# iris1997jiatong/I-DCCRN-VAE

Hardware: AMD Instinct MI355X
Metric: 4s@16kHz utterances/sec fwd+SI-SNR, DCCRN-CL, 1/2/4/8 MI355X vs host CPU (higher is better)
Workload: dtype f32; 1 GPU; supervised DCCRN-CL forward(train=False) + final_ete_loss (weights 0/0/1); batch_per_gpu=64, utterance=4 s @ 16 kHz (64000 samples, 641 frames), parallelism=replicas x1, streams=1, input=resident in HBM

## Files before the change

i-dccrn-vae_amd/csrc/cgemm_tw.hip:

```cpp
#include <atomic>
#include <cstdint>
#include <cstdlib>
#include <type_traits>
#include "cgemm.hpp"
#include "../../include/idccrn_hip.h"

namespace {

struct TwArgs {
    const float* x0;
    const float* x1;
    int C0, C1;
    int Fin, Fout;
    int J, Jp, Tp;
    const float* wfrag;
    int UP;
    const float* epi;
    int has_fold;
    const float* slope;
    float* out;
    int Cout, cotiles;
    int tshift, t_valid;
    double* stats;
    int stats_rep;
    const float* add;
    int add_div, add_Jp;
    int jtiles, ftiles;
    int xcd_split;
    int cgroups;
    int stagger;
};

constexpr int TW_PACK_CI = 8;

template <int PH> __device__ __forceinline__ int tw_ra(int r) {
    if (PH == 0) return r == 0 ? 0 : (r == 2 ? 2 : 1);
    return r == 0 ? 1 : 2;
}
template <int PH> __device__ __forceinline__ int tw_rb(int r) {
    if (PH == 0) return r == 2 ? 1 : (r == 3 ? 3 : 2);
    return r == 0 ? 2 : 3;
}
template <int PH> __device__ __forceinline__ float tw_cb(int r) {
    if (PH == 0) return r == 1 ? 1.f : -1.f;
    return r == 1 ? 0.f : -1.f;
}
template <int PH> constexpr int tw_nr() { return PH == 0 ? 4 : 3; }
template <int PH> constexpr int tw_nt() { return tw_nr<PH>() * 9; }
template <int PH> constexpr int tw_ntp() { return PH == 0 ? 36 : 32; }
template <int PH> constexpr int tw_ntw() { return (tw_nt<PH>() + 3) / 4; }
__host__ __device__ inline int tw_tile(int ph, int w, int k) {
    if (ph == 0) return w * 9 + k;
    if (w < 3) return k < 6 ? w * 9 + k : w * 9 + 8;
    return k < 6 ? (k >> 1) * 9 + 6 + (k & 1) : -1;
}
template <int PH> constexpr int tw_wslots() { return PH == 0 ? 9 : 8; }

template <int PH, int CIK, bool LEFT, int DBG = 0, int RDW = 2, bool WVEC = true, bool STATS = false, int NCT = 1>
__global__ __launch_bounds__(256 * NCT, NCT == 1 ? 2 : 1) void cconv_tw_kernel(const TwArgs a) {
    constexpr int NR = tw_nr<PH>(), NT = tw_nt<PH>(), NTP = tw_ntp<PH>(), NTW = tw_ntw<PH>();
    constexpr int NRAW = PH == 0 ? 4 : 3, ROW0 = PH == 0 ? 0 : 1;
    constexpr int KS = CIK / 2;
    constexpr int RT = NRAW * 9 * 32;
    constexpr int NE = CIK * RT;
    constexpr int NBUF = 2;
    constexpr int NITEM = CIK * NRAW * 16;
    constexpr int NTHR = 256 * NCT;
    constexpr int NLD = (NITEM + NTHR - 1) / NTHR;
    static_assert(NCT == 1 || NCT == 2, "one or two co tiles per workgroup");
    static_assert(KS % RDW == 0 && NLD <= 2, "weight ring slots are compile-time; at most two staging items per thread");
    static_assert(NLD + NCT - 1 < KS, "the staging k-steps (from 1 on, waves 4 .. 7 one later) end before the barrier's k-step");
    static_assert(NCT * NT * 4 * 64 <= NBUF * NE, "the epilogue exchange (one area per co tile) fits the patch buffers");

    extern __shared__ __attribute__((aligned(16))) float smem[];

    const int tid = threadIdx.x;
    const int lane = tid & 63;
    const int wave = __builtin_amdgcn_readfirstlane(tid >> 6);
    const int w4 = NCT == 1 ? wave : wave & 3, cth = NCT == 1 ? 0 : wave >> 2;
    const int half = lane >> 5, l31 = lane & 31;

    const int bid = blockIdx.x;
    const int xcd = bid & 7, slot = bid >> 3;
    int jt, ft, ct;
    if (a.xcd_split) {
        const int G = 8 / a.cgroups;
        ct = xcd % a.cgroups;
        jt = (slot / a.ftiles) * G + xcd / a.cgroups;
        ft = slot - (slot / a.ftiles) * a.ftiles;
    } else {
        const int per = a.cgroups * a.ftiles;
        jt = (slot / per) * 8 + xcd;
        const int rem = slot - (slot / per) * per;
        ft = rem / a.cgroups;
        ct = rem - ft * a.cgroups;
    }
    if (jt >= a.jtiles) return;
    ct = NCT * ct + cth;
    const int j0 = jt * 64;
    const int m0 = 2 * ft;
    const int rbase = m0 - 1 + ROW0;

    const int Cin = a.C0 + a.C1;
    const int nchunk = (Cin + CIK - 1) / CIK;

    f32x16 acc[NTW];
#pragma unroll
    for (int k = 0; k < NTW; ++k)
#pragma unroll
        for (int r = 0; r < 16; ++r) acc[k][r] = 0.f;
    constexpr int NPAIR = (NTW - 1) / 2;
    constexpr bool UNI = PH == 0;
    int offA[UNI ? 1 : NPAIR + 1], offB[UNI ? 1 : NPAIR + 1];
    float cbj[UNI ? 1 : NPAIR + 1];
    if (UNI) {
        cbj[0] = tw_cb<PH>(w4);
        offA[0] = (tw_ra<PH>(w4) - ROW0) * 288;
        offB[0] = (tw_rb<PH>(w4) - ROW0) * 288;
    } else {
#pragma unroll
        for (int j = 0; j <= NPAIR; ++j) {
            int t = tw_tile(PH, w4, j < NPAIR ? 2 * j : NTW - 1);
            t = t < 0 ? 0 : t;
            const int r = t / 9, plane = t - r * 9;
            cbj[j] = tw_cb<PH>(r);
            const int po = plane == 8 ? 256 : (plane >> 1) * 64;
            offA[j] = (tw_ra<PH>(r) - ROW0) * 288 + po;
            offB[j] = cbj[j] != 0.f ? (tw_rb<PH>(r) - ROW0) * 288 + po : offA[j];
        }
    }

    f32x4 v_r[NLD], v_i[NLD];
    float e_r[NLD], e_i[NLD];
    unsigned off_v[NLD], off_e[NLD], ldsoff[NLD];
    unsigned okmask[NLD];
    int item_cl[NLD];
    bool interior[NLD];
#pragma unroll
    for (int i = 0; i < NLD; ++i) {
        const int e = tid + i * NTHR;
        const int c8 = e & 15;
        const int rl = (e >> 4) % NRAW, cl = e / (16 * NRAW);
        item_cl[i] = cl;
        const int f = rbase + rl;
        const int jc = j0 + 4 * c8;
        const int je = LEFT ? jc - 1 : jc + 4;
        const bool exists = e < NITEM;
        const bool okr = exists && f >= 0 && f < a.Fin;
        unsigned m = 0;
#pragma unroll
        for (int q = 0; q < 5; ++q) {
            const int c = jc + q + (LEFT ? -1 : 0);
            if (c >= 0 && c < a.J) m |= 1u << q;
        }
        if (okr) m |= 1u << 5;
        if (exists) m |= 1u << 7;
        const int jcv = jc + 3 < a.Jp ? jc : 0;
        const int jev = (je >= 0 && je < a.Jp) ? je : 0;
        off_v[i] = okr ? (unsigned)((cl * a.Fin + f) * a.Jp + jcv) : 0u;
        off_e[i] = okr ? (unsigned)((cl * a.Fin + f) * a.Jp + jev) : 0u;
        if (jc + 3 >= a.Jp) m &= ~0x1fu;
        if (!(je >= 0 && je < a.Jp)) m &= LEFT ? ~1u : ~(1u << 4);
        okmask[i] = m;
        interior[i] = __builtin_amdgcn_ballot_w64((m & 0xbfu) == 0xbfu) == ~0ull;
        ldsoff[i] = (unsigned)((cl * NRAW + rl) * 288 + 4 * c8);
    }
    auto stage_load = [&](int chunk, int i) {
        const int ci0 = chunk * CIK;
        const bool from0 = ci0 < a.C0;
        const float* br = from0 ? a.x0 + (size_t)ci0 * a.Fin * a.Jp : a.x1 + (size_t)(ci0 - a.C0) * a.Fin * a.Jp;
        const float* bi = from0 ? br + (size_t)a.C0 * a.Fin * a.Jp : br + (size_t)a.C1 * a.Fin * a.Jp;
        const int cvalid = (from0 ? a.C0 : Cin) - ci0;
        const bool dead = item_cl[i] >= cvalid;
        const unsigned ov = dead ? 0u : off_v[i], oe = dead ? 0u : off_e[i];
        v_r[i] = *(const f32x4*)(br + ov);
        v_i[i] = *(const f32x4*)(bi + ov);
        e_r[i] = br[oe];
        e_i[i] = bi[oe];
    };
    float fr[5], fi[5];
    auto stage_window = [&](int chunk, int i) {
        const int ci0s = chunk * CIK;
        const int cvalid = (ci0s < a.C0 ? a.C0 : Cin) - ci0s;
        constexpr bool left = LEFT;
        if (interior[i] && cvalid >= CIK) {
#pragma unroll
            for (int q = 0; q < 5; ++q) {
                fr[q] = left ? (q == 0 ? e_r[i] : v_r[i][q == 0 ? 0 : q - 1]) : (q == 4 ? e_r[i] : v_r[i][q == 4 ? 3 : q]);
                fi[q] = left ? (q == 0 ? e_i[i] : v_i[i][q == 0 ? 0 : q - 1]) : (q == 4 ? e_i[i] : v_i[i][q == 4 ? 3 : q]);
            }
            return;
        }
        unsigned m = okmask[i];
        if (item_cl[i] >= cvalid || !((m >> 5) & 1u)) m &= ~0x1fu;
#pragma unroll
        for (int q = 0; q < 5; ++q) {
            const float xr = left ? (q == 0 ? e_r[i] : v_r[i][q == 0 ? 0 : q - 1]) : (q == 4 ? e_r[i] : v_r[i][q == 4 ? 3 : q]);
            const float xi = left ? (q == 0 ? e_i[i] : v_i[i][q == 0 ? 0 : q - 1]) : (q == 4 ? e_i[i] : v_i[i][q == 4 ? 3 : q]);
            const bool cok = (m >> q) & 1u;
            fr[q] = cok ? xr : 0.f;
            fi[q] = cok ? xi : 0.f;
        }
    };
    auto plane_val = [&](int gt, int pr) -> float {
        const int g = gt / 3, tau = gt - g * 3;
        const int q0 = 2 * pr;
        const float xa_ = g == 0 ? fr[q0] + fi[q0] : (g == 1 ? fr[q0] : fi[q0]);
        const float xb_ = g == 0 ? fr[q0 + 1] + fi[q0 + 1] : (g == 1 ? fr[q0 + 1] : fi[q0 + 1]);
        const float xd_ = g == 0 ? fr[q0 + 2] + fi[q0 + 2] : (g == 1 ? fr[q0 + 2] : fi[q0 + 2]);
        return tau == 0 ? xa_ - xb_ : (tau == 1 ? xb_ : xb_ - xd_);
    };
    auto item_exists = [&](int i) -> bool { return NITEM >= (i + 1) * NTHR || wave * 64 + i * NTHR < NITEM; };
    auto stage_plane2 = [&](float* dst, int i, int j) {
        if (!item_exists(i)) return;
        if (j < 4) {
            f32x4 o = {plane_val(2 * j, 0), plane_val(2 * j + 1, 0), plane_val(2 * j, 1), plane_val(2 * j + 1, 1)};
            *(f32x4*)(dst + ldsoff[i] + j * 64) = o;
        } else {
            *(float2*)(dst + ldsoff[i] - 2 * (int)(tid & 15) + 256) = make_float2(plane_val(8, 0), plane_val(8, 1));
        }
    };
    auto stage_store = [&](float* dst, int chunk, int i) {
        stage_window(chunk, i);
#pragma unroll
        for (int j = 0; j < 5; ++j) stage_plane2(dst, i, j);
    };

    constexpr int WS = tw_wslots<PH>();
    const float* wbase = a.wfrag + ((size_t)(PH == 1 ? (size_t)a.cotiles * a.UP * tw_ntp<0>() : 0) + (size_t)ct * a.UP * NTP) * 64 +
                         (size_t)w4 * WS * 64;
    const int total_ks = nchunk * KS;
    float a_w[RDW][NTW];
    auto load_w = [&](int g, float (&dst)[NTW]) {
        g = g < total_ks ? g : total_ks - 1;
        const float* ws = wbase + (size_t)g * NTP * 64;
        if (WVEC) {
            const f32x4 w0 = *(const f32x4*)(ws + lane * 4), w1 = *(const f32x4*)(ws + 256 + lane * 4);
#pragma unroll
            for (int k = 0; k < 4; ++k) {
                dst[k] = w0[k];
                if (4 + k < NTW) dst[4 + k] = w1[k];
            }
            if (NTW == 9) dst[NTW - 1] = ws[512 + lane];
        } else {
#pragma unroll
            for (int k = 0; k < NTW; ++k) dst[k] = ws[k * 64 + lane];
        }
    };
    float xa[NTW], xb[NTW];
    auto load_raw2 = [&](const float* base, int j) {
        if (j < NPAIR) {
            const int oa = UNI ? offA[0] + j * 64 : offA[UNI ? 0 : j], ob = UNI ? offB[0] + j * 64 : offB[UNI ? 0 : j];
            const float2 pa_ = *(const float2*)(base + oa + 2 * l31), pb_ = *(const float2*)(base + ob + 2 * l31);
            xa[2 * j] = pa_.x; xa[2 * j + 1] = pa_.y;
            xb[2 * j] = pb_.x; xb[2 * j + 1] = pb_.y;
        } else {
            xa[NTW - 1] = base[(UNI ? offA[0] + 256 : offA[UNI ? 0 : NPAIR]) + l31];
            xb[NTW - 1] = base[(UNI ? offB[0] + 256 : offB[UNI ? 0 : NPAIR]) + l31];
        }
    };
    auto load_raw_all = [&](const float* base) {
#pragma unroll
        for (int j = 0; j <= NPAIR; ++j) load_raw2(base, j);
    };

#pragma unroll
    for (int i = 0; i < NLD; ++i) stage_load(0, i);
#pragma unroll
    for (int u = 0; u < RDW; ++u) load_w(u, a_w[u]);
#pragma unroll
    for (int i = 0; i < NLD; ++i) stage_store(smem, 0, i);
#pragma unroll
    for (int i = 0; i < NLD; ++i) stage_load(nchunk > 1 ? 1 : 0, i);
    __syncthreads();

    load_raw_all(smem + (size_t)half * RT);
    auto run = [&](auto late_) {
        constexpr bool LATE = decltype(late_)::value;
        for (int chunk = 0; chunk < nchunk; ++chunk) {
            const float* P = smem + (chunk & 1) * NE;
            float* Pn = smem + ((chunk + 1) & 1) * NE;
            const int nxt = chunk + 1 < nchunk ? chunk + 1 : chunk, nxt2 = chunk + 2 < nchunk ? chunk + 2 : nchunk - 1;
#pragma unroll
            for (int ul = 0; ul < KS; ++ul) {
                const float* bnext = ul + 1 < KS ? P + (size_t)(2 * (ul + 1) + half) * RT : Pn + (size_t)half * RT;
                const int si = ul - 1 - (LATE ? 1 : 0);
                const bool staging = !(DBG & 1) && si >= 0 && si < NLD;
#pragma unroll
                for (int k = 0; k < NTW; ++k) {
                    const float b = xa[k] + cbj[UNI ? 0 : (k >> 1 < NPAIR ? k >> 1 : NPAIR)] * xb[k];
                    acc[k] = __builtin_amdgcn_mfma_f32_32x32x2f32(a_w[ul % RDW][k], b, acc[k], 0, 0, 0);
                    if (ul == KS - 1 && k == 0) {
                        __builtin_amdgcn_sched_barrier(0);
                        __syncthreads();
                    }
                    if ((k & 1) && (k >> 1) < NPAIR) load_raw2(bnext, k >> 1);
                    if (k == NTW - 1) load_raw2(bnext, NPAIR);
                    if (staging) {
                        if (k == 0) stage_window(nxt, si);
                        if ((k & 1) && k < 6) stage_plane2(Pn, si, k >> 1);
                        if (k == (NTW == 9 ? 7 : 6)) stage_plane2(Pn, si, 3);
                        if (k == NTW - 1) stage_plane2(Pn, si, 4);
                        if (k == NTW - 1) stage_load(nxt2, si);
                    }
                    __builtin_amdgcn_sched_barrier(0);
                }
                if (!(DBG & 2)) load_w(chunk * KS + ul + RDW, a_w[ul % RDW]);
            }
        }
    };
    if (NCT == 2 && PH == 1 && a.stagger && cth)
        run(std::integral_constant<bool, NCT == 2 && PH == 1>{});
    else
        run(std::false_type{});
    __syncthreads();

    const float slope = a.slope ? *a.slope : 1.0f;
    const bool has_act = a.slope != nullptr;
    float* E = smem + cth * (NT * 4 * 64);
    const int jA = j0 + 2 * l31;
    bool keep[2], inb[2];
    int ja[2];
#pragma unroll
    for (int q = 0; q < 2; ++q) {
        const int j = jA + q;
        const int bj = j / a.Tp, tp = j - bj * a.Tp;
        inb[q] = j < a.J;
        keep[q] = inb[q] && tp >= 1 && tp <= a.t_valid;
        ja[q] = j - (bj - bj / a.add_div) * a.Tp;
    }
#pragma unroll
    for (int s = 0; s < ((DBG & 4) ? 1 : 4); ++s) {
        if (s > 0) __syncthreads();
#pragma unroll
        for (int k = 0; k < NTW; ++k) {
            const int t = tw_tile(PH, w4, k);
            if (t >= 0) {
#pragma unroll
                for (int rr = 0; rr < 4; ++rr) E[(t * 4 + rr) * 64 + lane] = acc[k][4 * s + rr];
            }
        }
        __syncthreads();
        float v[NT];
#pragma unroll
        for (int t = 0; t < NT; ++t) v[t] = E[(t * 4 + w4) * 64 + lane];
        float pr[NR][2], pi[NR][2];
#pragma unroll
        for (int r = 0; r < NR; ++r) {
            float y[3][2];
#pragma unroll
            for (int g = 0; g < 3; ++g) {
                const float m1 = v[r * 9 + g * 3], m2 = v[r * 9 + g * 3 + 1], m3 = v[r * 9 + g * 3 + 2];
                y[g][0] = m1 + m2;
                y[g][1] = m2 - m3;
            }
#pragma unroll
            for (int q = 0; q < 2; ++q) {
                pr[r][q] = y[0][q] - y[2][q];
                pi[r][q] = y[0][q] + y[1][q];
            }
        }
        const int rg = 4 * s + w4;
        const int co = ct * 32 + (rg & 3) + 8 * (rg >> 2) + 4 * half;
        const bool cok = co < a.Cout;
        const f32x4 e0 = *(const f32x4*)(a.epi + (size_t)co * 8);
        const float e4 = a.epi[(size_t)co * 8 + 4], e5 = a.epi[(size_t)co * 8 + 5];
        float st[5] = {0.f, 0.f, 0.f, 0.f, 0.f};
#pragma unroll
        for (int rt = 0; rt < 2; ++rt) {
            const int fo = 2 * m0 + PH + 2 * rt;
            if (fo >= a.Fout) continue;
            float yr[2], yi[2];
#pragma unroll
            for (int q = 0; q < 2; ++q) {
                float re, im;
                if (PH == 0) {
                    re = rt == 0 ? pr[0][q] + pr[1][q] + pr[2][q] : pr[1][q] - pr[2][q] - pr[NR - 1][q];
                    im = rt == 0 ? pi[0][q] + pi[1][q] + pi[2][q] : pi[1][q] - pi[2][q] - pi[NR - 1][q];
                } else {
                    re = rt == 0 ? pr[0][q] + pr[1][q] : pr[1][q] - pr[2][q];
                    im = rt == 0 ? pi[0][q] + pi[1][q] : pi[1][q] - pi[2][q];
                }
                if (a.add && cok && inb[q]) {
                    re += a.add[((size_t)co * a.Fout + fo) * a.add_Jp + ja[q]];
                    im += a.add[((size_t)(a.Cout + co) * a.Fout + fo) * a.add_Jp + ja[q]];
                }
                float r_, i_;
                if (a.has_fold) {
                    r_ = e0[0] * re + e0[1] * im + e4;
                    i_ = e0[2] * re + e0[3] * im + e5;
                } else {
                    r_ = re + e4;
                    i_ = im + e5;
                }
                if (has_act) {
                    r_ = r_ >= 0.f ? r_ : slope * r_;
                    i_ = i_ >= 0.f ? i_ : slope * i_;
                }
                yr[q] = keep[q] ? r_ : 0.f;
                yi[q] = keep[q] ? i_ : 0.f;
                if (STATS && keep[q]) {
                    st[0] += yr[q];
                    st[1] += yi[q];
                    st[2] += yr[q] * yr[q];
                    st[3] += yi[q] * yi[q];
                    st[4] += yr[q] * yi[q];
                }
            }
            if (cok) {
                float* o_r = a.out + ((size_t)co * a.Fout + fo) * a.Jp + jA;
                float* o_i = a.out + ((size_t)(a.Cout + co) * a.Fout + fo) * a.Jp + jA;
                if (inb[1]) {
                    *(float2*)o_r = make_float2(yr[0], yr[1]);
                    *(float2*)o_i = make_float2(yi[0], yi[1]);
                } else if (inb[0]) {
                    o_r[0] = yr[0];
                    o_i[0] = yi[0];
                }
            }
        }
        if (STATS) {
#pragma unroll
            for (int q = 0; q < 5; ++q) {
                float tsum = st[q];
#pragma unroll
                for (int o = 16; o > 0; o >>= 1) tsum += __shfl_xor(tsum, o, 64);
                if (l31 == 0 && cok)
                    atomicAdd(&a.stats[((size_t)(a.stats_rep > 1 ? (blockIdx.x & (a.stats_rep - 1)) : 0) * a.Cout + co) * 5 + q], (double)tsum);
            }
        }
    }
}

__global__ void pack_cconv_tw_kernel(const float* __restrict__ wino, int cotiles, int UN, int UP, int vec, float* __restrict__ out) {
    const long long n0 = (long long)cotiles * UP * tw_ntp<0>() * 64, n1 = (long long)cotiles * UP * tw_ntp<1>() * 64;
    for (long long idx = blockIdx.x * (long long)blockDim.x + threadIdx.x; idx < n0 + n1; idx += (long long)gridDim.x * blockDim.x) {
        const int ph = idx >= n0;
        const long long i = ph ? idx - n0 : idx;
        const int ntp = ph ? tw_ntp<1>() : tw_ntp<0>(), nt = ph ? tw_nt<1>() : tw_nt<0>();
        const int lane = (int)(i & 63);
        long long t_ = i >> 6;
        const int t = (int)(t_ % ntp); t_ /= ntp;
        const int u = (int)(t_ % UP);
        const int ct = (int)(t_ / UP);
        float val = 0.f;
        const int ws_ = ph ? tw_wslots<1>() : tw_wslots<0>();
        const int pos = t * 64 + lane, w = pos / (ws_ * 64), q = pos % (ws_ * 64);
        const bool vec_ = (vec >> ph) & 1;
        const int k = !vec_ ? q >> 6 : (q < 512 ? (q >> 8) * 4 + (q & 3) : 8);
        const int ln = !vec_ ? q & 63 : (q < 512 ? (q & 255) >> 2 : q - 512);
        const int tt = k < (ph ? 7 : 9) ? tw_tile(ph, w, k) : -1;
        const int ci = 2 * u + (ln >> 5), co = ln & 31;
        if (tt >= 0 && ci * 3 < UN) {
            const int r = tt / 9, g = (tt % 9) / 3, tau = tt % 3;
            const float* src = wino + ((((size_t)ph * cotiles + ct) * UN + (size_t)ci * 3 + g) * 4 + r) * 64;
            const float w0 = src[co], w1 = src[32 + co];
            val = tau == 0 ? w0 : (tau == 1 ? w0 + w1 : w1);
        }
        out[idx] = val;
    }
}

template <int PH, int CIK, bool LEFT, int DBG, int RDW, bool WVEC = true, bool STATS = false, int NCT = 1>
int launch_tw_ph_l(const TwArgs& a, hipStream_t st);
inline int tw_wvec_mask() {
    static const int v = [] { const char* e = getenv("IDV_TW_WVEC"); return e ? atoi(e) : 1; }();
    return v;
}
template <int PH, int CIK, int DBG = 0, int RDW = 2>
int launch_tw_ph(const TwArgs& a, hipStream_t st) {
    const bool wv = (tw_wvec_mask() >> PH) & 1;
    if (DBG == 0 && RDW == 2 && wv == (PH == 0) && a.cotiles % 2 == 0 && ((idv_tw_pair(-1) >> PH) & 1)) {
        constexpr bool WV = PH == 0;
        if (a.stats) return a.tshift ? launch_tw_ph_l<PH, CIK, true, 0, 2, WV, true, 2>(a, st) : launch_tw_ph_l<PH, CIK, false, 0, 2, WV, true, 2>(a, st);
        return a.tshift ? launch_tw_ph_l<PH, CIK, true, 0, 2, WV, false, 2>(a, st) : launch_tw_ph_l<PH, CIK, false, 0, 2, WV, false, 2>(a, st);
    }
    if (DBG == 0 && RDW == 2 && a.stats) {
        constexpr bool WV = PH == 0;
        if (wv != WV) return IDV_EINVAL;
        return a.tshift ? launch_tw_ph_l<PH, CIK, true, 0, 2, WV, true>(a, st) : launch_tw_ph_l<PH, CIK, false, 0, 2, WV, true>(a, st);
    }
    if (DBG == 0 && RDW == 2 && !wv)
        return a.tshift ? launch_tw_ph_l<PH, CIK, true, 0, 2, false>(a, st) : launch_tw_ph_l<PH, CIK, false, 0, 2, false>(a, st);
    return a.tshift ? launch_tw_ph_l<PH, CIK, true, DBG, RDW>(a, st) : launch_tw_ph_l<PH, CIK, false, DBG, RDW>(a, st);
}
template <int PH, int CIK, bool LEFT, int DBG, int RDW, bool WVEC, bool STATS, int NCT>
int launch_tw_ph_l(const TwArgs& a, hipStream_t st) {
    constexpr int NE = CIK * (PH == 0 ? 4 : 3) * 9 * 32;
    constexpr size_t smem = 2 * NE * sizeof(float);
    static_assert(smem * (NCT == 1 ? 2 : 1) <= 160 * 1024, "the patch buffers of two workgroups (NCT = 2: of one) must fit the 160 KB of LDS");
    TwArgs b = a;
    b.jtiles = (a.J + 63) / 64;
    b.ftiles = PH == 1 ? a.Fin / 2 : (a.Fin + 1) / 2;
    if (b.ftiles == 0) return IDV_OK;
    static const int xsplit = [] { const char* e = getenv("IDV_TW_XCD_SPLIT"); return e ? atoi(e) : 1; }();
    b.cgroups = b.cotiles / NCT;
    if (b.cgroups * NCT != b.cotiles) return IDV_EINVAL;
    static const int stag = [] { const char* e = getenv("IDV_TW_PAIR_STAGGER"); return e ? atoi(e) : 1; }();
    b.stagger = stag;
    b.xcd_split = (xsplit && (b.cgroups == 2 || b.cgroups == 4 || b.cgroups == 8)) ? 1 : 0;
    long long nblk = (long long)((b.jtiles + 7) / 8) * 8 * b.ftiles * b.cgroups;
    if (b.xcd_split) {
        const int G = 8 / b.cgroups;
        nblk = (long long)((b.jtiles + G - 1) / G) * b.ftiles * 8;
    }
    if (nblk > 0x7fffffffLL) return IDV_EINVAL;
    auto k = cconv_tw_kernel<PH, CIK, LEFT, DBG, RDW, WVEC, STATS, NCT>;
    static std::atomic<bool> attr_set[64];
    int dev = 0;
    if (hipGetDevice(&dev) != hipSuccess || dev < 0 || dev >= 64) return IDV_ELAUNCH;
    if (smem > 64 * 1024 && !attr_set[dev].load(std::memory_order_acquire)) {
        if (hipFuncSetAttribute((const void*)k, hipFuncAttributeMaxDynamicSharedMemorySize, (int)smem) != hipSuccess) return IDV_ELAUNCH;
        attr_set[dev].store(true, std::memory_order_release);
    }
    hipLaunchKernelGGL(k, dim3((unsigned)nblk), dim3(256 * NCT), smem, st, b);
    if (NCT > 1) idv_tw_pair_note_launch();
    return idv_launch_status();
}

}

namespace {
std::atomic<int>& tw_pair_mask() {
    static std::atomic<int> v{[] { const char* e = getenv("IDV_TW_PAIR"); return e ? atoi(e) & IDV_TW_PAIR_ALL : IDV_TW_PAIR_DEFAULT; }()};
    return v;
}
std::atomic<long long> tw_pair_launches{0};
}
void idv_tw_pair_note_launch() { tw_pair_launches.fetch_add(1, std::memory_order_relaxed); }
extern "C" int idv_tw_pair(int mask) {
    if (mask < 0) return tw_pair_mask().load(std::memory_order_relaxed);
    return tw_pair_mask().exchange(mask & IDV_TW_PAIR_ALL, std::memory_order_relaxed);
}
extern "C" long long idv_tw_pair_launches(int reset) {
    return reset ? tw_pair_launches.exchange(0, std::memory_order_relaxed) : tw_pair_launches.load(std::memory_order_relaxed);
}

extern "C" int idv_cconv_tw_supported(int C0, int C1, int Cout, int Fin) {
    static const int min_cout = [] { const char* e = getenv("IDV_TW_MIN_COUT"); return e ? atoi(e) : 32; }();
    if (Cout < min_cout || Fin < 2) return 0;
    if (!idv_cconv_gauss_supported(C0, C1, Cout)) return 0;
    return (C1 == 0 || C0 % 8 == 0) ? 1 : 0;
}

extern "C" long long idv_cconv_tw_wfrag_floats(int Cout, int cin_used) {
    const long long cotiles = (Cout + 31) / 32, cpad = (cin_used + TW_PACK_CI - 1) / TW_PACK_CI * TW_PACK_CI;
    return cotiles * (cpad / 2) * (36 + 32) * 64;
}

extern "C" int idv_pack_cconv_tw(const float* wino_frag, int Cout, int cin_used, float* tw_frag, void* stream) {
    if (!wino_frag || !tw_frag || Cout <= 0 || cin_used <= 0) return IDV_EINVAL;
    const int cotiles = (Cout + 31) / 32;
    const int cpad = (cin_used + TW_PACK_CI - 1) / TW_PACK_CI * TW_PACK_CI;
    const long long n = idv_cconv_tw_wfrag_floats(Cout, cin_used);
    const unsigned blocks = (unsigned)((n + 255) / 256 > 4096 ? 4096 : (n + 255) / 256);
    hipLaunchKernelGGL(pack_cconv_tw_kernel, dim3(blocks), dim3(256), 0, (hipStream_t)stream, wino_frag, cotiles, cpad * 3, cpad / 2,
                       tw_wvec_mask(), tw_frag);
    return idv_launch_status();
}

extern "C" int idv_ctconv2d_tw_fwd(const float* x0, int C0, const float* x1, int C1, const float* wfrag, const float* epi, int has_fold,
                                   const float* prelu_slope, float* out, double* stats, double* stats_work, int stats_rep, int tshift,
                                   int Cout, int Fin, int B, int Tp, int Jp, int t_valid_out, const float* addend, int addend_div,
                                   int addend_Jp, void* stream) {
    if (!x0 || !wfrag || !epi || !out || C0 <= 0 || Cout <= 0 || Fin <= 0 || B <= 0 || Tp <= 1) return IDV_EINVAL;
    if (stats && stats_work && (stats_rep < 2 || (stats_rep & (stats_rep - 1)))) return IDV_EINVAL;
    if (addend && (addend_div < 1 || B % addend_div || addend_Jp < (B / addend_div) * Tp)) return IDV_EINVAL;
    if (C1 > 0 && !x1) return IDV_EINVAL;
    if (tshift != 0 && tshift != -1) return IDV_EINVAL;
    if (!idv_cconv_tw_supported(C0, C1, Cout, Fin)) return IDV_EINVAL;
    if ((Jp & 3) || (reinterpret_cast<uintptr_t>(x0) & 15) || (C1 > 0 && (reinterpret_cast<uintptr_t>(x1) & 15)) ||
        (reinterpret_cast<uintptr_t>(out) & 7))
        return IDV_EINVAL;
    TwArgs a{};
    a.x0 = x0; a.x1 = x1; a.C0 = C0; a.C1 = C1;
    a.Fin = Fin; a.Fout = 2 * Fin - 1;
    a.J = B * Tp; a.Jp = Jp; a.Tp = Tp;
    a.wfrag = wfrag; a.UP = (C0 + C1 + TW_PACK_CI - 1) / TW_PACK_CI * TW_PACK_CI / 2;
    a.epi = epi; a.has_fold = has_fold; a.slope = prelu_slope; a.out = out;
    a.Cout = Cout; a.cotiles = (Cout + 31) / 32;
    a.tshift = tshift; a.t_valid = t_valid_out;
    a.add = addend; a.add_div = addend ? addend_div : 1; a.add_Jp = addend_Jp;
    if (Jp < a.J) return IDV_EINVAL;
    if ((long long)8 * Fin * (long long)Jp >= 0xffffffffLL) return IDV_EINVAL;
    hipStream_t st = (hipStream_t)stream;
    a.stats = stats;
    if (stats && stats_work) { a.stats = stats_work; a.stats_rep = stats_rep; }
    int rc = 0;
#ifdef IDV_TW_EXPERIMENTS
    static const int dbg = [] { const char* e = getenv("IDV_TW_DBG"); return e ? atoi(e) : 0; }();
    static const int only = [] { const char* e = getenv("IDV_TW_ONLY"); return e ? atoi(e) : 0; }();
    if (dbg && !stats) {
        if (only != 2) rc = dbg == 1 ? launch_tw_ph<0, 8, 1>(a, st) : (dbg == 2 ? launch_tw_ph<0, 8, 2>(a, st) : launch_tw_ph<0, 8, 3>(a, st));
        if (rc) return rc;
        if (only != 1) rc = dbg == 1 ? launch_tw_ph<1, 8, 1>(a, st) : (dbg == 2 ? launch_tw_ph<1, 8, 2>(a, st) : launch_tw_ph<1, 8, 3>(a, st));
        return rc;
    }
    if (only) return only == 1 ? launch_tw_ph<0, 8>(a, st) : launch_tw_ph<1, 8>(a, st);
#endif
    rc = launch_tw_ph<0, 8>(a, st);
    if (!rc) rc = launch_tw_ph<1, 8>(a, st);
    if (rc || !(stats && stats_work)) return rc;
    return idv_launch_stats_collapse(stats_work, stats_rep, Cout * 5, stats, st);
}
```

i-dccrn-vae_amd/csrc/cgemm_tw2.hip:

```cpp
#include <atomic>
#include <cstdint>
#include <cstdlib>
#include <type_traits>
#include "cgemm.hpp"
#include "../../include/idccrn_hip.h"

namespace {

struct Tw2Args {
    const float* x0;
    int Cin;
    int Fin, Fout;
    int J, Jp, Tp;
    const float* wfrag;
    int UP;
    const float* epi;
    int has_fold;
    const float* slope;
    float* out;
    int Cout, cotiles;
    int tshift, t_valid;
    double* stats;
    int stats_rep;
    int jtiles, ftiles;
    int xcd_split;
    int cgroups;
    int stagger;
};

constexpr int TW2_PACK_CI = 8;

__host__ __device__ constexpr int tw2_ra(int q) { return q == 0 ? 0 : (q == 1 ? 2 : (q == 2 ? 4 : (q == 3 ? 2 : (q == 4 ? 1 : 3)))); }
__host__ __device__ constexpr int tw2_rb(int q) { return q == 0 ? 4 : (q == 1 ? 4 : (q == 2 ? 2 : (q == 3 ? 6 : (q == 4 ? 3 : (q == 5 ? 3 : 5))))); }
__host__ __device__ constexpr float tw2_cb(int q) { return q == 1 ? 1.f : (q == 5 ? 0.f : -1.f); }
__host__ __device__ constexpr int tw2_qx(int a) { return a == 0 ? 0 : (a == 1 ? 1 : 3); }
__host__ __device__ constexpr int tw2_qy(int a) { return a == 0 ? 4 : (a == 1 ? 5 : 6); }
__host__ __device__ constexpr int tw2_main_acc(int w) { return w == 2 ? 3 : w; }
__host__ __device__ inline void tw2_slot(int w, int k, int& q, int& plane) {
    if (w < 3) {
        if (k < 14) { q = (k & 1) ? tw2_qy(tw2_main_acc(w)) : tw2_qx(tw2_main_acc(w)); plane = k >> 1; }
        else { q = 2; plane = 2 * w + (k - 14); }
    } else {
        if (k < 12) { const int a = tw2_main_acc(k >> 2); q = (k & 1) ? tw2_qy(a) : tw2_qx(a); plane = 7 + ((k >> 1) & 1); }
        else if (k < 15) { q = 2; plane = 6 + (k - 12); }
        else { q = -1; plane = 0; }
    }
}
__host__ __device__ inline int tw2_acc_tile(int w, int i) {
    if (w < 3) return i < 7 ? tw2_main_acc(w) * 9 + i : 2 * 9 + 2 * w + (i - 7);
    return i < 6 ? tw2_main_acc(i >> 1) * 9 + 7 + (i & 1) : 2 * 9 + 6 + (i - 6);
}

__device__ __forceinline__ int tw2_poff(int p, int l31) { return p < 8 ? (p >> 1) * 64 + 2 * l31 + (p & 1) : 256 + l31; }

constexpr int tw2_smem_floats(int nct) {
    return nct == 1 ? 2 * 4 * 7 * 288 : (2 * (4 * 7 * 288 + 288) > 2 * 36 * 4 * 64 ? 2 * (4 * 7 * 288 + 288) : 2 * 36 * 4 * 64);
}
template <bool LEFT, bool STATS, int DBG = 0, int NCT = 1>
__global__ __launch_bounds__(256 * NCT, NCT == 1 ? 2 : 1) void cconv_tw2_kernel(const Tw2Args a) {
    constexpr int NT = 36, NACC = 9, NSLOT = 16;
    constexpr int NRAW = 7, CIK = 4, KS = 2;
    constexpr int RT = NRAW * 288;
    constexpr int NE = CIK * RT;
    constexpr int NEB = NCT == 1 ? NE : NE + 288;
    constexpr int NITEM = CIK * NRAW * 16;
    constexpr int NTHR = 256 * NCT;
    constexpr int NLD = (NITEM + NTHR - 1) / NTHR;
    static_assert(NCT == 1 || NCT == 2, "one or two co tiles per workgroup");
    static_assert(2 * NEB <= tw2_smem_floats(NCT) && NCT * NT * 4 * 64 <= tw2_smem_floats(NCT),
                  "the patch buffers and the epilogue exchange (one area per co tile) fit the allocation");

    extern __shared__ __attribute__((aligned(16))) float smem[];

    const int tid = threadIdx.x;
    const int lane = tid & 63;
    const int wave = __builtin_amdgcn_readfirstlane(tid >> 6);
    const int w4 = NCT == 1 ? wave : wave & 3, cth = NCT == 1 ? 0 : wave >> 2;
    const int half = lane >> 5, l31 = lane & 31;

    const int bid = blockIdx.x;
    const int xcd = bid & 7, slot = bid >> 3;
    int jt, ft, ct;
    if (a.xcd_split) {
        const int G = 8 / a.cgroups;
        ct = xcd % a.cgroups;
        jt = (slot / a.ftiles) * G + xcd / a.cgroups;
        ft = slot - (slot / a.ftiles) * a.ftiles;
    } else {
        const int per = a.cgroups * a.ftiles;
        jt = (slot / per) * 8 + xcd;
        const int rem = slot - (slot / per) * per;
        ft = rem / a.cgroups;
        ct = rem - ft * a.cgroups;
    }
    if (jt >= a.jtiles) return;
    ct = NCT * ct + cth;
    const int j0 = jt * 64;
    const int m0 = 2 * ft;
    const int rbase = 2 * m0 - 2;

    const int Cin = a.Cin;
    const int nchunk = (Cin + CIK - 1) / CIK;

    f32x16 acc[NACC];
#pragma unroll
    for (int k = 0; k < NACC; ++k)
#pragma unroll
        for (int r = 0; r < 16; ++r) acc[k][r] = 0.f;

    f32x4 v_r[NLD], v_i[NLD];
    float e_r[NLD], e_i[NLD];
    unsigned off_v[NLD], ldsoff[NLD];
    unsigned okmask[NLD];
    bool interior[NLD];
    auto item_cl = [&](int i) -> int { return (tid + i * NTHR) / (16 * NRAW); };
#pragma unroll
    for (int i = 0; i < NLD; ++i) {
        const int e = tid + i * NTHR;
        const int c8 = e & 15;
        const int cl = e / (16 * NRAW), rl = (NCT == 2 && e >= NITEM) ? 0 : (e >> 4) % NRAW;
        const int f = rbase + rl;
        const int jc = j0 + 4 * c8;
        const int je = LEFT ? jc - 1 : jc + 4;
        const bool exists = e < NITEM;
        const bool okr = exists && f >= 0 && f < a.Fin;
        unsigned m = 0;
#pragma unroll
        for (int q = 0; q < 5; ++q) {
            const int c = jc + q + (LEFT ? -1 : 0);
            if (c >= 0 && c < a.J) m |= 1u << q;
        }
        if (okr) m |= 1u << 5;
        const int jcv = jc + 3 < a.Jp ? jc : 0;
        off_v[i] = okr ? (unsigned)((cl * a.Fin + f) * a.Jp + jcv) : 4u;
        if (jc + 3 >= a.Jp) m &= ~0x1fu;
        if (!(je >= 0 && je < a.Jp)) m &= LEFT ? ~1u : ~(1u << 4);
        okmask[i] = m;
        interior[i] = __builtin_amdgcn_ballot_w64((m & 0x3fu) == 0x3fu) == ~0ull;
        ldsoff[i] = (unsigned)((cl * NRAW + rl) * 288 + 4 * c8);
    }
    auto item_exists = [&](int i) -> bool { return i == 0 || wave * 64 + 256 < NITEM; };
    auto stage_load = [&](int chunk, int i) {
        if (!item_exists(i)) return;
        const int ci0 = chunk * CIK;
        const float* br = a.x0 + (size_t)ci0 * a.Fin * a.Jp;
        const float* bi = br + (size_t)Cin * a.Fin * a.Jp;
        const bool dead = item_cl(i) >= Cin - ci0;
        const unsigned ov = dead ? 4u : off_v[i];
        v_r[i] = *(const f32x4*)(br + ov);
        v_i[i] = *(const f32x4*)(bi + ov);
        e_r[i] = (br + ov)[LEFT ? -1 : 4];
        e_i[i] = (bi + ov)[LEFT ? -1 : 4];
    };
    float fr[5], fi[5];
    auto stage_window = [&](int chunk, int i) {
        if (!item_exists(i)) return;
        const int cvalid = Cin - chunk * CIK;
        constexpr bool left = LEFT;
        if (interior[i] && cvalid >= CIK) {
#pragma unroll
            for (int q = 0; q < 5; ++q) {
                fr[q] = left ? (q == 0 ? e_r[i] : v_r[i][q == 0 ? 0 : q - 1]) : (q == 4 ? e_r[i] : v_r[i][q == 4 ? 3 : q]);
                fi[q] = left ? (q == 0 ? e_i[i] : v_i[i][q == 0 ? 0 : q - 1]) : (q == 4 ? e_i[i] : v_i[i][q == 4 ? 3 : q]);
            }
            return;
        }
        unsigned m = okmask[i];
        if (item_cl(i) >= cvalid || !((m >> 5) & 1u)) m &= ~0x1fu;
#pragma unroll
        for (int q = 0; q < 5; ++q) {
            const float xr = left ? (q == 0 ? e_r[i] : v_r[i][q == 0 ? 0 : q - 1]) : (q == 4 ? e_r[i] : v_r[i][q == 4 ? 3 : q]);
            const float xi = left ? (q == 0 ? e_i[i] : v_i[i][q == 0 ? 0 : q - 1]) : (q == 4 ? e_i[i] : v_i[i][q == 4 ? 3 : q]);
            const bool cok = (m >> q) & 1u;
            fr[q] = cok ? xr : 0.f;
            fi[q] = cok ? xi : 0.f;
        }
    };
    auto plane_val = [&](int gt, int pr) -> float {
        const int g = gt / 3, tau = gt - g * 3;
        const int q0 = 2 * pr;
        const float xa_ = g == 0 ? fr[q0] + fi[q0] : (g == 1 ? fr[q0] : fi[q0]);
        const float xb_ = g == 0 ? fr[q0 + 1] + fi[q0 + 1] : (g == 1 ? fr[q0 + 1] : fi[q0 + 1]);
        const float xd_ = g == 0 ? fr[q0 + 2] + fi[q0 + 2] : (g == 1 ? fr[q0 + 2] : fi[q0 + 2]);
        return tau == 0 ? xa_ - xb_ : (tau == 1 ? xb_ : xb_ - xd_);
    };
    auto stage_plane2 = [&](float* dst, int i, int j) {
        if (!item_exists(i)) return;
        if (j < 4) {
            f32x4 o = {plane_val(2 * j, 0), plane_val(2 * j + 1, 0), plane_val(2 * j, 1), plane_val(2 * j + 1, 1)};
            *(f32x4*)(dst + ldsoff[i] + j * 64) = o;
        } else {
            *(float2*)(dst + ldsoff[i] - 2 * (int)(tid & 15) + 256) = make_float2(plane_val(8, 0), plane_val(8, 1));
        }
    };
    auto stage_store = [&](float* dst, int chunk, int i) {
        stage_window(chunk, i);
#pragma unroll
        for (int j = 0; j < 5; ++j) stage_plane2(dst, i, j);
    };

    const float* wbase = a.wfrag + (((size_t)ct * a.UP) * 4 + w4) * 1024 + lane * 4;
    const int total_ks = nchunk * KS;
    float a_w[NSLOT];
    auto load_wg = [&](int g, int grp) {
        g = g < total_ks ? g : total_ks - 1;
        const f32x4 w4 = *(const f32x4*)(wbase + (size_t)g * 4096 + grp * 256);
#pragma unroll
        for (int k = 0; k < 4; ++k) a_w[grp * 4 + k] = w4[k];
    };

    const int am = tw2_main_acc(w4 < 3 ? w4 : 0);
    const int qxm = tw2_qx(am), qym = tw2_qy(am);
    const int rxa = tw2_ra(qxm) * 288, rxb = tw2_rb(qxm) * 288, rya = tw2_ra(qym) * 288, ryb = tw2_rb(qym) * 288;
    const float cbx = tw2_cb(qxm), cby = tw2_cb(qym);
    const int r2a = tw2_ra(2) * 288 + w4 * 64, r2b = tw2_rb(2) * 288 + w4 * 64;
    float xa[2][4], xb[2][4];
    auto load_grp_a = [&](const float* base, int g, float (&oa)[4], float (&ob)[4]) {
        if (g < 3) {
            const float2 xa_ = *(const float2*)(base + rxa + g * 64 + 2 * l31), xb_ = *(const float2*)(base + rxb + g * 64 + 2 * l31);
            const float2 ya_ = *(const float2*)(base + rya + g * 64 + 2 * l31), yb_ = *(const float2*)(base + ryb + g * 64 + 2 * l31);
            oa[0] = xa_.x; oa[2] = xa_.y; ob[0] = xb_.x; ob[2] = xb_.y;
            oa[1] = ya_.x; oa[3] = ya_.y; ob[1] = yb_.x; ob[3] = yb_.y;
        } else {
            oa[0] = base[rxa + 3 * 64 + 2 * l31]; ob[0] = base[rxb + 3 * 64 + 2 * l31];
            oa[1] = base[rya + 3 * 64 + 2 * l31]; ob[1] = base[ryb + 3 * 64 + 2 * l31];
            const float2 pa_ = *(const float2*)(base + r2a + 2 * l31), pb_ = *(const float2*)(base + r2b + 2 * l31);
            oa[2] = pa_.x; oa[3] = pa_.y; ob[2] = pb_.x; ob[3] = pb_.y;
        }
    };
    auto load_grp_b = [&](const float* base, int g, float (&oa)[4], float (&ob)[4]) {
#pragma unroll
        for (int s4 = 0; s4 < 4; ++s4) {
            int q, plane;
            tw2_slot(3, 4 * g + s4, q, plane);
            if (q < 0) continue;
            oa[s4] = base[tw2_ra(q) * 288 + tw2_poff(plane, l31)];
            ob[s4] = base[tw2_rb(q) * 288 + tw2_poff(plane, l31)];
        }
    };

#pragma unroll
    for (int i = 0; i < NLD; ++i) stage_load(0, i);
#pragma unroll
    for (int grp = 0; grp < 4; ++grp) load_wg(0, grp);
#pragma unroll
    for (int i = 0; i < NLD; ++i) stage_store(smem, 0, i);
#pragma unroll
    for (int i = 0; i < NLD; ++i) stage_load(nchunk > 1 ? 1 : 0, i);
    __syncthreads();
    if (w4 < 3)
        load_grp_a(smem + (size_t)half * RT, 0, xa[0], xb[0]);
    else
        load_grp_b(smem + (size_t)half * RT, 0, xa[0], xb[0]);

    auto run = [&](auto role, auto late_) {
        constexpr bool ROLE_B = decltype(role)::value;
        for (int chunk = 0; chunk < nchunk; ++chunk) {
            const float* P = smem + (chunk & 1) * NEB;
            float* Pn = smem + ((chunk + 1) & 1) * NEB;
            const int nxt = chunk + 1 < nchunk ? chunk + 1 : chunk, nxt2 = chunk + 2 < nchunk ? chunk + 2 : nchunk - 1;
#pragma unroll
            for (int ul = 0; ul < KS; ++ul) {
                const float* bnext = ul + 1 < KS ? P + (size_t)(2 * (ul + 1) + half) * RT : Pn + (size_t)half * RT;
                const bool staging = !(DBG & 1) && ul == 0;
#pragma unroll
                for (int k = 0; k < (ROLE_B ? NSLOT - 1 : NSLOT); ++k) {
                    const int g = k >> 2, s4 = k & 3;
                    float cb;
                    int ai;
                    if (ROLE_B) {
                        int q, plane;
                        tw2_slot(3, k, q, plane);
                        cb = tw2_cb(q);
                        ai = k < 12 ? k >> 1 : 6 + (k - 12);
                    } else {
                        cb = k < 14 ? ((k & 1) ? cby : cbx) : -1.f;
                        ai = k < 14 ? k >> 1 : 7 + (k - 14);
                    }
                    if (s4 == 0) {
                        const float* src = g < 3 ? P + (size_t)(2 * ul + half) * RT : bnext;
                        if (!(ul == KS - 1 && g == 3)) {
                            if (ROLE_B) load_grp_b(src, (g + 1) & 3, xa[(g + 1) & 1], xb[(g + 1) & 1]);
                            else load_grp_a(src, (g + 1) & 3, xa[(g + 1) & 1], xb[(g + 1) & 1]);
                        }
                    }
                    const float b = xa[g & 1][s4] + cb * xb[g & 1][s4];
                    acc[ai] = __builtin_amdgcn_mfma_f32_32x32x2f32(a_w[k], b, acc[ai], 0, 0, 0);
                    if (ul == KS - 1 && k == 0) {
                        __builtin_amdgcn_sched_barrier(0);
                        __syncthreads();
                    }
                    if (ul == KS - 1 && k == 12) {
                        if (ROLE_B) load_grp_b(bnext, 0, xa[0], xb[0]);
                        else load_grp_a(bnext, 0, xa[0], xb[0]);
                    }
                    if (((k & 3) == 3 || (ROLE_B && k == NSLOT - 2)) && !(DBG & 2)) load_wg(chunk * KS + ul + 1, k >> 2);
                    if constexpr (NCT == 2) if (staging) {
                        constexpr bool late = decltype(late_)::value;
                        if (k <= 5 && !late) {
                            if (k == 0) stage_window(nxt, 0);
                            if (k >= 1) stage_plane2(Pn, 0, k - 1);
                            if (k == 5) stage_load(nxt2, 0);
                        }
                        if (k >= 8 && k <= 13 && late) {
                            if (k == 8) stage_window(nxt, 0);
                            if (k >= 9) stage_plane2(Pn, 0, k - 9);
                            if (k == 13) stage_load(nxt2, 0);
                        }
                    }
                    if constexpr (NCT == 1) if (staging) {
                        if (k == 0) stage_window(nxt, 0);
                        if (k >= 1 && k <= 5) stage_plane2(Pn, 0, k - 1);
                        if (k == 5) stage_load(nxt2, 0);
                        if (!ROLE_B) {
                            if (k == 8) stage_window(nxt, 1);
                            if (k >= 9 && k <= 13) stage_plane2(Pn, 1, k - 9);
                            if (k == 13) stage_load(nxt2, 1);
                        }
                    }
                    __builtin_amdgcn_sched_barrier(0);
                }
            }
        }
    };
    if (NCT == 2 && a.stagger && cth) {
        if (w4 < 3)
            run(std::false_type{}, std::integral_constant<bool, NCT == 2>{});
        else
            run(std::true_type{}, std::integral_constant<bool, NCT == 2>{});
    } else if (w4 < 3)
        run(std::false_type{}, std::false_type{});
    else
        run(std::true_type{}, std::false_type{});
    __syncthreads();

    const float slope = a.slope ? *a.slope : 1.0f;
    const bool has_act = a.slope != nullptr;
    float* E = smem + cth * (NT * 4 * 64);
    const int jA = j0 + 2 * l31;
    bool keep[2], inb[2];
#pragma unroll
    for (int q = 0; q < 2; ++q) {
        const int j = jA + q;
        const int tp = j % a.Tp;
        inb[q] = j < a.J;
        keep[q] = inb[q] && tp >= 1 && tp <= a.t_valid;
    }
#pragma unroll
    for (int s = 0; s < 4; ++s) {
        if (s > 0) __syncthreads();
#pragma unroll
        for (int k = 0; k < NACC; ++k) {
            const int t = tw2_acc_tile(w4, k);
#pragma unroll
            for (int rr = 0; rr < 4; ++rr) E[(t * 4 + rr) * 64 + lane] = acc[k][4 * s + rr];
        }
        __syncthreads();
        float v[NT];
#pragma unroll
        for (int t = 0; t < NT; ++t) v[t] = E[(t * 4 + w4) * 64 + lane];
        float pr[4][2], pi[4][2];
#pragma unroll
        for (int r = 0; r < 4; ++r) {
            float y[3][2];
#pragma unroll
            for (int g = 0; g < 3; ++g) {
                const float m1 = v[r * 9 + g * 3], m2 = v[r * 9 + g * 3 + 1], m3 = v[r * 9 + g * 3 + 2];
                y[g][0] = m1 + m2;
                y[g][1] = m2 - m3;
            }
#pragma unroll
            for (int q = 0; q < 2; ++q) {
                pr[r][q] = y[0][q] - y[2][q];
                pi[r][q] = y[0][q] + y[1][q];
            }
        }
        const int rg = 4 * s + w4;
        const int co = ct * 32 + (rg & 3) + 8 * (rg >> 2) + 4 * half;
        const bool cok = co < a.Cout;
        const f32x4 e0 = *(const f32x4*)(a.epi + (size_t)co * 8);
        const float e4 = a.epi[(size_t)co * 8 + 4], e5 = a.epi[(size_t)co * 8 + 5];
        float st[5] = {0.f, 0.f, 0.f, 0.f, 0.f};
#pragma unroll
        for (int rt = 0; rt < 2; ++rt) {
            const int fo = m0 + rt;
            if (fo >= a.Fout) continue;
            float yr[2], yi[2];
#pragma unroll
            for (int q = 0; q < 2; ++q) {
                const float re = rt == 0 ? pr[0][q] + pr[1][q] + pr[2][q] : pr[1][q] - pr[2][q] - pr[3][q];
                const float im = rt == 0 ? pi[0][q] + pi[1][q] + pi[2][q] : pi[1][q] - pi[2][q] - pi[3][q];
                float r_, i_;
                if (a.has_fold) {
                    r_ = e0[0] * re + e0[1] * im + e4;
                    i_ = e0[2] * re + e0[3] * im + e5;
                } else {
                    r_ = re + e4;
                    i_ = im + e5;
                }
                if (has_act) {
                    r_ = r_ >= 0.f ? r_ : slope * r_;
                    i_ = i_ >= 0.f ? i_ : slope * i_;
                }
                yr[q] = keep[q] ? r_ : 0.f;
                yi[q] = keep[q] ? i_ : 0.f;
                if (STATS && keep[q]) {
                    st[0] += yr[q];
                    st[1] += yi[q];
                    st[2] += yr[q] * yr[q];
                    st[3] += yi[q] * yi[q];
                    st[4] += yr[q] * yi[q];
                }
            }
            if (cok) {
                float* o_r = a.out + ((size_t)co * a.Fout + fo) * a.Jp + jA;
                float* o_i = a.out + ((size_t)(a.Cout + co) * a.Fout + fo) * a.Jp + jA;
                if (inb[1]) {
                    *(float2*)o_r = make_float2(yr[0], yr[1]);
                    *(float2*)o_i = make_float2(yi[0], yi[1]);
                } else if (inb[0]) {
                    o_r[0] = yr[0];
                    o_i[0] = yi[0];
                }
            }
        }
        if (STATS) {
#pragma unroll
            for (int q = 0; q < 5; ++q) {
                float tsum = st[q];
#pragma unroll
                for (int o = 16; o > 0; o >>= 1) tsum += __shfl_xor(tsum, o, 64);
                if (l31 == 0 && cok)
                    atomicAdd(&a.stats[((size_t)(a.stats_rep > 1 ? (blockIdx.x & (a.stats_rep - 1)) : 0) * a.Cout + co) * 5 + q], (double)tsum);
            }
        }
    }
}

__global__ void pack_cconv_tw2_kernel(const float* __restrict__ wino, int cotiles, int UN, int UP, float* __restrict__ out) {
    const long long n = (long long)cotiles * UP * 4096;
    for (long long idx = blockIdx.x * (long long)blockDim.x + threadIdx.x; idx < n; idx += (long long)gridDim.x * blockDim.x) {
        const int kk = (int)(idx & 3), ln = (int)((idx >> 2) & 63), grp = (int)((idx >> 8) & 3), w = (int)((idx >> 10) & 3);
        const long long t_ = idx >> 12;
        const int u = (int)(t_ % UP), ct = (int)(t_ / UP);
        int q, plane;
        tw2_slot(w, grp * 4 + kk, q, plane);
        float val = 0.f;
        const int ci = 2 * u + (ln >> 5), co = ln & 31;
        if (q >= 0 && ci * 3 < UN) {
            const int g = plane / 3, tau = plane % 3;
            const float* src = wino + ((((size_t)ct * UN + (size_t)ci * 3 + g) * 8 + q)) * 64;
            const float w0 = src[co], w1 = src[32 + co];
            val = tau == 0 ? w0 : (tau == 1 ? w0 + w1 : w1);
        }
        out[idx] = val;
    }
}

template <bool LEFT, bool STATS, int DBG, int NCT = 1>
int launch_tw2(const Tw2Args& a, hipStream_t st) {
    constexpr size_t smem = tw2_smem_floats(NCT) * sizeof(float);
    static_assert(smem * (NCT == 1 ? 2 : 1) <= 160 * 1024, "the patch buffers of two workgroups (NCT = 2: of one) must fit the 160 KB of LDS");
    Tw2Args b = a;
    b.jtiles = (a.J + 63) / 64;
    b.ftiles = (a.Fout + 1) / 2;
    static const int xsplit = [] { const char* e = getenv("IDV_TW_XCD_SPLIT"); return e ? atoi(e) : 1; }();
    b.cgroups = b.cotiles / NCT;
    if (b.cgroups * NCT != b.cotiles) return IDV_EINVAL;
    static const int stag = [] { const char* e = getenv("IDV_TW_PAIR_STAGGER"); return e ? atoi(e) : 1; }();
    b.stagger = stag;
    b.xcd_split = (xsplit && (b.cgroups == 2 || b.cgroups == 4 || b.cgroups == 8)) ? 1 : 0;
    long long nblk = (long long)((b.jtiles + 7) / 8) * 8 * b.ftiles * b.cgroups;
    if (b.xcd_split) {
        const int G = 8 / b.cgroups;
        nblk = (long long)((b.jtiles + G - 1) / G) * b.ftiles * 8;
    }
    if (nblk > 0x7fffffffLL) return IDV_EINVAL;
    auto k = cconv_tw2_kernel<LEFT, STATS, DBG, NCT>;
    static std::atomic<bool> attr_set[64];
    int dev = 0;
    if (hipGetDevice(&dev) != hipSuccess || dev < 0 || dev >= 64) return IDV_ELAUNCH;
    if (smem > 64 * 1024 && !attr_set[dev].load(std::memory_order_acquire)) {
        if (hipFuncSetAttribute((const void*)k, hipFuncAttributeMaxDynamicSharedMemorySize, (int)smem) != hipSuccess) return IDV_ELAUNCH;
        attr_set[dev].store(true, std::memory_order_release);
    }
    hipLaunchKernelGGL(k, dim3((unsigned)nblk), dim3(256 * NCT), smem, st, b);
    if (NCT > 1) idv_tw_pair_note_launch();
    return idv_launch_status();
}

}

extern "C" int idv_cconv_tw2_supported(int Cin, int Cout, int Fin) {
    static const int min_cout = [] { const char* e = getenv("IDV_TW2_MIN_COUT"); return e ? atoi(e) : 32; }();
    static const int min_cin = [] { const char* e = getenv("IDV_TW2_MIN_CIN"); return e ? atoi(e) : 64; }();
    if (Cout < min_cout || Cin < min_cin || (Fin - 1) / 2 + 1 < 2) return 0;
    return idv_cconv_gauss_supported(Cin, 0, Cout);
}

extern "C" long long idv_cconv_tw2_wfrag_floats(int Cout, int cin_used) {
    const long long cotiles = (Cout + 31) / 32, cpad = (cin_used + TW2_PACK_CI - 1) / TW2_PACK_CI * TW2_PACK_CI;
    return cotiles * (cpad / 2) * 4096;
}

extern "C" int idv_pack_cconv_tw2(const float* wino_frag, int Cout, int cin_used, float* tw_frag, void* stream) {
    if (!wino_frag || !tw_frag || Cout <= 0 || cin_used <= 0) return IDV_EINVAL;
    const int cotiles = (Cout + 31) / 32;
    const int cpad = (cin_used + TW2_PACK_CI - 1) / TW2_PACK_CI * TW2_PACK_CI;
    const long long n = idv_cconv_tw2_wfrag_floats(Cout, cin_used);
    const unsigned blocks = (unsigned)((n + 255) / 256 > 4096 ? 4096 : (n + 255) / 256);
    hipLaunchKernelGGL(pack_cconv_tw2_kernel, dim3(blocks), dim3(256), 0, (hipStream_t)stream, wino_frag, cotiles, cpad * 3, cpad / 2,
                       tw_frag);
    return idv_launch_status();
}

extern "C" int idv_cconv2d_tw_fwd(const float* x0, int Cin, const float* wfrag, const float* epi, int has_fold, const float* prelu_slope,
                                  float* out, double* stats, double* stats_work, int stats_rep, int tshift, int Cout, int Fin, int B, int Tp,
                                  int Jp, int t_valid_out, void* stream) {
    if (!x0 || !wfrag || !epi || !out || Cin <= 0 || Cout <= 0 || Fin <= 0 || B <= 0 || Tp <= 1) return IDV_EINVAL;
    if (stats && stats_work && (stats_rep < 2 || (stats_rep & (stats_rep - 1)))) return IDV_EINVAL;
    if (tshift != 0 && tshift != -1) return IDV_EINVAL;
    if (!idv_cconv_tw2_supported(Cin, Cout, Fin)) return IDV_EINVAL;
    if ((Jp & 3) || (reinterpret_cast<uintptr_t>(x0) & 15) || (reinterpret_cast<uintptr_t>(out) & 7)) return IDV_EINVAL;
    Tw2Args a{};
    a.x0 = x0; a.Cin = Cin;
    a.Fin = Fin; a.Fout = (Fin - 1) / 2 + 1;
    a.J = B * Tp; a.Jp = Jp; a.Tp = Tp;
    a.wfrag = wfrag; a.UP = (Cin + TW2_PACK_CI - 1) / TW2_PACK_CI * TW2_PACK_CI / 2;
    a.epi = epi; a.has_fold = has_fold; a.slope = prelu_slope; a.out = out;
    a.Cout = Cout; a.cotiles = (Cout + 31) / 32;
    a.tshift = tshift; a.t_valid = t_valid_out;
    if (Jp < a.J) return IDV_EINVAL;
    if ((long long)4 * Fin * (long long)Jp >= 0xffffffffLL) return IDV_EINVAL;
    hipStream_t st = (hipStream_t)stream;
    a.stats = stats;
    if (stats && stats_work) { a.stats = stats_work; a.stats_rep = stats_rep; }
    int rc;
#ifdef IDV_TW_EXPERIMENTS
    static const int dbg = [] { const char* e = getenv("IDV_TW_DBG"); return e ? atoi(e) : 0; }();
    if (!stats && dbg == 1) return tshift ? launch_tw2<true, false, 1>(a, st) : launch_tw2<false, false, 1>(a, st);
    if (!stats && dbg == 2) return tshift ? launch_tw2<true, false, 2>(a, st) : launch_tw2<false, false, 2>(a, st);
    if (!stats && dbg == 3) return tshift ? launch_tw2<true, false, 3>(a, st) : launch_tw2<false, false, 3>(a, st);
#endif
    const bool pair = a.cotiles % 2 == 0 && (idv_tw_pair(-1) & IDV_TW_PAIR_CONV);
    if (stats && pair)
        rc = tshift ? launch_tw2<true, true, 0, 2>(a, st) : launch_tw2<false, true, 0, 2>(a, st);
    else if (stats)
        rc = tshift ? launch_tw2<true, true, 0>(a, st) : launch_tw2<false, true, 0>(a, st);
    else if (pair)
        rc = tshift ? launch_tw2<true, false, 0, 2>(a, st) : launch_tw2<false, false, 0, 2>(a, st);
    else
        rc = tshift ? launch_tw2<true, false, 0>(a, st) : launch_tw2<false, false, 0>(a, st);
    if (rc || !(stats && stats_work)) return rc;
    return idv_launch_stats_collapse(stats_work, stats_rep, Cout * 5, stats, st);
}
```

i-dccrn-vae_amd/csrc/common.hpp:

```cpp
#pragma once
#include <hip/hip_runtime.h>
#include <stdint.h>

#define IDV_SLACK 256

typedef float f32x16 __attribute__((ext_vector_type(16)));
typedef float f32x4 __attribute__((ext_vector_type(4)));

#define IDV_OK 0
#define IDV_EINVAL (-1)
#define IDV_ELAUNCH (-2)

static inline int idv_launch_status() {
    hipError_t e = hipGetLastError();
    return e == hipSuccess ? IDV_OK : IDV_ELAUNCH;
}

__device__ __forceinline__ float wave_sum(float v) {
#pragma unroll
    for (int o = 32; o > 0; o >>= 1) v += __shfl_xor(v, o, 64);
    return v;
}
__device__ __forceinline__ double wave_sum_d(double v) {
#pragma unroll
    for (int o = 32; o > 0; o >>= 1) v += __shfl_xor(v, o, 64);
    return v;
}

__device__ __forceinline__ float sigmoidf_(float x) {
    return __builtin_amdgcn_rcpf(1.0f + __builtin_amdgcn_exp2f(-1.44269504088896341f * x));
}
__device__ __forceinline__ float tanhf_(float x) {
    return 2.0f * __builtin_amdgcn_rcpf(1.0f + __builtin_amdgcn_exp2f(-2.88539008177792681f * x)) - 1.0f;
}

int idv_launch_stats_collapse(const double* work, int rep, int n, double* stats, hipStream_t st);
void idv_tw_pair_note_launch();
```

i-dccrn-vae_amd/ops.py:

```python
from __future__ import annotations

import os
from typing import Optional, Sequence

import torch

from . import _lib as L
from ._lib import call, p, i, f, d, ll, stream_ptr

SLACK = 256

PRECISION = os.environ.get("IDV_PRECISION", "fp32")


def set_precision(mode: str):
    global PRECISION
    if mode not in ("fp32", "bf16x3"):
        raise ValueError("precision must be 'fp32' or 'bf16x3'")
    PRECISION = mode


def bucket(n: int) -> int:
    if n <= 4096:
        return n
    step = 1 << (n.bit_length() - 4)
    return (n + step - 1) // step * step


class Planar:

    __slots__ = ("buf", "C", "F", "B", "T", "Tp", "Jp", "lengths")

    def __init__(self, buf, C, F, B, T, Tp, Jp, lengths=None):
        self.buf, self.C, self.F, self.B, self.T, self.Tp, self.Jp, self.lengths = buf, C, F, B, T, Tp, Jp, lengths

    @staticmethod
    def jp_for(B: int, Tp: int) -> int:
        return (B * Tp + 3) // 4 * 4

    @classmethod
    def empty(cls, C, F, B, T, Tp, device, zero=False):
        Jp = cls.jp_for(B, Tp)
        n = bucket(2 * C * F * Jp + 2 * SLACK)
        buf = (torch.zeros if zero else torch.empty)(n, dtype=torch.float32, device=device)
        return cls(buf, C, F, B, T, Tp, Jp)

    @property
    def data(self) -> torch.Tensor:
        return self.buf[SLACK:SLACK + 2 * self.C * self.F * self.Jp]

    def ptr(self, plane_offset: int = 0):
        return L._P(self.buf.data_ptr() + 4 * (SLACK + plane_offset * self.F * self.Jp))

    def planes(self) -> torch.Tensor:
        return torch.as_strided(self.buf, (2, self.C, self.F, self.B, self.Tp),
                                (self.C * self.F * self.Jp, self.F * self.Jp, self.Jp, self.Tp, 1), SLACK)

    def tensor5(self) -> torch.Tensor:
        return self.planes()[..., 1:1 + self.T].permute(3, 1, 2, 4, 0)

    def tensor4(self) -> torch.Tensor:
        return self.tensor5()[:, 0]

    def channel_slice(self, c0: int, c1: int) -> torch.Tensor:
        assert self.F == 1
        return self.planes()[:, c0:c1, 0, :, 1:1 + self.T].permute(2, 3, 1, 0)

    @classmethod
    def from_tensor5(cls, x: torch.Tensor, Tp: Optional[int] = None):
        B, C, F, T, _ = x.shape
        Tp = Tp or T + 1
        out = cls.empty(C, F, B, T, Tp, x.device, zero=True)
        out.tensor5().copy_(x)
        return out


IMG_SLACK = 4096
IMAGE_PATH = os.environ.get("IDV_IMAGE_PATH", "1") != "0"
IMAGE_TRAIN = os.environ.get("IDV_IMAGE_TRAIN", "1") != "0"


class Image:

    __slots__ = ("buf", "C", "F", "B", "T", "Tp", "Jp", "lo_off")

    def __init__(self, buf, C, F, B, T, Tp, Jp, lo_off):
        self.buf, self.C, self.F, self.B, self.T, self.Tp, self.Jp, self.lo_off = buf, C, F, B, T, Tp, Jp, lo_off

    @classmethod
    def empty(cls, C, F, B, T, Tp, device):
        Jp = Planar.jp_for(B, Tp)
        plane = (2 * C + 7) // 8 * F * Jp * 8
        lo_off = plane + IMG_SLACK
        buf = torch.empty(bucket(2 * IMG_SLACK + lo_off + plane), dtype=torch.int16, device=device)
        return cls(buf, C, F, B, T, Tp, Jp, lo_off)

    def ptr(self):
        return L._P(self.buf.data_ptr() + 2 * IMG_SLACK)

    @property
    def lo_slots(self) -> int:
        return self.lo_off // 8


def to_image(x: Planar) -> Image:
    out = Image.empty(x.C, x.F, x.B, x.T, x.Tp, x.buf.device)
    call("idv_planar_to_image", x.ptr(), i(x.C), i(x.F), i(x.B * x.Tp), i(x.Jp), out.ptr(), ll(out.lo_off), stream_ptr())
    return out


def to_image_repeat(x: Planar, n: int) -> Image:
    out = Image.empty(x.C, x.F, x.B * n, x.T, x.Tp, x.buf.device)
    call("idv_planar_to_image_repeat", x.ptr(), i(x.C), i(x.F), i(x.B), i(x.Tp), i(x.Jp), i(n), out.ptr(), ll(out.lo_off),
         i(out.Jp), stream_ptr())
    return out


def to_planar(x: Image) -> Planar:
    out = Planar.empty(x.C, x.F, x.B, x.T, x.Tp, x.buf.device)
    call("idv_image_to_planar", x.ptr(), ll(x.lo_off), i(x.C), i(x.F), i(x.B * x.Tp), i(x.Jp), out.ptr(), stream_ptr())
    return out


class KImage:

    __slots__ = ("buf", "nplanes", "Jp", "lo_off")

    def __init__(self, nplanes: int, Jp: int, device):
        assert nplanes % 8 == 0
        plane = nplanes // 8 * Jp * 8
        self.nplanes, self.Jp, self.lo_off = nplanes, Jp, plane + IMG_SLACK
        self.buf = torch.empty(bucket(2 * IMG_SLACK + self.lo_off + plane), dtype=torch.int16, device=device)

    def ptr(self, octet: int = 0):
        return L._P(self.buf.data_ptr() + 2 * IMG_SLACK + 16 * octet * self.Jp)

    @property
    def lo_slots(self) -> int:
        return self.lo_off // 8

    @classmethod
    def from_planes(cls, x_ptr, nvalid: int, J: int, Jp: int, device, pad_to: int = 8):
        nplanes = (nvalid + pad_to - 1) // pad_to * pad_to
        out = cls(nplanes, Jp, device)
        call("idv_planar_to_kimage", x_ptr, i(nvalid), i(nplanes), i(J), i(Jp), out.ptr(), ll(out.lo_off), stream_ptr())
        return out


def pack_pw_bf16(w):
    M, K = w.shape
    L.lib().idv_pw_bf16_wfrag_bytes.restype = L._L
    wf = torch.empty(int(L.lib().idv_pw_bf16_wfrag_bytes(i(M), i(K))), dtype=torch.uint8, device=w.device)
    call("idv_pack_pw_bf16", p(w.contiguous()), i(M), i(K), p(wf), stream_ptr())
    return wf


def pw_bf16x3(kimg: KImage, octet0: int, K: int, wfrag16, bias, M: int, B: int, Tp: int, t_valid: int, out_ptr):
    call("idv_pw_bf16x3", kimg.ptr(octet0), ll(kimg.lo_slots), i(K), p(wfrag16), p(bias), out_ptr, i(M), i(B), i(Tp), i(kimg.Jp),
         i(t_valid), stream_ptr())


def pw_bf16x3_rows(kimg: KImage, K: int, wfrag16, bias, M: int, ldo: int, B: int, T: int, Tp: int, out_ptr):
    call("idv_pw_bf16x3_rows", kimg.ptr(), ll(kimg.lo_slots), i(K), p(wfrag16), p(bias), out_ptr, i(M), i(ldo), i(B), i(T), i(Tp),
         i(kimg.Jp), stream_ptr())


def _dev_scratch(n: int, device, dtype=torch.float32, zero=False):
    return (torch.zeros if zero else torch.empty)(n, dtype=dtype, device=device)


def mtiles_alloc(M: int) -> int:
    return (M + 127) // 128 * 4


def cbn_fold(moments, g_rr, g_ri, g_ii, b_r, b_i):
    C = g_rr.numel()
    fold = torch.empty(C, 6, dtype=torch.float32, device=g_rr.device)
    call("idv_cbn_fold", p(moments), p(g_rr), p(g_ri), p(g_ii), p(b_r), p(b_i), i(C), p(fold), stream_ptr())
    return fold


def pack_cconv(w_re, w_im, b_re, b_im, fold, cin_used: Optional[int] = None, transposed=False):
    if transposed:
        cin_total, cout = w_re.shape[0], w_re.shape[1]
    else:
        cout, cin_total = w_re.shape[0], w_re.shape[1]
    cin_used = cin_total if cin_used is None else cin_used
    cck = L.lib().idv_cconv_cck(cin_used)
    ccp = (2 * cin_used + cck - 1) // cck * cck
    mt = mtiles_alloc(2 * cout)
    wfrag = torch.empty(mt * ccp * 5 * 64, dtype=torch.float32, device=w_re.device)
    bias = torch.empty(mt * 32, dtype=torch.float32, device=w_re.device)
    call("idv_pack_cconv", p(w_re.contiguous()), p(w_im.contiguous()), p(b_re.contiguous()), p(b_im.contiguous()),
         p(fold), i(cout), i(cin_total), i(cin_used), i(1 if transposed else 0), p(wfrag), p(bias), stream_ptr())
    return wfrag, bias


SKIP_ONCE = os.environ.get("IDV_SKIP_ONCE", "1") != "0"
GAUSS_FWD = os.environ.get("IDV_GAUSS_FWD", "1") != "0"
GAUSS_BWD = os.environ.get("IDV_GAUSS_BWD", "1") != "0"


def gauss_supported(c0: int, c1: int, cout: int, bwd: bool = False) -> bool:
    if not (GAUSS_BWD if bwd else GAUSS_FWD):
        return False
    return bool(L.lib().idv_cconv_gauss_supported(i(c0), i(c1), i(cout)))


def pack_cconv_gauss(w_re, w_im, b_re, b_im, fold, cin_used: Optional[int] = None, transposed=False, *, adjoint_of=None):
    if adjoint_of is not None:
        cout, cin_total, cin_used, transposed = adjoint_of
    else:
        if transposed:
            cin_total, cout = w_re.shape[0], w_re.shape[1]
        else:
            cout, cin_total = w_re.shape[0], w_re.shape[1]
        cin_used = cin_total if cin_used is None else cin_used
    lib = L.lib()
    lib.idv_cconv_gauss_wfrag_floats.restype = L._L
    wfrag = torch.empty(int(lib.idv_cconv_gauss_wfrag_floats(i(cout), i(cin_used))), dtype=torch.float32, device=w_re.device)
    epi = torch.empty(int(lib.idv_cconv_gauss_epi_rows(i(cout))) * 8, dtype=torch.float32, device=w_re.device)
    if adjoint_of is not None:
        call("idv_pack_cconv_gauss", p(w_re), p(w_im), p(None), p(None), p(None), i(cout), i(cin_total), i(cin_used),
             i(1 if transposed else 0), i(1), p(wfrag), p(epi), stream_ptr())
        return (wfrag, epi, 0) + _pack_wino_tw(w_re, w_im, cout, cin_total, cin_used, transposed, 1)
    w_re, w_im = w_re.contiguous(), w_im.contiguous()
    call("idv_pack_cconv_gauss", p(w_re), p(w_im), p(b_re.contiguous()), p(b_im.contiguous()), p(fold),
         i(cout), i(cin_total), i(cin_used), i(1 if transposed else 0), i(0), p(wfrag), p(epi), stream_ptr())
    return (wfrag, epi, (1 if fold is not None else 0)) + _pack_wino_tw(w_re, w_im, cout, cin_total, cin_used, transposed, 0)


WINO = os.environ.get("IDV_WINO", "1") != "0"
WINO_CFG = 4000000


def _pack_wino(w_re, w_im, cout: int, cin_total: int, cin_used: int, transposed: bool, conj: int):
    if not WINO:
        return None
    n = int(_ll_fn("idv_cconv_wino_wfrag_floats")(i(1 if transposed else 0), i(cout), i(cin_used)))
    wf = torch.empty(n, dtype=torch.float32, device=w_re.device)
    call("idv_pack_cconv_wino", p(w_re), p(w_im), i(cout), i(cin_total), i(cin_used), i(1 if transposed else 0), i(conj), p(wf),
         stream_ptr())
    return wf


TW = os.environ.get("IDV_TW", "1") != "0"
TW_CONV = os.environ.get("IDV_TW_CONV", "1") != "0"
TW_CFG = 5000000
TW_PAIR = None
_tw_pair_lib = None
_tw_pair_pushed = None


def _sync_tw_pair():
    global _tw_pair_lib, _tw_pair_pushed
    if TW_PAIR == _tw_pair_pushed:
        return
    if _tw_pair_lib is None:
        _tw_pair_lib = int(L.lib().idv_tw_pair(-1))
    L.lib().idv_tw_pair(_tw_pair_lib if TW_PAIR is None else int(TW_PAIR))
    _tw_pair_pushed = TW_PAIR


def tw_pair_launches(reset: bool = False) -> int:
    return int(L.lib().idv_tw_pair_launches(1 if reset else 0))


def _pack_wino_tw(w_re, w_im, cout: int, cin_total: int, cin_used: int, transposed: bool, conj: int):
    wf = _pack_wino(w_re, w_im, cout, cin_total, cin_used, transposed, conj)
    if wf is None or not TW or (not transposed and not TW_CONV):
        return wf, None
    if transposed:
        tw = torch.empty(int(_ll_fn("idv_cconv_tw_wfrag_floats")(i(cout), i(cin_used))), dtype=torch.float32, device=w_re.device)
        call("idv_pack_cconv_tw", p(wf), i(cout), i(cin_used), p(tw), stream_ptr())
    else:
        tw = torch.empty(int(_ll_fn("idv_cconv_tw2_wfrag_floats")(i(cout), i(cin_used))), dtype=torch.float32, device=w_re.device)
        call("idv_pack_cconv_tw2", p(wf), i(cout), i(cin_used), p(tw), stream_ptr())
    return wf, tw


def _tw2_ok(gauss, x: Planar, c1: int, cout: int) -> bool:
    return (gauss is not None and TW and TW_CONV and WINO and c1 == 0 and len(gauss) > 4 and gauss[4] is not None and x.Jp % 4 == 0
            and bool(L.lib().idv_cconv_tw2_supported(i(x.C), i(cout), i(x.F))))


def _tw_ok(gauss, x: Planar, c1: int, cout: int, skip_jp: Optional[int]) -> bool:
    return (gauss is not None and TW and WINO and len(gauss) > 4 and gauss[4] is not None and x.Jp % 4 == 0
            and (skip_jp is None or skip_jp == x.Jp) and bool(L.lib().idv_cconv_tw_supported(i(x.C), i(c1), i(cout), i(x.F))))


def _wino_ok(gauss, transposed: bool, x: Planar, c1: int, cout: int, skip_jp: Optional[int]) -> bool:
    return (gauss is not None and WINO and len(gauss) > 3 and gauss[3] is not None and x.Jp % 4 == 0
            and (skip_jp is None or skip_jp == x.Jp)
            and bool(L.lib().idv_cconv_wino_supported(i(1 if transposed else 0), i(x.C), i(c1), i(cout), i(x.F))))


def pack_cconv_gauss_skip_part(w_re, w_im, c0: int):
    wr, wi = w_re[c0:].contiguous(), w_im[c0:].contiguous()
    cin, cout = wr.shape[0], wr.shape[1]
    lib = L.lib()
    lib.idv_cconv_gauss_wfrag_floats.restype = L._L
    wfrag = torch.empty(int(lib.idv_cconv_gauss_wfrag_floats(i(cout), i(cin))), dtype=torch.float32, device=wr.device)
    epi = torch.empty(int(lib.idv_cconv_gauss_epi_rows(i(cout))) * 8, dtype=torch.float32, device=wr.device)
    call("idv_pack_cconv_gauss", p(wr), p(wi), p(None), p(None), p(None), i(cout), i(cin), i(cin), i(1), i(0), p(wfrag), p(epi),
         stream_ptr())
    return (wfrag, epi, 0) + _pack_wino_tw(wr, wi, cout, cin, cin, True, 0)


def bf16_supported(transposed: bool, c0: int, c1: int, skip_div: int, cout: int) -> bool:
    return bool(L.lib().idv_cconv_bf16_supported(i(1 if transposed else 0), i(c0), i(c1), i(skip_div), i(cout)))


def pack_cconv_bf16(w_re, w_im, fold, cin_used: Optional[int] = None, transposed=False):
    if transposed:
        cin_total, cout = w_re.shape[0], w_re.shape[1]
    else:
        cout, cin_total = w_re.shape[0], w_re.shape[1]
    cin_used = cin_total if cin_used is None else cin_used
    L.lib().idv_cconv_bf16_wfrag_bytes.restype = L._L
    nbytes = L.lib().idv_cconv_bf16_wfrag_bytes(i(cout), i(cin_used))
    wfrag = torch.empty(int(nbytes), dtype=torch.uint8, device=w_re.device)
    call("idv_pack_cconv_bf16", p(w_re.contiguous()), p(w_im.contiguous()), p(fold), i(cout), i(cin_total), i(cin_used),
         i(1 if transposed else 0), p(wfrag), stream_ptr())
    return wfrag


def pack_ctconv_c1(w_re, w_im, fold, cin_used: Optional[int] = None):
    cin_total = w_re.shape[0]
    cin_used = cin_total if cin_used is None else cin_used
    L.lib().idv_ctconv_c1_wfrag_bytes.restype = L._L
    wfrag = torch.empty(int(L.lib().idv_ctconv_c1_wfrag_bytes(i(cin_used))), dtype=torch.uint8, device=w_re.device)
    call("idv_pack_ctconv_c1_bf16", p(w_re.contiguous()), p(w_im.contiguous()), p(fold), i(cin_total), i(cin_used), p(wfrag),
         stream_ptr())
    return wfrag


def ctconv_c1(x, wfrag_c1, bias, *, slope=None, skip=None) -> Planar:
    out = Planar.empty(1, 2 * x.F - 1, x.B, x.T, x.Tp, x.buf.device)
    c1 = skip.C if skip is not None else 0
    if LAUNCH_LOG is not None:
        macs = 4 * (x.C + c1) * 10 * x.B * x.T * x.F
        ev0, ev1 = torch.cuda.Event(enable_timing=True), torch.cuda.Event(enable_timing=True)
        ev0.record()
    if isinstance(x, Image):
        if skip is not None and not isinstance(skip, Image):
            raise RuntimeError("ctconv_c1: x and skip must have the same format")
        call("idv_ctconv_c1_img_fwd", x.ptr(), ll(x.lo_slots), i(x.C), skip.ptr() if skip is not None else p(None),
             ll(skip.lo_slots if skip is not None else 0), i(c1), p(wfrag_c1), p(bias), p(slope), out.ptr(), i(x.F), i(x.B),
             i(x.Tp), i(x.Jp), i(x.T), stream_ptr())
    else:
        call("idv_ctconv_c1_bf16x3_fwd", x.ptr(), i(x.C), skip.ptr() if skip is not None else p(None), i(c1),
             i(skip.Jp if skip is not None else 0), p(wfrag_c1), p(bias), p(slope), out.ptr(), i(x.F), i(x.B), i(x.Tp), i(x.Jp),
             i(x.T), stream_ptr())
    if LAUNCH_LOG is not None:
        ev1.record()
        LAUNCH_LOG.append((-98 if isinstance(x, Image) else -99, macs, ev0, ev1))
    return out


def pack_pw(w, bias):
    M, K = w.shape
    mt = mtiles_alloc(M)
    ks = (K + 7) // 8 * 4
    wfrag = torch.empty(mt * ks * 64, dtype=torch.float32, device=w.device)
    bout = torch.empty(mt * 32, dtype=torch.float32, device=w.device)
    call("idv_pack_pw", p(w.contiguous()), p(None if bias is None else bias.contiguous()), i(M), i(K), p(wfrag),
         p(bout), stream_ptr())
    return wfrag, bout


LAUNCH_LOG = None

STREAM_SPLIT = int(os.environ.get("IDV_STREAM_SPLIT", "1"))
CONCURRENT = os.environ.get("IDV_CONCURRENT", "0") != "0"
STREAM_STAGGER = os.environ.get("IDV_STREAM_STAGGER", "1") != "0"
STREAM_STAGGER_BELOW = 1 << 30
STREAM_SPLIT_MIN_BATCH = 16
_SIDE_STREAMS = {}


def stream_split(batch: int) -> int:
    n = max(1, STREAM_SPLIT)
    while n > 1 and batch < n * STREAM_SPLIT_MIN_BATCH:
        n -= 1
    return n


def side_streams(n: int, device):
    key = (torch.device(device).index or 0)
    pool = _SIDE_STREAMS.setdefault(key, [])
    while len(pool) < n:
        pool.append(torch.cuda.Stream(device=device))
    return pool[:n]


def repeat_batch(x: Planar, n: int) -> Planar:
    out = Planar.empty(x.C, x.F, x.B * n, x.T, x.Tp, x.buf.device)
    dst = torch.as_strided(out.buf, (2, x.C, x.F, x.B, n, x.Tp),
                           (x.C * x.F * out.Jp, x.F * out.Jp, out.Jp, n * x.Tp, x.Tp, 1), SLACK)
    dst.copy_(x.planes().unsqueeze(4).expand(2, x.C, x.F, x.B, n, x.Tp))
    return out


def concurrent(fns, device=None):
    if not CONCURRENT:
        return [fn() for fn in fns]
    device = torch.device("cuda", torch.cuda.current_device()) if device is None else device
    main = torch.cuda.current_stream(device)
    streams = side_streams(len(fns), device)
    ready = torch.cuda.Event()
    ready.record(main)
    outs = []
    for fn, st in zip(fns, streams):
        st.wait_event(ready)
        with torch.cuda.stream(st):
            outs.append(fn())
    for st in streams:
        main.wait_stream(st)
    hand_over(outs, main)
    return outs


def hand_over(obj, stream):
    if isinstance(obj, torch.Tensor):
        if obj.is_cuda:
            obj.record_stream(stream)
        pl = getattr(obj, "_idv", None)
        if pl is not None and isinstance(getattr(pl, "buf", None), torch.Tensor) and pl.buf.is_cuda:
            pl.buf.record_stream(stream)
    elif isinstance(obj, (Planar, Image)):
        obj.buf.record_stream(stream)
    elif isinstance(obj, (tuple, list)):
        for o in obj:
            hand_over(o, stream)


class CoopTimeout(RuntimeError):
    """A cooperative (spin-synchronised) recurrence ran into its spin bound: its outputs are NaN-poisoned."""


def coop_check(sync: bool = True, clear: bool = True) -> None:
    if sync:
        torch.cuda.current_stream().synchronize()
    if L.lib().idv_coop_last_status(1 if clear else 0) != 0:
        raise CoopTimeout("a cooperative LSTM recurrence timed out on this device (a sibling workgroup never became resident, e.g. "
                          "a CU-masked or shared GPU): results computed since the last check are NaN-poisoned"
                          + ("" if clear else "; cooperative launches are refused until ops.coop_clear()"))


def coop_clear() -> bool:
    return L.lib().idv_coop_last_status(1) != 0


STATS_REP = int(os.environ.get("IDV_STATS_REP", "32"))


def _stats_work(stats, cout: int):
    if stats is None or STATS_REP < 2:
        return None
    return torch.zeros(STATS_REP, cout, 5, dtype=torch.float64, device=stats.device)


def cconv2d(x: Planar, wfrag, bias, cout: int, *, transposed=False, causal=True, slope=None, skip: Optional[Planar] = None,
            skip_div: int = 1, stats: Optional[torch.Tensor] = None, out: Optional[Planar] = None,
            wfrag_bf16: Optional[torch.Tensor] = None, image: str = "", adjoint_time: bool = False, gauss=None,
            addend: Optional[Planar] = None, addend_div: int = 1):
    Fout = 2 * x.F - 1 if transposed else (x.F - 1) // 2 + 1
    if causal:
        t_out = x.T
    else:
        t_out = x.T + 1 if transposed else x.T - 1
    tshift = -1 if (causal or transposed) else 0
    if adjoint_time:
        assert transposed and causal
        tshift = 0
    if out is None and image != "only":
        out = Planar.empty(cout, Fout, x.B, t_out, x.Tp, x.buf.device)
    c1 = skip.C if skip is not None else 0
    if image:
        assert stats is None and skip_div == 1 and wfrag_bf16 is None
        img = Image.empty(cout, Fout, x.B, t_out, x.Tp, x.buf.device)
        call("idv_cconv2d_fwd_img", x.ptr(), i(x.C), skip.ptr() if skip is not None else p(None), i(c1),
             i(skip.Jp if skip is not None else 0), p(wfrag), p(bias), p(slope), out.ptr() if out is not None else p(None),
             img.ptr(), ll(img.lo_off), i(1 if transposed else 0), i(tshift), i(cout), i(x.F), i(x.B), i(x.Tp), i(x.Jp),
             i(t_out), stream_ptr())
        return out, img
    if LAUNCH_LOG is not None:
        cfg = L.lib().idv_cconv_config(i(1 if transposed else 0), i(x.C + c1), i(cout), i(x.F))
        pos = x.B * x.T * (x.F if transposed else Fout)
        macs = 4 * (x.C + c1) * cout * 10 * pos
        ev0, ev1 = torch.cuda.Event(enable_timing=True), torch.cuda.Event(enable_timing=True)
        ev0.record()
    if wfrag_bf16 is not None:
        if LAUNCH_LOG is not None:
            cfg = -(1000000 + L.lib().idv_cconv_bf16_config(i(1 if transposed else 0), i(cout), i(x.F)))
        swork = _stats_work(stats, cout)
        call("idv_cconv2d_bf16x3_fwd", x.ptr(), i(x.C), skip.ptr() if skip is not None else p(None), i(c1),
             i(skip.Jp if skip is not None else 0), i(skip_div), p(wfrag_bf16), p(bias), p(slope), out.ptr(), p(stats), p(swork),
             i(STATS_REP), i(1 if transposed else 0), i(tshift), i(cout), i(x.F), i(x.B), i(x.Tp), i(x.Jp), i(t_out), stream_ptr())
        if LAUNCH_LOG is not None:
            ev1.record()
            LAUNCH_LOG.append((cfg, macs, ev0, ev1))
        return out
    if transposed and skip_div == 1 and _tw_ok(gauss, x, c1, cout, skip.Jp if skip is not None else None):
        if LAUNCH_LOG is not None:
            cfg = TW_CFG + (1 if tshift else 0)
        swork = _stats_work(stats, cout)
        _sync_tw_pair()
        call("idv_ctconv2d_tw_fwd", x.ptr(), i(x.C), skip.ptr() if skip is not None else p(None), i(c1), p(gauss[4]), p(gauss[1]),
             i(gauss[2]), p(slope), out.ptr(), p(stats), p(swork), i(STATS_REP), i(tshift), i(cout), i(x.F), i(x.B), i(x.Tp), i(x.Jp),
             i(t_out), addend.ptr() if addend is not None else p(None), i(addend_div), i(addend.Jp if addend is not None else 0),
             stream_ptr())
    elif not transposed and addend is None and _tw2_ok(gauss, x, c1, cout):
        if LAUNCH_LOG is not None:
            cfg = TW_CFG + 2 + (1 if tshift else 0)
        swork = _stats_work(stats, cout)
        _sync_tw_pair()
        call("idv_cconv2d_tw_fwd", x.ptr(), i(x.C), p(gauss[4]), p(gauss[1]), i(gauss[2]), p(slope), out.ptr(), p(stats), p(swork),
             i(STATS_REP), i(tshift), i(cout), i(x.F), i(x.B), i(x.Tp), i(x.Jp), i(t_out), stream_ptr())
    elif skip_div == 1 and _wino_ok(gauss, transposed, x, c1, cout, skip.Jp if skip is not None else None):
        if LAUNCH_LOG is not None:
            cfg = WINO_CFG + (1000 if transposed else 0) + L.lib().idv_cconv_wino_config(i(1 if transposed else 0), i(x.C + c1), i(cout))
        swork = _stats_work(stats, cout)
        call("idv_cconv2d_wino_fwd", x.ptr(), i(x.C), skip.ptr() if skip is not None else p(None), i(c1), p(gauss[3]), p(gauss[1]),
             i(gauss[2]), p(slope), out.ptr(), p(stats), p(swork), i(STATS_REP), i(1 if transposed else 0), i(tshift), i(cout), i(x.F),
             i(x.B), i(x.Tp), i(x.Jp), i(t_out), addend.ptr() if addend is not None else p(None), i(addend_div),
             i(addend.Jp if addend is not None else 0), stream_ptr())
    elif gauss is not None:
        if LAUNCH_LOG is not None:
            cfg = L.lib().idv_cconv_gauss_config(i(1 if transposed else 0), i(x.C + c1), i(cout), i(x.F))
        swork = _stats_work(stats, cout)
        call("idv_cconv2d_gauss_fwd", x.ptr(), i(x.C), skip.ptr() if skip is not None else p(None), i(c1),
             i(skip.Jp if skip is not None else 0), i(skip_div), p(gauss[0]), p(gauss[1]), i(gauss[2]), p(slope), out.ptr(),
             p(stats), p(swork), i(STATS_REP), i(1 if transposed else 0), i(tshift), i(cout), i(x.F), i(x.B), i(x.Tp), i(x.Jp), i(t_out),
             addend.ptr() if addend is not None else p(None), i(addend_div), i(addend.Jp if addend is not None else 0), stream_ptr())
    else:
        swork = _stats_work(stats, cout)
        call("idv_cconv2d_fwd", x.ptr(), i(x.C), skip.ptr() if skip is not None else p(None), i(c1),
             i(skip.Jp if skip is not None else 0), i(skip_div), p(wfrag), p(bias), p(slope), out.ptr(), p(stats), p(swork),
             i(STATS_REP), i(1 if transposed else 0), i(tshift), i(cout), i(x.F), i(x.B), i(x.Tp), i(x.Jp), i(t_out), stream_ptr())
    if LAUNCH_LOG is not None:
        ev1.record()
        LAUNCH_LOG.append((cfg, macs, ev0, ev1))
    return out


def cconv2d_img(x, wfrag_bf16, bias, cout: int, *, transposed=False, causal=True, slope=None, skip=None,
                want_planar=False, want_image=True, adjoint=False):
    src_img = isinstance(x, Image)
    if skip is not None and isinstance(skip, Image) != src_img:
        raise RuntimeError("cconv2d_img: x and skip must have the same format")
    Fout = 2 * x.F - 1 if transposed else (x.F - 1) // 2 + 1
    t_out = x.T if causal else (x.T + 1 if transposed else x.T - 1)
    tshift = -1 if (causal or transposed) else 0
    if adjoint:
        assert causal
        tshift, t_out = 0, x.T
    dev = x.buf.device
    outp = Planar.empty(cout, Fout, x.B, t_out, x.Tp, dev) if want_planar else None
    outi = Image.empty(cout, Fout, x.B, t_out, x.Tp, dev) if want_image else None
    c1 = skip.C if skip is not None else 0
    if LAUNCH_LOG is not None:
        cfg = -(100000000 + L.lib().idv_cconv_img_config(i(1 if src_img else 0), i(1 if transposed else 0), i(x.C + c1),
                                                          i(cout), i(x.F)))
        pos = x.B * x.T * (x.F if transposed else Fout)
        macs = 4 * (x.C + c1) * cout * 10 * pos
        ev0, ev1 = torch.cuda.Event(enable_timing=True), torch.cuda.Event(enable_timing=True)
        ev0.record()
    call("idv_cconv2d_img_fwd", i(1 if src_img else 0), x.ptr(), ll(x.lo_slots if src_img else 0), i(x.C),
         skip.ptr() if skip is not None else p(None), ll(skip.lo_slots if (skip is not None and src_img) else 0), i(c1),
         p(wfrag_bf16), p(bias), p(slope), outp.ptr() if outp is not None else p(None),
         outi.ptr() if outi is not None else p(None), ll(outi.lo_off if outi is not None else 0),
         i(1 if transposed else 0), i(tshift), i(cout), i(x.F), i(x.B), i(x.Tp), i(x.Jp), i(t_out), stream_ptr())
    if LAUNCH_LOG is not None:
        ev1.record()
        LAUNCH_LOG.append((cfg, macs, ev0, ev1))
    return outp, outi


def cconv2d_img_train(x: Image, wfrag_bf16, bias, cout: int, stats, *, transposed=False, skip: Optional[Image] = None) -> Planar:
    Fout = 2 * x.F - 1 if transposed else (x.F - 1) // 2 + 1
    out = Planar.empty(cout, Fout, x.B, x.T, x.Tp, x.buf.device)
    c1 = skip.C if skip is not None else 0
    if LAUNCH_LOG is not None:
        cfg = -(100000000 + L.lib().idv_cconv_img_config(i(1), i(1 if transposed else 0), i(x.C + c1), i(cout), i(x.F)))
        macs = 4 * (x.C + c1) * cout * 10 * x.B * x.T * (x.F if transposed else Fout)
        ev0, ev1 = torch.cuda.Event(enable_timing=True), torch.cuda.Event(enable_timing=True)
        ev0.record()
    swork = _stats_work(stats, cout)
    call("idv_cconv2d_img_train_fwd", x.ptr(), ll(x.lo_slots), i(x.C), skip.ptr() if skip is not None else p(None),
         ll(skip.lo_slots if skip is not None else 0), i(c1), p(wfrag_bf16), p(bias), out.ptr(), p(stats), p(swork), i(STATS_REP),
         i(1 if transposed else 0), i(cout), i(x.F), i(x.B), i(x.Tp), i(x.Jp), i(x.T), stream_ptr())
    if LAUNCH_LOG is not None:
        ev1.record()
        LAUNCH_LOG.append((cfg, macs, ev0, ev1))
    return out


def pw_gemm(x_ptr, K: int, wfrag, bias, M: int, B: int, Tp: int, Jp: int, t_valid: int, out_ptr, *, slope=None,
            swap=False, ldo=0):
    call("idv_pw_gemm", x_ptr, i(K), p(wfrag), p(bias), p(slope), out_ptr, i(M), i(B), i(Tp), i(Jp), i(t_valid),
         i(1 if swap else 0), i(ldo), stream_ptr())


def pack_lstm(sd_get, H: int, K: int, layer: int, device):
    g = lambda n: sd_get(n).contiguous()
    l = layer
    M = 8 * H
    mt = mtiles_alloc(M)
    ks = (K + 7) // 8 * 4
    wih = torch.empty(mt * ks * 64, dtype=torch.float32, device=device)
    bih = torch.empty(mt * 32, dtype=torch.float32, device=device)
    call("idv_pack_lstm_ih", p(g(f"lstm_re.weight_ih_l{l}")), p(g(f"lstm_re.bias_ih_l{l}")), p(g(f"lstm_re.bias_hh_l{l}")),
         p(g(f"lstm_im.weight_ih_l{l}")), p(g(f"lstm_im.bias_ih_l{l}")), p(g(f"lstm_im.bias_hh_l{l}")), i(H), i(K),
         p(wih), p(bih), stream_ptr())
    whh = torch.empty(4 * 4 * H * H, dtype=torch.float32, device=device)
    call("idv_pack_lstm_hh", p(g(f"lstm_re.weight_hh_l{l}")), p(g(f"lstm_im.weight_hh_l{l}")), i(H), p(whh), stream_ptr())
    wih16 = None
    if L.lib().idv_lstm_proj_bf16_supported(i(H), i(K)) and (layer == 0 or (4 * H) % 256 == 0):
        L.lib().idv_lstm_ih_bf16_bytes.restype = L._L
        wih16 = torch.empty(int(L.lib().idv_lstm_ih_bf16_bytes(i(H), i(K))), dtype=torch.uint8, device=device)
        call("idv_pack_lstm_ih_bf16", p(g(f"lstm_re.weight_ih_l{l}")), p(g(f"lstm_im.weight_ih_l{l}")), i(H), i(K), p(wih16),
             stream_ptr())
    wih_hh = None
    if layer == 1 and K == H and H == 128:
        wih_hh = torch.empty(4 * 4 * H * H, dtype=torch.float32, device=device)
        call("idv_pack_lstm_hh", p(g(f"lstm_re.weight_ih_l{l}")), p(g(f"lstm_im.weight_ih_l{l}")), i(H), p(wih_hh), stream_ptr())
    return wih, bih, whh, wih16, wih_hh


LSTM_PERSISTENT = os.environ.get("IDV_LSTM_PERSISTENT", "1") != "0"
LSTM_STACK2 = os.environ.get("IDV_LSTM_STACK2", "1") != "0"


def clstm(x: Planar, packed0, packed1, H: int) -> Planar:
    K = x.C * x.F
    out = Planar.empty(H, 1, x.B, x.T, x.Tp, x.buf.device)
    nwork = L.lib().idv_clstm_work_floats(i(H), i(x.B), i(x.T), i(x.Jp))
    work = torch.empty(bucket(int(nwork)), dtype=torch.float32, device=x.buf.device)
    flags = 1 if PRECISION == "bf16x3" else 0
    if not LSTM_PERSISTENT:
        flags |= 8
    if (flags & 1) and packed0[3] is not None:
        kimg = KImage.from_planes(x.ptr(), 2 * K, x.B * x.Tp, x.Jp, x.buf.device)
        call("idv_lstm_proj_bf16x3", kimg.ptr(), ll(kimg.lo_slots), i(K), p(packed0[3]), p(packed0[1]), p(work), i(H), i(x.B),
             i(x.T), i(x.Tp), i(x.Jp), stream_ptr())
        flags |= 2
    call("idv_clstm_fwd2", x.ptr(), i(K), p(packed0[0]), p(packed0[1]), p(packed0[2]), p(packed1[0]), p(packed1[1]),
         p(packed1[2]), p(packed1[4] if (LSTM_STACK2 and len(packed1) > 4) else None), i(H), i(x.B), i(x.T), i(x.Tp), i(x.Jp), p(work), out.ptr(),
         i(flags), p(packed1[3] if (flags & 1) else None), stream_ptr())
    return out


def cdense(x: Planar, packed_r, packed_i, M: int, C_out: int, F_out: int) -> Planar:
    K = x.C * x.F
    out = Planar.empty(C_out, F_out, x.B, x.T, x.Tp, x.buf.device)
    if PRECISION == "bf16x3" and K % 64 == 0 and len(packed_r) > 2 and packed_r[2] is not None:
        kimg = KImage.from_planes(x.ptr(), 2 * K, x.B * x.Tp, x.Jp, x.buf.device)
        for ri, pk in enumerate((packed_r, packed_i)):
            pw_bf16x3(kimg, ri * K // 8, K, pk[2], pk[1], M, x.B, x.Tp, x.T, out.ptr(ri * C_out))
        return out
    for ri, pk in enumerate((packed_r, packed_i)):
        pw_gemm(x.ptr(ri * x.C), K, pk[0], pk[1], M, x.B, x.Tp, x.Jp, x.T, out.ptr(ri * C_out))
    return out


class DftPlan:

    def __init__(self, n_fft, win, hop, T, device):
        self.n_fft, self.win, self.hop, self.T = n_fft, win, hop, T
        self.F = n_fft // 2 + 1
        F = self.F
        w_fwd = torch.empty(2 * F, win, dtype=torch.float32, device=device)
        w_inv = torch.empty(win, 2 * F, dtype=torch.float32, device=device)
        self.env_inv = torch.empty(n_fft + hop * (T - 1), dtype=torch.float32, device=device)
        call("idv_make_dft", i(n_fft), i(win), i(hop), i(T), p(w_fwd), p(w_inv), p(self.env_inv), stream_ptr())
        self.fwd = pack_pw(w_fwd, None)
        self.inv = pack_pw(w_inv, None)
        self.fwd16 = pack_pw_bf16(w_fwd)
        self.inv16 = pack_pw_bf16(w_inv)
        self._w_fwd, self._w_inv = w_fwd, w_inv
        self._fwd_T = self._inv_T = None

    def fwd_T(self):
        if self._fwd_T is None:
            self._fwd_T = pack_pw(self._w_fwd.t().contiguous(), None)
        return self._fwd_T

    def inv_T(self):
        if self._inv_T is None:
            self._inv_T = pack_pw(self._w_inv.t().contiguous(), None)
        return self._inv_T


def check_lengths(lengths, B: int, L: int, n_fft: Optional[int]) -> list:
    if isinstance(lengths, Lengths):
        lengths = lengths.host
    if isinstance(lengths, torch.Tensor):
        if lengths.is_cuda:
            raise ValueError("lengths must be a python sequence or a CPU integer tensor: they size the batch on the host, and "
                             "a GPU tensor would have to be fetched with a synchronisation")
        if lengths.dim() != 1 or lengths.is_floating_point() or lengths.is_complex() or lengths.dtype == torch.bool:
            raise ValueError("lengths must be a 1-D integer tensor")
        lengths = lengths.tolist()
    elif isinstance(lengths, (str, bytes)) or not isinstance(lengths, Sequence):
        raise ValueError("lengths must be a python sequence or a CPU integer tensor")
    if any(isinstance(v, bool) or not isinstance(v, int) for v in lengths):
        raise ValueError("lengths must be integers (sample counts)")
    if len(lengths) != B:
        raise ValueError(f"{len(lengths)} lengths for a batch of {B} utterances")
    for b, v in enumerate(lengths):
        if n_fft is None and v <= 0:
            raise ValueError(f"lengths[{b}] = {v}: a length must be positive")
        if n_fft is not None and v <= n_fft // 2:
            raise ValueError(f"lengths[{b}] = {v}: torch.stft's reflect padding needs more than n_fft/2 = {n_fft // 2} samples")
        if v > L:
            raise ValueError(f"lengths[{b}] = {v} exceeds the {L} samples per row of the padded batch")
    return list(lengths)


class Lengths:

    __slots__ = ("host", "dev")

    def __init__(self, host, device, dev=None):
        self.host = list(host)
        self.dev = torch.tensor(self.host, dtype=torch.int32, device=device) if dev is None else dev

    def __len__(self):
        return len(self.host)

    def part(self, b0: int, b1: int) -> "Lengths":
        return Lengths(self.host[b0:b1], None, self.dev[b0:b1])

    def outputs(self, hop: int) -> "Lengths":
        return Lengths([hop * (v // hop) for v in self.host], self.dev.device)


def _ragged_rows(x: torch.Tensor) -> torch.Tensor:
    if x.dtype != torch.float32 or x.stride(1) != 1 or x.stride(0) < x.shape[1]:
        x = x.float().contiguous()
    return x


def stft(x: torch.Tensor, plan: DftPlan, Tp: Optional[int] = None, lengths=None) -> Planar:
    if lengths is not None:
        return _stft_ragged(x, plan, Tp, lengths)
    B, Lx = x.shape
    T = 1 + Lx // plan.hop
    assert T == plan.T, "DftPlan built for another length"
    Tp = Tp or T + 1
    x = x.contiguous()
    if PRECISION == "bf16x3":
        Jp = Planar.jp_for(B, Tp)
        kimg = KImage((plan.win + 63) // 64 * 64, Jp, x.device)
        call("idv_stft_frames_kimage", p(x), i(B), i(Lx), i(plan.n_fft), i(plan.win), i(plan.hop), i(T), kimg.ptr(),
             ll(kimg.lo_off), i(Tp), i(Jp), stream_ptr())
        out = Planar.empty(1, plan.F, B, T, Tp, x.device)
        pw_bf16x3(kimg, 0, plan.win, plan.fwd16, None, 2 * plan.F, B, Tp, T, out.ptr())
        return out
    fr = Planar.empty(1, plan.win // 2, B, T, Tp, x.device)
    assert plan.win % 2 == 0
    call("idv_stft_frames", p(x), i(B), i(Lx), i(plan.n_fft), i(plan.win), i(plan.hop), i(T), fr.ptr(), i(Tp), i(fr.Jp),
         stream_ptr())
    out = Planar.empty(1, plan.F, B, T, Tp, x.device)
    pw_gemm(fr.ptr(), plan.win, plan.fwd[0], plan.fwd[1], 2 * plan.F, B, Tp, fr.Jp, T, out.ptr())
    return out


def _stft_ragged(x: torch.Tensor, plan: DftPlan, Tp: Optional[int], lengths) -> Planar:
    B, Lx = x.shape
    T = 1 + Lx // plan.hop
    assert T == plan.T, "DftPlan built for another length"
    host = check_lengths(lengths, B, Lx, plan.n_fft)
    if not isinstance(lengths, Lengths):
        lengths = Lengths(host, x.device)
    Tp = Tp or T + 1
    x = _ragged_rows(x)
    assert plan.win % 2 == 0
    out = Planar.empty(1, plan.F, B, T, Tp, x.device)
    out.lengths = lengths
    if PRECISION == "bf16x3":
        kimg = KImage((plan.win + 63) // 64 * 64, out.Jp, x.device)
        call("idv_stft_frames_kimage_ragged", p(x), ll(x.stride(0)), p(lengths.dev), i(B), i(plan.n_fft), i(plan.win), i(plan.hop),
             i(T), kimg.ptr(), ll(kimg.lo_off), i(Tp), i(out.Jp), stream_ptr())
        pw_bf16x3(kimg, 0, plan.win, plan.fwd16, None, 2 * plan.F, B, Tp, T, out.ptr())
        return out
    fr = Planar.empty(1, plan.win // 2, B, T, Tp, x.device)
    call("idv_stft_frames_ragged", p(x), ll(x.stride(0)), p(lengths.dev), i(B), i(plan.n_fft), i(plan.win), i(plan.hop), i(T),
         fr.ptr(), i(Tp), i(fr.Jp), stream_ptr())
    pw_gemm(fr.ptr(), plan.win, plan.fwd[0], plan.fwd[1], 2 * plan.F, B, Tp, fr.Jp, T, out.ptr())
    return out


def istft(spec: Planar, plan: DftPlan, lengths=None) -> torch.Tensor:
    B, T = spec.B, spec.T
    if lengths is not None:
        nl = len(lengths)
        if nl < 1 or B % nl:
            raise ValueError(f"{nl} lengths for {B} rows: the row count must be a multiple of the number of lengths")
        if not isinstance(lengths, Lengths):
            lengths = Lengths(check_lengths(lengths, nl, plan.hop * T + plan.hop - 1, plan.n_fft), spec.buf.device)
        if max(lengths.host) // plan.hop + 1 > T:
            raise ValueError("a length needs more frames than the spectrum holds")
    fr = Planar.empty(1, plan.win // 2, B, T, spec.Tp, spec.buf.device)
    if PRECISION == "bf16x3":
        kimg = KImage.from_planes(spec.ptr(), 2 * plan.F, B * spec.Tp, spec.Jp, spec.buf.device, pad_to=64)
        pw_bf16x3(kimg, 0, 2 * plan.F, plan.inv16, None, plan.win, B, spec.Tp, T, fr.ptr())
    else:
        pw_gemm(spec.ptr(), 2 * plan.F, plan.inv[0], plan.inv[1], plan.win, B, spec.Tp, spec.Jp, T, fr.ptr())
    y = torch.empty(B, plan.hop * (T - 1), dtype=torch.float32, device=spec.buf.device)
    if lengths is not None:
        call("idv_istft_ola_ragged", fr.ptr(), p(lengths.dev), i(B // len(lengths)), i(B), i(plan.n_fft), i(plan.win), i(plan.hop),
             i(T), i(spec.Tp), i(fr.Jp), p(y), ll(y.stride(0)), stream_ptr())
        return y
    call("idv_istft_ola", fr.ptr(), p(plan.env_inv), i(B), i(plan.n_fft), i(plan.win), i(plan.hop), i(T), i(spec.Tp),
         i(fr.Jp), p(y), stream_ptr())
    return y


def mask_apply(mask: Planar, X: Planar, x_div: int = 1):
    B, F, T = mask.B, mask.F, mask.T
    pred = Planar.empty(1, F, B, T, mask.Tp, mask.buf.device)
    pc = torch.empty(B, F, T, 2, dtype=torch.float32, device=mask.buf.device)
    call("idv_mask_apply", mask.ptr(), X.ptr(), i(x_div), i(X.Jp), pred.ptr(), p(pc), i(F), i(B), i(T), i(mask.Tp),
         i(mask.Jp), stream_ptr())
    return pred, torch.view_as_complex(pc)


def msd(a: Planar, ca0: int, b: Planar, cb0: int, C: int) -> torch.Tensor:
    work = torch.empty(3, dtype=torch.float64, device=a.buf.device)
    out = torch.empty(1, dtype=torch.float32, device=a.buf.device)
    call("idv_msd", a.ptr(), i(a.C), i(ca0), i(a.Jp), b.ptr(), i(b.C), i(cb0), i(b.Jp), i(C), i(a.F), i(a.B), i(a.Tp), i(a.T),
         p(work), p(out), stream_ptr())
    return out[0]


def planar_to_complex(act: Planar) -> torch.Tensor:
    pc = torch.empty(act.B, act.F, act.T, 2, dtype=torch.float32, device=act.buf.device)
    call("idv_planar_to_complex", act.ptr(), p(pc), i(act.F), i(act.B), i(act.T), i(act.Tp), i(act.Jp), stream_ptr())
    return torch.view_as_complex(pc)


def cbn_train(act: Planar, stats: torch.Tensor, bn, slope, first_call: bool, momentum: float = 0.9):
    C = act.C
    dev = act.buf.device
    moments = torch.empty(5, C, dtype=torch.float32, device=dev)
    fold = torch.empty(C, 6, dtype=torch.float32, device=dev)
    count = float(act.B) * act.F * act.T
    if BN_SYNC is not None:
        count = count * BN_SYNC(stats)
    call("idv_cbn_finalize", p(stats), d(count), p(bn.gamma_rr), p(bn.gamma_ri), p(bn.gamma_ii), p(bn.beta_r), p(bn.beta_i),
         i(C), i(1 if first_call else 0), f(momentum), p(bn.running_mean_real), p(bn.running_mean_imag), p(bn.Vrr), p(bn.Vri),
         p(bn.Vii), p(moments), p(fold), stream_ptr())
    call("idv_cbn_apply_prelu", act.ptr(), p(fold), p(slope), i(C), i(act.F), i(act.B), i(act.Tp), i(act.Jp), i(act.T),
         stream_ptr())
    return moments


def reparam(lat: Planar, off, zdim: int, eps_r, eps_i, ns: int) -> Planar:
    B, T = lat.B, lat.T
    z = Planar.empty(zdim, 1, B * ns, T, lat.Tp, lat.buf.device)
    call("idv_reparam", lat.ptr(), i(lat.C), i(off[0]), i(off[1]), i(off[2]), i(zdim), p(eps_r.contiguous()),
         p(eps_i.contiguous()), i(ns), i(B), i(T), i(lat.Tp), i(lat.Jp), z.ptr(), i(z.Jp), stream_ptr())
    return z


def check_dev_f32(t: torch.Tensor, name: str, device=None):
    if not isinstance(t, torch.Tensor) or not t.is_cuda:
        raise L.IdvError(f"{name}: expected a CUDA (ROCm) tensor, got {type(t).__name__} on "
                         f"{getattr(t, 'device', '?')}; the HIP hot path has no CPU fallback")
    if device is not None and t.device != torch.device(device):
        raise L.IdvError(f"{name}: on {t.device}, expected {device}")


def sisnr(source: torch.Tensor, est: torch.Tensor, src_div: int = 1) -> torch.Tensor:
    B, Ln = est.shape
    check_dev_f32(source, "source", est.device)
    if source.dtype != torch.float32 or est.dtype != torch.float32 or source.shape[-1] < Ln:
        raise L.IdvError("sisnr: float32 tensors with source length >= estimate length expected")
    assert source.stride(-1) == 1 and est.stride(-1) == 1
    work = torch.empty(3 * B, dtype=torch.float64, device=est.device)
    out = torch.empty(1, dtype=torch.float32, device=est.device)
    call("idv_sisnr", p(source), i(source.stride(0)), i(src_div), p(est), i(est.stride(0)), i(B), i(Ln), p(work), p(out),
         stream_ptr())
    return out[0]


def recon_loss(pred_c: torch.Tensor, ori: torch.Tensor, ori_div: int = 1):
    pr = torch.view_as_real(pred_c)
    assert pr.is_contiguous()
    check_dev_f32(ori, "ori_cpx_stft", pr.device)
    if ori.dtype != torch.float32:
        raise L.IdvError("recon_loss: float32 STFT expected")
    B, F, T, _ = pr.shape
    if tuple(ori.shape[1:]) != (F, T, 2):
        raise L.IdvError(f"recon_loss: STFT shape {tuple(ori.shape)} does not match the prediction {tuple(pr.shape)}")
    work = torch.empty(3, dtype=torch.float64, device=pr.device)
    out = torch.empty(2, dtype=torch.float32, device=pr.device)
    sb, sf, st, sr = ori.stride()
    call("idv_recon_loss", p(pr), p(ori), ll(sb), ll(sf), ll(st), ll(sr), i(ori_div), i(B), i(F), i(T), p(work), p(out),
         stream_ptr())
    return out[0], out[1]


def ckl(q1: Planar, off1, q2: Optional[Planar], off2, zdim: int, eps: float) -> torch.Tensor:
    work = torch.empty(3, dtype=torch.float64, device=q1.buf.device)
    out = torch.empty(1, dtype=torch.float32, device=q1.buf.device)
    o2 = off2 if q2 is not None else (0, 0, 0)
    call("idv_ckl", q1.ptr(), i(q1.C), i(q1.Jp), i(off1[0]), i(off1[1]), i(off1[2]),
         q2.ptr() if q2 is not None else p(None), i(q2.C if q2 is not None else 0), i(q2.Jp if q2 is not None else 0),
         i(o2[0]), i(o2[1]), i(o2[2]), i(zdim), f(eps), i(q1.B), i(q1.T), i(q1.Tp), p(work), p(out), stream_ptr())
    return out[0]


def mi_estimate(lat: Planar, off, z: Planar, zdim: int, ns: int, eps: float):
    lib = L.lib()
    lib.idv_mi_work_floats.restype = L._L
    if (z.C, z.B, z.T, z.Tp) != (zdim, lat.B * ns, lat.T, lat.Tp):
        raise ValueError(f"mutual_information: samples {(z.C, z.B, z.T)} do not belong to a posterior {(zdim, lat.B, lat.T)} x {ns}")
    work = torch.empty(int(lib.idv_mi_work_floats(i(lat.B), i(ns), i(lat.T), i(zdim))), dtype=torch.float32, device=lat.buf.device)
    acc = torch.empty(1, dtype=torch.float64, device=lat.buf.device)
    out = torch.empty(1, dtype=torch.float32, device=lat.buf.device)
    call("idv_mi_fwd", lat.ptr(), i(lat.C), i(lat.Jp), i(off[0]), i(off[1]), i(off[2]), z.ptr(), i(z.Jp), i(zdim), i(ns), i(lat.B),
         i(lat.T), i(lat.Tp), f(eps), p(work), p(acc), p(out), stream_ptr())
    return out[0], work


def mi_bwd(lat: Planar, off, z: Planar, zdim: int, ns: int, eps: float, work, gout, dlat: Optional[Planar], dz: Optional[Planar]):
    call("idv_mi_bwd", lat.ptr(), i(lat.C), i(lat.Jp), i(off[0]), i(off[1]), i(off[2]), z.ptr(), i(z.Jp), i(zdim), i(ns), i(lat.B),
         i(lat.T), i(lat.Tp), f(eps), p(work), p(gout), dlat.ptr() if dlat is not None else p(None),
         dz.ptr() if dz is not None else p(None), stream_ptr())


def miu_dist(q1: Planar, off1: int, q2: Planar, off2: int, zdim: int) -> torch.Tensor:
    work = torch.empty(3 * 2 * zdim, dtype=torch.float64, device=q1.buf.device)
    out = torch.empty(1, dtype=torch.float32, device=q1.buf.device)
    call("idv_miu_dist", q1.ptr(), i(q1.C), i(q1.Jp), i(off1), q2.ptr(), i(q2.C), i(q2.Jp), i(off2), i(zdim), i(q1.B), i(q1.T),
         i(q1.Tp), p(work), p(out), stream_ptr())
    return out[0]


def cbn_stats(act: Planar) -> torch.Tensor:
    stats = torch.zeros(act.C, 5, dtype=torch.float64, device=act.buf.device)
    call("idv_cbn_stats", act.ptr(), i(act.C), i(act.F), i(act.B), i(act.Tp), i(act.Jp), i(act.T), p(stats), stream_ptr())
    return stats


def cbn_apply(act: Planar, fold: torch.Tensor, slope=None):
    call("idv_cbn_apply_prelu", act.ptr(), p(fold), p(slope), i(act.C), i(act.F), i(act.B), i(act.Tp), i(act.Jp), i(act.T),
         stream_ptr())
    return act


_LL = L._L


def _ll_fn(name):
    fn = getattr(L.lib(), name)
    fn.restype = _LL
    return fn


def like(x: Planar, C: Optional[int] = None, F: Optional[int] = None, zero=False) -> Planar:
    return Planar.empty(x.C if C is None else C, x.F if F is None else F, x.B, x.T, x.Tp, x.buf.device, zero=zero)


def rewrap(buf: torch.Tensor, x: Planar, C: Optional[int] = None, F: Optional[int] = None) -> Planar:
    return Planar(buf, x.C if C is None else C, x.F if F is None else F, x.B, x.T, x.Tp, x.Jp)


def pack_cconv_adjoint(w_re, w_im, cout: int, cin_total: int, cin_used: int, transposed: bool):
    cck = L.lib().idv_cconv_cck(cin_used)
    ccp = (2 * cin_used + cck - 1) // cck * cck
    mt = mtiles_alloc(2 * cout)
    wfrag = torch.empty(mt * ccp * 5 * 64, dtype=torch.float32, device=w_re.device)
    bias = torch.empty(mt * 32, dtype=torch.float32, device=w_re.device)
    call("idv_pack_cconv_adjoint", p(w_re), p(w_im), i(cout), i(cin_total), i(cin_used), i(1 if transposed else 0), p(wfrag),
         p(bias), stream_ptr())
    return wfrag, bias


def pack_cconv_bf16_adjoint(w_re, w_im, cout: int, cin_total: int, cin_used: int, transposed: bool):
    L.lib().idv_cconv_bf16_wfrag_bytes.restype = L._L
    wfrag = torch.empty(int(L.lib().idv_cconv_bf16_wfrag_bytes(i(cout), i(cin_used))), dtype=torch.uint8, device=w_re.device)
    call("idv_pack_cconv_bf16_adjoint", p(w_re), p(w_im), i(cout), i(cin_total), i(cin_used), i(1 if transposed else 0),
         p(wfrag), stream_ptr())
    return wfrag


_ZBIAS = {}


def zero_bias(cout: int, device):
    key = (mtiles_alloc(2 * cout), str(device))
    if key not in _ZBIAS:
        _ZBIAS[key] = torch.zeros(key[0] * 32, dtype=torch.float32, device=device)
        torch.cuda.current_stream(device).synchronize()
    return _ZBIAS[key]


def cconv_dgrad(dy: Planar, wfrag, bias, cout_adj: int, fwd_transposed: bool, causal: bool, wfrag_bf16=None, gauss=None) -> Planar:
    adj_transposed = not fwd_transposed
    Fout = 2 * dy.F - 1 if adj_transposed else (dy.F - 1) // 2 + 1
    if causal:
        tshift_adj, t_out = 0, dy.T
    elif adj_transposed:
        tshift_adj, t_out = -1, dy.T + 1
    else:
        tshift_adj, t_out = 0, dy.T - 1
    if t_out + 1 > dy.Tp:
        raise RuntimeError("cconv_dgrad: the input of the block had more frames than the buffer's columns per utterance")
    out = Planar.empty(cout_adj, Fout, dy.B, t_out, dy.Tp, dy.buf.device)
    if LAUNCH_LOG is not None:
        cfg = L.lib().idv_cconv_config(i(1 if adj_transposed else 0), i(dy.C), i(cout_adj), i(dy.F))
        macs = 4 * dy.C * cout_adj * 10 * dy.B * dy.T * (dy.F if adj_transposed else Fout)
        ev0, ev1 = torch.cuda.Event(enable_timing=True), torch.cuda.Event(enable_timing=True)
        if wfrag_bf16 is not None:
            cfg = -(1000000 + L.lib().idv_cconv_bf16_config(i(1 if adj_transposed else 0), i(cout_adj), i(dy.F)))
        ev0.record()
    if wfrag_bf16 is None and adj_transposed and _tw_ok(gauss, dy, 0, cout_adj, None):
        if LAUNCH_LOG is not None:
            cfg = TW_CFG + (1 if tshift_adj else 0)
        _sync_tw_pair()
        call("idv_ctconv2d_tw_fwd", dy.ptr(), i(dy.C), p(None), i(0), p(gauss[4]), p(gauss[1]), i(0), p(None), out.ptr(), p(None), p(None),
             i(0), i(tshift_adj), i(cout_adj), i(dy.F), i(dy.B), i(dy.Tp), i(dy.Jp), i(t_out), p(None), i(1), i(0), stream_ptr())
    elif wfrag_bf16 is None and not adj_transposed and _tw2_ok(gauss, dy, 0, cout_adj):
        if LAUNCH_LOG is not None:
            cfg = TW_CFG + 2 + (1 if tshift_adj else 0)
        _sync_tw_pair()
        call("idv_cconv2d_tw_fwd", dy.ptr(), i(dy.C), p(gauss[4]), p(gauss[1]), i(0), p(None), out.ptr(), p(None), p(None), i(0),
             i(tshift_adj), i(cout_adj), i(dy.F), i(dy.B), i(dy.Tp), i(dy.Jp), i(t_out), stream_ptr())
    elif wfrag_bf16 is None and _wino_ok(gauss, adj_transposed, dy, 0, cout_adj, None):
        if LAUNCH_LOG is not None:
            cfg = WINO_CFG + (1000 if adj_transposed else 0) + L.lib().idv_cconv_wino_config(i(1 if adj_transposed else 0), i(dy.C), i(cout_adj))
        call("idv_cconv2d_wino_fwd", dy.ptr(), i(dy.C), p(None), i(0), p(gauss[3]), p(gauss[1]), i(0), p(None), out.ptr(), p(None), p(None),
             i(0), i(1 if adj_transposed else 0), i(tshift_adj), i(cout_adj), i(dy.F), i(dy.B), i(dy.Tp), i(dy.Jp), i(t_out), p(None), i(1),
             i(0), stream_ptr())
    elif gauss is not None and wfrag_bf16 is None:
        if LAUNCH_LOG is not None:
            cfg = L.lib().idv_cconv_gauss_config(i(1 if adj_transposed else 0), i(dy.C), i(cout_adj), i(dy.F))
        call("idv_cconv2d_gauss_fwd", dy.ptr(), i(dy.C), p(None), i(0), i(0), i(1), p(gauss[0]), p(gauss[1]), i(0), p(None),
             out.ptr(), p(None), p(None), i(0), i(1 if adj_transposed else 0), i(tshift_adj), i(cout_adj), i(dy.F), i(dy.B), i(dy.Tp),
             i(dy.Jp), i(t_out), p(None), i(1), i(0), stream_ptr())
    elif wfrag_bf16 is not None:
        call("idv_cconv2d_bf16x3_fwd", dy.ptr(), i(dy.C), p(None), i(0), i(0), i(1), p(wfrag_bf16), p(bias), p(None), out.ptr(), p(None),
             p(None), i(0), i(1 if adj_transposed else 0), i(tshift_adj), i(cout_adj), i(dy.F), i(dy.B), i(dy.Tp), i(dy.Jp), i(t_out),
             stream_ptr())
    else:
        call("idv_cconv2d_fwd", dy.ptr(), i(dy.C), p(None), i(0), i(0), i(1), p(wfrag), p(bias), p(None), out.ptr(), p(None), p(None),
             i(0), i(1 if adj_transposed else 0), i(tshift_adj), i(cout_adj), i(dy.F), i(dy.B), i(dy.Tp), i(dy.Jp), i(t_out), stream_ptr())
    if LAUNCH_LOG is not None:
        ev1.record()
        LAUNCH_LOG.append((cfg, macs, ev0, ev1))
    return out


_WORK = {}
WGRAD_BF16_CFG = -96
WGRAD_BF16 = os.environ.get("IDV_WGRAD_BF16", "1") != "0"
WGRAD_GAUSS_CFG = -95
WGRAD_CFG = -97


def _scratch(n: int, device, tag="w") -> torch.Tensor:
    key = (str(device), torch.cuda.current_stream().cuda_stream, tag)
    t = _WORK.get(key)
    if t is None or t.numel() < n:
        t = torch.empty(bucket(n), dtype=torch.float32, device=device)
        _WORK[key] = t
    return t


def cconv_wgrad(x: Planar, ci_off: int, dy: Planar, cout: int, cin_total: int, transposed: bool, causal: bool, dw_re, dw_im):
    tshift = -1 if (causal or transposed) else 0
    cs, cl = (x.C, cout) if transposed else (cout, x.C)
    bf16 = PRECISION == "bf16x3" and WGRAD_BF16 and 2 * cs >= 32 and 2 * cl >= 32
    gauss = not bf16 and bool(L.lib().idv_cconv_wgrad_gauss_supported(i(cs), i(cl)))
    if gauss:
        n = int(_ll_fn("idv_cconv_wgrad_gauss_work_floats")(i(x.C), i(cout), i(1 if transposed else 0), i(x.F), i(x.B), i(x.Tp),
                                                            i(x.Jp), i(dy.Jp)))
    else:
        n = int(_ll_fn("idv_cconv_wgrad_bf16_work_floats" if bf16 else "idv_cconv_wgrad_work_floats")(i(cs), i(cl), i(x.B), i(x.Tp)))
    work = _scratch(n, x.buf.device)
    if LAUNCH_LOG is not None:
        macs = 4 * x.C * cout * 10 * x.B * x.T * (x.F if transposed else dy.F)
        ev0, ev1 = torch.cuda.Event(enable_timing=True), torch.cuda.Event(enable_timing=True)
        ev0.record()
    call("idv_cconv2d_bwd_weight_bf16x3" if bf16 else ("idv_cconv2d_bwd_weight_gauss" if gauss else "idv_cconv2d_bwd_weight"),
         x.ptr(), i(x.C), i(ci_off), dy.ptr(), i(cout), i(cin_total), i(1 if transposed else 0),
         i(tshift), i(x.F), i(x.B), i(x.Tp), i(x.Jp), i(dy.Jp), p(work), ll(work.numel()), p(dw_re), p(dw_im), stream_ptr())
    if LAUNCH_LOG is not None:
        ev1.record()
        LAUNCH_LOG.append((WGRAD_BF16_CFG if bf16 else (WGRAD_GAUSS_CFG if gauss else WGRAD_CFG), macs, ev0, ev1))


def cconv_bias_grad(dy: Planar):
    stats = cbn_stats(dy)
    db_re = torch.empty(dy.C, dtype=torch.float32, device=dy.buf.device)
    db_im = torch.empty_like(db_re)
    call("idv_cconv2d_bwd_bias", p(stats), i(dy.C), p(db_re), p(db_im), stream_ptr())
    return db_re, db_im


def train_image_ok(C: int) -> bool:
    return PRECISION == "bf16x3" and IMAGE_TRAIN and C % 8 == 0 and 2 * C >= 64


def cbn_apply_to(y: Planar, fold, slope, want_image: bool = False):
    out = like(y)
    if want_image:
        img = Image.empty(y.C, y.F, y.B, y.T, y.Tp, y.buf.device)
        call("idv_cbn_apply_prelu_to_img", y.ptr(), p(fold), p(slope), i(y.C), i(y.F), i(y.B), i(y.Tp), i(y.Jp), i(y.T), out.ptr(),
             img.ptr(), ll(img.lo_off), stream_ptr())
        return out, img
    call("idv_cbn_apply_prelu_to", y.ptr(), p(fold), p(slope), i(y.C), i(y.F), i(y.B), i(y.Tp), i(y.Jp), i(y.T), out.ptr(),
         stream_ptr())
    return out


BN_SYNC = None


def cbn_bwd(dz: Planar, y: Planar, fold, moments, bn, slope, count: float, want_image: bool = False):
    C, dev = y.C, y.buf.device
    sums = torch.empty(C, 8, dtype=torch.float64, device=dev)
    call("idv_cbn_bwd_reduce", dz.ptr(), y.ptr(), p(fold), p(slope), i(C), i(y.F), i(y.B), i(y.Tp), i(y.Jp), i(y.T), p(sums),
         stream_ptr())
    world = 1
    if BN_SYNC is not None:
        world = BN_SYNC(sums)
        count = count * world
    coef = torch.empty(C, 12, dtype=torch.float32, device=dev)
    g = [torch.empty(C, dtype=torch.float32, device=dev) for _ in range(5)]
    dslope = torch.zeros(1, dtype=torch.float32, device=dev)
    call("idv_cbn_bwd_finalize", p(sums), d(count), p(moments), p(bn[0]), p(bn[1]), p(bn[2]), i(C), p(coef), p(g[0]), p(g[1]),
         p(g[2]), p(g[3]), p(g[4]), p(dslope if slope is not None else None), f(1.0 / world), stream_ptr())
    dy = like(y)
    if want_image:
        img = Image.empty(y.C, y.F, y.B, y.T, y.Tp, dev)
        call("idv_cbn_bwd_apply_img", dz.ptr(), y.ptr(), p(fold), p(coef), p(slope), i(C), i(y.F), i(y.B), i(y.Tp), i(y.Jp), i(y.T),
             dy.ptr(), img.ptr(), ll(img.lo_off), stream_ptr())
        return ((dy, img), *g, dslope)
    call("idv_cbn_bwd_apply", dz.ptr(), y.ptr(), p(fold), p(coef), p(slope), i(C), i(y.F), i(y.B), i(y.Tp), i(y.Jp), i(y.T),
         dy.ptr(), stream_ptr())
    return (dy, *g, dslope)


def cbn_finalize(stats, count: float, bn_mod, first_call: bool, momentum: float, update_running: bool = True):
    C = bn_mod.C
    dev = stats.device
    if BN_SYNC is not None:
        count = count * BN_SYNC(stats)
    moments = torch.empty(5, C, dtype=torch.float32, device=dev)
    fold = torch.empty(C, 6, dtype=torch.float32, device=dev)
    rb = (bn_mod.running_mean_real, bn_mod.running_mean_imag, bn_mod.Vrr, bn_mod.Vri, bn_mod.Vii) if update_running else (None,) * 5
    call("idv_cbn_finalize", p(stats), d(count), p(bn_mod.gamma_rr), p(bn_mod.gamma_ri), p(bn_mod.gamma_ii), p(bn_mod.beta_r),
         p(bn_mod.beta_i), i(C), i(1 if first_call else 0), f(momentum), p(rb[0]), p(rb[1]), p(rb[2]), p(rb[3]), p(rb[4]),
         p(moments), p(fold), stream_ptr())
    return moments, fold


def pw_wgrad(dout_ptr, M: int, Jp_d: int, x_ptr, K: int, Jp_x: int, J: int, dw: torch.Tensor, *, shift=0, rowmap=0, H=0,
             accumulate=False):
    n = int(_ll_fn("idv_pw_wgrad_work_floats")(i(M), i(K), i(J)))
    work = _scratch(n, dw.device)
    bf16 = PRECISION == "bf16x3" and WGRAD_BF16 and M >= 64 and K >= 64
    call("idv_pw_bwd_weight_bf16x3" if bf16 else "idv_pw_bwd_weight", dout_ptr, i(M), i(Jp_d), x_ptr, i(K), i(Jp_x), i(J), i(shift), p(work), ll(work.numel()), p(dw),
         i(dw.stride(0)), i(rowmap), i(H), i(1 if accumulate else 0), stream_ptr())


def planar_rowsum(x_ptr, M: int, Jp: int, J: int, out: torch.Tensor, accumulate=False):
    call("idv_planar_rowsum", x_ptr, i(M), i(Jp), i(J), i(1 if accumulate else 0), p(out), stream_ptr())


def mask_apply_bwd(mask: Planar, X: Planar, x_div: int, dpred: Optional[Planar], dpred_c, want_dx: bool = False):
    dm = like(mask)
    dX = like(X) if want_dx else None
    call("idv_mask_apply_bwd", mask.ptr(), X.ptr(), i(x_div), i(X.Jp), dpred.ptr() if dpred is not None else p(None),
         p(dpred_c), i(mask.F), i(mask.B), i(mask.T), i(mask.Tp), i(mask.Jp), dm.ptr(), dX.ptr() if dX is not None else p(None),
         stream_ptr())
    return dm, dX


def complex_to_planar(xc: torch.Tensor, Tp: Optional[int] = None) -> Planar:
    B, F, T, _ = xc.shape
    out = Planar.empty(1, F, B, T, Tp or T + 1, xc.device)
    call("idv_complex_to_planar", p(xc.contiguous()), out.ptr(), i(F), i(B), i(T), i(out.Tp), i(out.Jp), stream_ptr())
    return out


def istft_bwd(dy: torch.Tensor, spec: Planar, plan: "DftPlan") -> Planar:
    B, T = spec.B, spec.T
    dfr = Planar.empty(1, plan.win // 2, B, T, spec.Tp, dy.device)
    call("idv_istft_ola_bwd", p(dy.contiguous()), p(plan.env_inv), i(B), i(plan.n_fft), i(plan.win), i(plan.hop), i(T),
         i(spec.Tp), i(dfr.Jp), dfr.ptr(), stream_ptr())
    out = like(spec)
    wT = plan.inv_T()
    pw_gemm(dfr.ptr(), plan.win, wT[0], wT[1], 2 * plan.F, B, spec.Tp, dfr.Jp, T, out.ptr())
    return out


def stft_bwd(dX: Planar, plan: "DftPlan", Lx: int) -> torch.Tensor:
    B, T = dX.B, dX.T
    dfr = Planar.empty(1, plan.win // 2, B, T, dX.Tp, dX.buf.device)
    wT = plan.fwd_T()
    pw_gemm(dX.ptr(), 2 * plan.F, wT[0], wT[1], plan.win, B, dX.Tp, dX.Jp, T, dfr.ptr())
    dx = torch.empty(B, Lx, dtype=torch.float32, device=dX.buf.device)
    call("idv_stft_frames_bwd", dfr.ptr(), i(B), i(Lx), i(plan.n_fft), i(plan.win), i(plan.hop), i(T), i(dX.Tp), i(dfr.Jp),
         p(dx), stream_ptr())
    return dx


def reparam_bwd(lat: Planar, off, zdim: int, eps_r, eps_i, ns: int, dz: Planar, dlat: Planar):
    call("idv_reparam_bwd", lat.ptr(), i(lat.C), i(off[0]), i(off[1]), i(off[2]), i(zdim), p(eps_r), p(eps_i), i(ns), i(lat.B),
         i(lat.T), i(lat.Tp), i(lat.Jp), dz.ptr(), i(dz.Jp), dlat.ptr(), stream_ptr())
```

include/idccrn_hip.h:

```cpp
#ifndef IDCCRN_HIP_H
#define IDCCRN_HIP_H

#ifdef __cplusplus
extern "C" {
#endif

#define IDV_ABI_VERSION 9
#define IDV_SLACK_FLOATS 256

int idv_abi_version(void);

int idv_coop_last_status(int clear);
int idv_coop_max_workgroups(void);


int idv_cconv_cck(int cin_used);
int idv_cconv_config(int transposed, int cin_used, int Cout, int Fin);

int idv_cbn_fold(const float* moments, const float* gamma_rr, const float* gamma_ri, const float* gamma_ii,
                 const float* beta_r, const float* beta_i, int C, float* fold, void* stream);

int idv_pack_cconv(const float* w_re, const float* w_im, const float* b_re, const float* b_im, const float* fold,
                   int Cout, int Cin_total, int Cin_used, int transposed, float* wfrag, float* bias_out, void* stream);

int idv_pack_pw(const float* w, const float* bias, int M, int K, float* wfrag, float* bias_out, void* stream);

int idv_pack_lstm_ih(const float* w_ih_re, const float* b_ih_re, const float* b_hh_re, const float* w_ih_im,
                     const float* b_ih_im, const float* b_hh_im, int H, int K, float* wfrag, float* bias_out,
                     void* stream);
int idv_pack_lstm_hh(const float* w_hh_re, const float* w_hh_im, int H, float* whh_frag, void* stream);

int idv_make_dft(int n_fft, int win, int hop, int T, float* w_fwd, float* w_inv, float* env_inv, void* stream);


int idv_cconv2d_fwd(const float* x0, int C0, const float* x1, int C1, int Jp1, int x1_div, const float* wfrag,
                    const float* bias, const float* prelu_slope, float* out, double* stats, double* stats_work, int stats_rep,
                    int transposed, int tshift, int Cout, int Fin, int B, int Tp, int Jp, int t_valid_out, void* stream);

int idv_cconv_gauss_supported(int C0, int C1, int Cout);
long long idv_cconv_gauss_wfrag_floats(int Cout, int cin_used);
int idv_cconv_gauss_epi_rows(int Cout);
int idv_cconv_gauss_config(int transposed, int Cin, int Cout, int Fin);
int idv_pack_cconv_gauss(const float* w_re, const float* w_im, const float* b_re, const float* b_im, const float* fold, int Cout,
                         int Cin_total, int Cin_used, int transposed, int conj, float* wfrag, float* epi, void* stream);
int idv_cconv2d_gauss_fwd(const float* x0, int C0, const float* x1, int C1, int Jp1, int x1_div, const float* wfrag,
                          const float* epi, int has_fold, const float* prelu_slope, float* out, double* stats, double* stats_work,
                          int stats_rep, int transposed, int tshift, int Cout, int Fin, int B, int Tp, int Jp, int t_valid_out,
                          const float* addend, int addend_div, int addend_Jp, void* stream);

long long idv_cconv_bf16_wfrag_bytes(int Cout, int cin_used);
int idv_cconv_bf16_supported(int transposed, int C0, int C1, int x1_div, int Cout);
int idv_cconv_bf16_config(int transposed, int Cout, int Fin);
int idv_pack_cconv_bf16(const float* w_re, const float* w_im, const float* fold, int Cout, int Cin_total, int Cin_used,
                        int transposed, void* wfrag, void* stream);
int idv_cconv2d_bf16x3_fwd(const float* x0, int C0, const float* x1, int C1, int Jp1, int x1_div, const void* wfrag_bf16,
                           const float* bias, const float* prelu_slope, float* out, double* stats, double* stats_work,
                           int stats_rep, int transposed, int tshift, int Cout, int Fin, int B, int Tp, int Jp, int t_valid_out,
                           void* stream);

int idv_cconv2d_fwd_img(const float* x0, int C0, const float* x1, int C1, int Jp1, const float* wfrag, const float* bias,
                        const float* prelu_slope, float* out_planar, void* out_img, long long out_lo_off_elems,
                        int transposed, int tshift, int Cout, int Fin, int B, int Tp, int Jp, int t_valid_out,
                        void* stream);
int idv_cconv2d_img_train_fwd(const void* x0_img, long long lo_off0, int C0, const void* x1_img, long long lo_off1, int C1,
                              const void* wfrag_bf16, const float* bias, float* out_planar, double* stats, double* stats_work,
                              int stats_rep, int transposed, int Cout, int Fin, int B, int Tp, int Jp, int t_valid_out, void* stream);
int idv_cconv_img_config(int src_is_image, int transposed, int Cin, int Cout, int Fin);
int idv_planar_to_image(const float* x, int C, int F, int J, int Jp, void* img, long long lo_off_elems, void* stream);
int idv_planar_to_image_repeat(const float* x, int C, int F, int B, int Tp, int Jp_in, int rep, void* img, long long lo_off_elems,
                               int Jp, void* stream);
int idv_image_to_planar(const void* img, long long lo_off_elems, int C, int F, int J, int Jp, float* x, void* stream);
int idv_cconv2d_img_fwd(int src_is_image , const void* x0_img, long long lo_off0_slots, int C0, const void* x1_img, long long lo_off1_slots,
                        int C1, const void* wfrag_bf16, const float* bias, const float* prelu_slope, float* out_planar,
                        void* out_img, long long out_lo_off_elems, int transposed, int tshift,
                        int Cout, int Fin, int B, int Tp, int Jp, int t_valid_out, void* stream);

long long idv_ctconv_c1_wfrag_bytes(int cin_used);
int idv_pack_ctconv_c1_bf16(const float* w_re, const float* w_im, const float* fold, int Cin_total, int Cin_used,
                            void* wfrag, void* stream);
int idv_ctconv_c1_bf16x3_fwd(const float* x0, int C0, const float* x1, int C1, int Jp1, const void* wfrag,
                             const float* bias, const float* prelu_slope, float* out, int Fin, int B, int Tp, int Jp,
                             int t_valid_out, void* stream);
int idv_ctconv_c1_img_fwd(const void* x0_img, long long lo_off0_slots, int C0, const void* x1_img, long long lo_off1_slots,
                          int C1, const void* wfrag, const float* bias, const float* prelu_slope, float* out, int Fin, int B,
                          int Tp, int Jp, int t_valid_out, void* stream);

int idv_pw_gemm(const float* x, int K, const float* wfrag, const float* bias, const float* prelu_slope, float* out,
                int M, int B, int Tp, int Jp, int t_valid, int swap, int ldo, void* stream);

int idv_cbn_finalize(const double* stats, double count, const float* gamma_rr, const float* gamma_ri,
                     const float* gamma_ii, const float* beta_r, const float* beta_i, int C, int first_call,
                     float momentum, float* running_mean_r, float* running_mean_i, float* Vrr, float* Vri,
                     float* Vii, float* moments, float* fold, void* stream);
int idv_cbn_stats(const float* act, int C, int F, int B, int Tp, int Jp, int t_valid, double* stats, void* stream);
int idv_cbn_apply_prelu(float* act, const float* fold, const float* prelu_slope, int C, int F, int B, int Tp, int Jp,
                        int t_valid, void* stream);

int idv_stft_frames(const float* x, int B, int L, int n_fft, int win, int hop, int T, float* frames, int Tp, int Jp,
                    void* stream);
int idv_istft_ola(const float* frames, const float* env_inv, int B, int n_fft, int win, int hop, int T, int Tp,
                  int Jp, float* y, void* stream);

int idv_mask_apply(const float* mask, const float* X, int x_div, int JpX, float* pred, float* pred_c, int F, int B,
                   int T, int Tp, int Jp, void* stream);
int idv_datanorm(const float* X, const float* mean, const float* stdv, int F, int B, int T, int Tp, int Jp, float* out, void* stream);
int idv_datadenorm(const float* P, const float* mean, const float* stdv, int F, int B, int T, int Tp, int Jp, float* out,
                   float* out_c, void* stream);
int idv_datanorm_bwd(const float* dout, const float* stdv, int F, int B, int T, int Tp, int Jp, float* dX, void* stream);
int idv_datadenorm_bwd(const float* dout, const float* dout_c, const float* stdv, int F, int B, int T, int Tp, int Jp, float* dP,
                       void* stream);
int idv_outtype_estimate(const float* speech_c, const float* noise_c, const float* X, long long sb, long long sf, long long st,
                         long long sr, int mode, int ns, int B, int F, int T, int Tp, int Jp, float* out, float* out_c,
                         void* stream);
int idv_planar_to_complex(const float* act, float* out_c, int F, int B, int T, int Tp, int Jp, void* stream);

long long idv_clstm_work_floats(int H, int B, int T, int Jp);
int idv_lstm_pers_supported(int H, int B);
long long idv_lstm_pers_work_bytes(int H, int B);
int idv_lstm_rec_pers(const float* g, long long g_run_z, long long g_run_s, int ldg, const float* whh_frag, float* hout, int H,
                      int B, int T, void* work, void* kimg, long long kimg_lo_slots, int Tp, int Jp, float* gsave, float* csave,
                      void* stream);
int idv_lstm_proj1_bf16x3(const void* himg, long long lo_off_slots, const void* wfrag_bf16, const float* bias, float* G1, int H,
                          int B, int T, int Tp, int Jp, void* stream);
int idv_lstm_coop_f32_supported(int H, int B);
long long idv_lstm_coop_f32_work_bytes(int H, int B);
int idv_lstm_rec_coop_f32(const float* g, long long g_run_z, long long g_run_s, int ldg, const float* whh_frag, float* hout, int H,
                          int B, int T, void* work, float* gsave, float* csave, void* stream);
int idv_lstm_pers_f32_supported(int H, int B);
long long idv_lstm_pers_f32_work_bytes(int H, int B);
int idv_lstm_rec_pers_f32(const float* g, long long g_run_z, long long g_run_s, int ldg, const float* whh_frag, float* hout, int H,
                          int B, int T, void* work, float* gsave, float* csave, void* stream);
void idv_lstm_pers_set_profile(unsigned long long* prof_cycles);
long long idv_clstm_train_work_floats(int H, int B, int T, int Jp);
int idv_clstm_fwd(const float* x, int K, const float* wih0, const float* bih0, const float* whh0, const float* wih1,
                  const float* bih1, const float* whh1, int H, int B, int T, int Tp, int Jp, float* work, float* out,
                  int flags, const void* wih1_bf16, void* stream);

int idv_lstm_stack2_f32_supported(int H, int B);
long long idv_lstm_stack2_f32_work_bytes(int H, int B);
int idv_lstm_stack2_f32(const float* g, long long g_run_z, long long g_run_s, int ldg, const float* whh0, const float* wih1_hh,
                        const float* whh1, const float* bias1, float* h0, float* hout, int H, int B, int T, void* work,
                        float* gsave1, float* csave0, float* csave1, void* stream);
int idv_clstm_fwd2(const float* x, int K, const float* wih0, const float* bih0, const float* whh0, const float* wih1,
                   const float* bih1, const float* whh1, const float* wih1_hh, int H, int B, int T, int Tp, int Jp, float* work,
                   float* out, int flags, const void* wih1_bf16, void* stream);

long long idv_lstm_ih_bf16_bytes(int H, int K);
int idv_lstm_proj_bf16_supported(int H, int K);
int idv_pack_lstm_ih_bf16(const float* w_ih_re, const float* w_ih_im, int H, int K, void* wfrag, void* stream);
int idv_planar_to_kimage(const float* x, int nvalid, int nplanes, int J, int Jp, void* img, long long lo_off_elems, void* stream);
int idv_pw_bf16x3_rows(const void* ximg, long long lo_off_slots, int K, const void* wfrag_bf16, const float* bias, float* out_rows,
                       int M, int ldo, int B, int T, int Tp, int Jp, void* stream);
long long idv_pw_bf16_wfrag_bytes(int M, int K);
int idv_pack_pw_bf16(const float* w, int M, int K, void* wfrag, void* stream);
int idv_pw_bf16x3(const void* ximg, long long lo_off_slots, int K, const void* wfrag_bf16, const float* bias, float* out, int M,
                  int B, int Tp, int Jp, int t_valid, void* stream);
int idv_stft_frames_kimage(const float* x, int B, int L, int n_fft, int win, int hop, int T, void* img, long long lo_off_elems,
                           int Tp, int Jp, void* stream);
int idv_lstm_proj_bf16x3(const void* ximg, long long lo_off_slots, int K, const void* wfrag_bf16, const float* bias, float* G,
                         int H, int B, int T, int Tp, int Jp, void* stream);

int idv_reparam(const float* lat, int Hl, int off_miu, int off_ls, int off_dl, int zdim, const float* eps_r,
                const float* eps_i, int ns, int B, int T, int Tp, int Jp, float* z, int Jpz, void* stream);


int idv_sisnr(const float* source, int src_ld, int src_div, const float* est, int est_ld, int B, int L, double* work,
              float* out, void* stream);
int idv_sisdr(const float* ref, int ref_ld, const float* est, int est_ld, int B, int L, double* work, float* out, void* stream);
int idv_mean_over_samples(const float* x, int ns, int B, int L, float* out, void* stream);
int idv_recon_loss(const float* pred_c, const float* ori, long long sb, long long sf, long long st, long long sr,
                   int ori_div, int B, int F, int T, double* work, float* out, void* stream);
int idv_ckl(const float* q1, int H1, int Jp1, int o1_miu, int o1_ls, int o1_dl, const float* q2, int H2, int Jp2,
            int o2_miu, int o2_ls, int o2_dl, int zdim, float eps, int B, int T, int Tp, double* work, float* out,
            void* stream);
int idv_msd(const float* a, int Ca, int ca0, int JpA, const float* b, int Cb, int cb0, int JpB, int C, int F, int B, int Tp,
            int t_valid, double* work, float* out, void* stream);
long long idv_mi_work_floats(int B, int ns, int T, int zdim);
int idv_mi_fwd(const float* lat, int H, int Jp, int o_miu, int o_ls, int o_dl, const float* z, int Jpz, int zdim, int ns, int B,
               int T, int Tp, float eps, float* work, double* acc, float* out, void* stream);
int idv_mi_bwd(const float* lat, int H, int Jp, int o_miu, int o_ls, int o_dl, const float* z, int Jpz, int zdim, int ns, int B,
               int T, int Tp, float eps, const float* work, const float* gout, float* dlat, float* dz, void* stream);
int idv_miu_dist(const float* q1, int H1, int Jp1, int off1, const float* q2, int H2, int Jp2, int off2, int zdim,
                 int B, int T, int Tp, double* work, float* out, void* stream);


int idv_pack_cconv_adjoint(const float* w_re, const float* w_im, int Cout, int Cin_total, int Cin_used, int transposed,
                           float* wfrag, float* bias_out, void* stream);
int idv_pack_cconv_bf16_adjoint(const float* w_re, const float* w_im, int Cout, int Cin_total, int Cin_used, int transposed,
                                void* wfrag, void* stream);

long long idv_cconv_wgrad_work_floats(int Cs, int Cl, int B, int Tp);
int idv_cconv2d_bwd_weight(const float* x, int Cx, int ci_off, const float* dy, int Cout, int Cin_total, int transposed,
                           int tshift, int Fin, int B, int Tp, int Jp_x, int Jp_dy, float* work, long long work_floats,
                           float* dw_re, float* dw_im, void* stream);
long long idv_cconv_wgrad_bf16_work_floats(int Cs, int Cl, int B, int Tp);
int idv_cconv2d_bwd_weight_bf16x3(const float* x, int Cx, int ci_off, const float* dy, int Cout, int Cin_total, int transposed,
                                  int tshift, int Fin, int B, int Tp, int Jp_x, int Jp_dy, float* work, long long work_floats,
                                  float* dw_re, float* dw_im, void* stream);
int idv_cconv_wgrad_gauss_supported(int Cs, int Cl);
long long idv_cconv_wgrad_gauss_work_floats(int Cx, int Cout, int transposed, int Fin, int B, int Tp, int Jp_x, int Jp_dy);
int idv_cconv2d_bwd_weight_gauss(const float* x, int Cx, int ci_off, const float* dy, int Cout, int Cin_total, int transposed,
                                 int tshift, int Fin, int B, int Tp, int Jp_x, int Jp_dy, float* work, long long work_floats,
                                 float* dw_re, float* dw_im, void* stream);
int idv_cconv2d_bwd_bias(const double* stats_dy, int Cout, float* db_re, float* db_im, void* stream);

long long idv_pw_wgrad_work_floats(int M, int K, int J);
int idv_pw_bwd_weight(const float* dout, int M, int Jp_d, const float* x, int K, int Jp_x, int J, int shift, float* work,
                      long long work_floats, float* dw, int ldw, int rowmap, int H, int accumulate, void* stream);
int idv_pw_bwd_weight_bf16x3(const float* dout, int M, int Jp_d, const float* x, int K, int Jp_x, int J, int shift, float* work,
                             long long work_floats, float* dw, int ldw, int rowmap, int H, int accumulate, void* stream);
int idv_planar_rowsum(const float* x, int M, int Jp, int J, int accumulate, float* out, void* stream);

int idv_cbn_apply_prelu_to(const float* y, const float* fold, const float* prelu_slope, int C, int F, int B, int Tp, int Jp,
                           int t_valid, float* out, void* stream);
int idv_cbn_bwd_reduce(const float* dz, const float* y, const float* fold, const float* prelu_slope, int C, int F, int B,
                       int Tp, int Jp, int t_valid, double* sums, void* stream);
int idv_cbn_bwd_finalize(const double* sums, double count, const float* moments, const float* gamma_rr, const float* gamma_ri,
                         const float* gamma_ii, int C, float* coef, float* dgamma_rr, float* dgamma_ri, float* dgamma_ii,
                         float* dbeta_r, float* dbeta_i, float* dslope, float param_grad_scale, void* stream);
int idv_cbn_bwd_apply(const float* dz, const float* y, const float* fold, const float* coef, const float* prelu_slope, int C,
                      int F, int B, int Tp, int Jp, int t_valid, float* dy, void* stream);
int idv_cbn_apply_prelu_to_img(const float* y, const float* fold, const float* prelu_slope, int C, int F, int B, int Tp, int Jp,
                               int t_valid, float* out, void* img, long long lo_off_elems, void* stream);
int idv_cbn_bwd_apply_img(const float* dz, const float* y, const float* fold, const float* coef, const float* prelu_slope, int C,
                          int F, int B, int Tp, int Jp, int t_valid, float* dy, void* img, long long lo_off_elems, void* stream);

int idv_mask_apply_bwd(const float* mask, const float* X, int x_div, int JpX, const float* dpred, const float* dpred_c, int F,
                       int B, int T, int Tp, int Jp, float* dmask, float* dX, void* stream);
int idv_repeat_batch_bwd(const float* drep, int n, int rows, int B, int Tp, int Jp_rep, int Jp, float* dx, void* stream);
int idv_complex_to_planar(const float* in_c, float* act, int F, int B, int T, int Tp, int Jp, void* stream);
int idv_istft_ola_bwd(const float* dy, const float* env_inv, int B, int n_fft, int win, int hop, int T, int Tp, int Jp,
                      float* dframes, void* stream);
int idv_stft_frames_bwd(const float* dframes, int B, int L, int n_fft, int win, int hop, int T, int Tp, int Jp, float* dx,
                        void* stream);
int idv_reparam_bwd(const float* lat, int Hl, int off_miu, int off_ls, int off_dl, int zdim, const float* eps_r,
                    const float* eps_i, int ns, int B, int T, int Tp, int Jp, const float* dz, int Jpz, float* dlat, void* stream);

int idv_sisnr_bwd(const float* source, int src_ld, int src_div, const float* est, int est_ld, int B, int L, const double* work,
                  const float* grad_out, float* dest, void* stream);
int idv_recon_loss_bwd(const float* pred_c, const float* ori, long long sb, long long sf, long long st, long long sr,
                       int ori_div, int B, int F, int T, const float* g_cpx, const float* g_mag, float* dpred_c, void* stream);
int idv_ckl_bwd(const float* q1, int H1, int Jp1, int o1_miu, int o1_ls, int o1_dl, const float* q2, int H2, int Jp2,
                int o2_miu, int o2_ls, int o2_dl, int zdim, float eps, int B, int T, int Tp, const float* grad_out, float* dq1,
                void* stream);
int idv_miu_dist_bwd(const float* q1, int H1, int Jp1, int off1, const float* q2, int H2, int Jp2, int off2, int zdim, int B,
                     int T, int Tp, const float* grad_out, const float* loss_value, float* dq1, float* dq2, void* stream);

int idv_lstm_uncombine(const float* dout, int H, int B, int T, int Tp, int Jp, float* dh, void* stream);
int idv_pack_lstm_hh_bwd(const float* w_hh_re, const float* w_hh_im, int H, float* whhT, void* stream);
long long idv_lstm_bptt_work_floats(int H, int B);
int idv_lstm_bptt(float* gates, long long g_run_z, long long g_run_s, int ldg, const float* cstates, const float* dhout,
                  const float* whhT, int H, int B, int T, float* work, void* stream);
int idv_lstm_bptt_coop_supported(int H, int B);
int idv_lstm_bptt_stack2_supported(int H, int B);
long long idv_lstm_bptt_stack2_work_bytes(int H, int B);
int idv_lstm_bptt_stack2(float* g1, float* g0, long long g0_run_z, long long g0_run_s, int ldg0, const float* c1, const float* c0,
                         const float* dhout1, const float* whhT1, const float* wihT1, const float* whhT0, int H, int B, int T,
                         void* work, void* stream);
long long idv_lstm_bptt_coop_work_bytes(int H, int B);
int idv_lstm_bptt_coop(float* gates, long long g_run_z, long long g_run_s, int ldg, const float* cstates, const float* dhout,
                       const float* whhT, int H, int B, int T, void* work, void* stream);
int idv_rows_to_planar(const float* src, long long ld, int c0, int ncol, int B, int T, int Tp, int Jp, float* dst, void* stream);
int idv_lstm_bias_grad(const float* dGp, int H, int Jp, int J, int accumulate, float* db, void* stream);

int idv_bucket_gather(const long long* table, int n, long long total, float* flat, void* stream);
int idv_bucket_scatter(const long long* table, int n, long long total, const float* flat, float scale, void* stream);
int idv_bucket_adam(const long long* ptable, const long long* gtable, const float* gflat, float* exp_avg, float* exp_avg_sq,
                    int n, long long total, float lr, double beta1, double beta2, float eps, float weight_decay,
                    float bias_correction1, float bias_correction2_sqrt, float grad_scale, void* stream);

int idv_cconv_wino_supported(int transposed, int C0, int C1, int Cout, int Fin);
long long idv_cconv_wino_wfrag_floats(int transposed, int Cout, int cin_used);
int idv_cconv_wino_config(int transposed, int Cin, int Cout);
int idv_pack_cconv_wino(const float* w_re, const float* w_im, int Cout, int Cin_total, int Cin_used, int transposed, int conj,
                        float* wfrag, void* stream);
int idv_cconv2d_wino_fwd(const float* x0, int C0, const float* x1, int C1, const float* wfrag, const float* epi, int has_fold,
                         const float* prelu_slope, float* out, double* stats, double* stats_work, int stats_rep, int transposed,
                         int tshift, int Cout, int Fin, int B, int Tp, int Jp, int t_valid_out, const float* addend,
                         int addend_div, int addend_Jp, void* stream);

int idv_cconv_tw_supported(int C0, int C1, int Cout, int Fin);
long long idv_cconv_tw_wfrag_floats(int Cout, int cin_used);
int idv_pack_cconv_tw(const float* wino_frag, int Cout, int cin_used, float* tw_frag, void* stream);
int idv_ctconv2d_tw_fwd(const float* x0, int C0, const float* x1, int C1, const float* wfrag, const float* epi, int has_fold,
                        const float* prelu_slope, float* out, double* stats, double* stats_work, int stats_rep, int tshift,
                        int Cout, int Fin, int B, int Tp, int Jp, int t_valid_out, const float* addend, int addend_div,
                        int addend_Jp, void* stream);

int idv_cconv_tw2_supported(int Cin, int Cout, int Fin);
long long idv_cconv_tw2_wfrag_floats(int Cout, int cin_used);
int idv_pack_cconv_tw2(const float* wino_frag, int Cout, int cin_used, float* tw_frag, void* stream);
int idv_cconv2d_tw_fwd(const float* x0, int Cin, const float* wfrag, const float* epi, int has_fold, const float* prelu_slope,
                       float* out, double* stats, double* stats_work, int stats_rep, int tshift, int Cout, int Fin, int B, int Tp,
                       int Jp, int t_valid_out, void* stream);

long long idv_stream_cconv_wfloats(int Cin, int Cout);
int idv_stream_pack_cconv(const float* w_re, const float* w_im, const float* b_re, const float* b_im, int Cin, int Cout,
                          int transposed, float* w, float* bias, void* stream);
int idv_stream_cconv_splits(int transposed, int Cin, int Cout, int Fin, int B);
int idv_stream_cconv(const float* x0, const float* h0, int C0, const float* x1, const float* h1, int C1, const float* w,
                     const float* bias, const float* fold, const float* prelu_slope, float* out, float* hist_out, float* x0hist_out,
                     float* work, int nsplit, int transposed, int Cout, int Fin, int B, int k, int Tp, int Jp, void* stream);
int idv_stream_lstm_supported(int H);
int idv_stream_clstm(const float* G, const float* wt, const float* b1, float* state, float* hout, float* out, int H, int B, int k,
                     int Tp, int Jp, void* stream);
int idv_stream_frames(const float* ring, int R, const float* x, long long ldx, int n_new, long long n_prev, long long L_end, int B,
                      int n_fft, int win, int hop, long long t0, int k, float* frames, int Tp, int Jp, void* stream);
int idv_stream_ring(float* ring, int R, const float* x, long long ldx, int n_new, long long n_prev, int B, void* stream);
int idv_stream_ola(const float* frames, int Tp, int Jp, const float* carry_in, int carry_in_len, float* carry_out, int cap, int B,
                   int n_fft, int win, int hop, long long t0, int k, long long T_total, long long e0, long long e1, long long p_end,
                   float* y, int ldy, long long y_off, void* stream);

int idv_stft_frames_ragged(const float* x, long long ldx, const int* lens, int B, int n_fft, int win, int hop, int Tmax, float* frames,
                           int Tp, int Jp, void* stream);
int idv_stft_frames_kimage_ragged(const float* x, long long ldx, const int* lens, int B, int n_fft, int win, int hop, int Tmax, void* img,
                                  long long lo_off_elems, int Tp, int Jp, void* stream);
int idv_istft_ola_ragged(const float* frames, const int* lens, int len_div, int B, int n_fft, int win, int hop, int Tmax, int Tp, int Jp,
                         float* y, long long ldy, void* stream);
int idv_sisdr_ragged(const float* ref, int ref_ld, const float* est, int est_ld, const int* lens, int B, double* work, float* out,
                     void* stream);

#define IDV_TW_PAIR_T_EVEN 1
#define IDV_TW_PAIR_T_ODD 2
#define IDV_TW_PAIR_CONV 4
#define IDV_TW_PAIR_ALL 7
#define IDV_TW_PAIR_DEFAULT 7
int idv_tw_pair(int mask);
long long idv_tw_pair_launches(int reset);

#ifdef __cplusplus
}
#endif
#endif
```

Before: 955.4 utterances/sec.

## Handle odd-row frequency edge tiles with dedicated reduced-tap edge weights

For odd frequency row counts, the last padded frequency tile of the TW transposed conv and the TW2 forward conv previously ran the full Winograd-style tile over a mostly-padded row. This change splits those edge rows into separate edge blocks (or a separate EDGE kernel launch for TW2). The edge blocks use a specially packed weight fragment that carries only the taps that reach the last output row, and each one covers two column tiles. The aim is to stop spending full tile compute on padding. In exchange the weight buffers grow, packing needs extra kernels, and TW2 gets an extra launch.

```diff
diff --git a/i-dccrn-vae_amd/csrc/cgemm_tw.hip b/i-dccrn-vae_amd/csrc/cgemm_tw.hip
--- a/i-dccrn-vae_amd/csrc/cgemm_tw.hip
+++ b/i-dccrn-vae_amd/csrc/cgemm_tw.hip
@@ -29,6 +29,7 @@
     int xcd_split;
     int cgroups;
     int stagger;
+    int nmain;
 };
 
 constexpr int TW_PACK_CI = 8;
@@ -82,8 +83,14 @@
 
     const int bid = blockIdx.x;
     const int xcd = bid & 7, slot = bid >> 3;
+    const bool edge = PH == 0 && bid >= a.nmain;
     int jt, ft, ct;
-    if (a.xcd_split) {
+    if (PH == 0 && edge) {
+        const int eb = bid - a.nmain;
+        ct = eb % a.cgroups;
+        jt = 2 * (eb / a.cgroups);
+        ft = a.ftiles;
+    } else if (a.xcd_split) {
         const int G = 8 / a.cgroups;
         ct = xcd % a.cgroups;
         jt = (slot / a.ftiles) * G + xcd / a.cgroups;
@@ -100,6 +107,7 @@
     const int j0 = jt * 64;
     const int m0 = 2 * ft;
     const int rbase = m0 - 1 + ROW0;
+    const bool has_y = jt + 1 < a.jtiles;
 
     const int Cin = a.C0 + a.C1;
     const int nchunk = (Cin + CIK - 1) / CIK;
@@ -114,9 +122,9 @@
     int offA[UNI ? 1 : NPAIR + 1], offB[UNI ? 1 : NPAIR + 1];
     float cbj[UNI ? 1 : NPAIR + 1];
     if (UNI) {
-        cbj[0] = tw_cb<PH>(w4);
-        offA[0] = (tw_ra<PH>(w4) - ROW0) * 288;
-        offB[0] = (tw_rb<PH>(w4) - ROW0) * 288;
+        cbj[0] = edge ? 0.f : tw_cb<PH>(w4);
+        offA[0] = edge ? w4 * 288 : (tw_ra<PH>(w4) - ROW0) * 288;
+        offB[0] = edge ? w4 * 288 : (tw_rb<PH>(w4) - ROW0) * 288;
     } else {
 #pragma unroll
         for (int j = 0; j <= NPAIR; ++j) {
@@ -142,11 +150,11 @@
         const int c8 = e & 15;
         const int rl = (e >> 4) % NRAW, cl = e / (16 * NRAW);
         item_cl[i] = cl;
-        const int f = rbase + rl;
-        const int jc = j0 + 4 * c8;
+        const int f = edge ? rbase + (rl & 1) : rbase + rl;
+        const int jc = j0 + 4 * c8 + (edge ? 64 * (rl >> 1) : 0);
         const int je = LEFT ? jc - 1 : jc + 4;
         const bool exists = e < NITEM;
-        const bool okr = exists && f >= 0 && f < a.Fin;
+        const bool okr = exists && f >= 0 && f < a.Fin && !(edge && (rl >> 1) && !has_y);
         unsigned m = 0;
 #pragma unroll
         for (int q = 0; q < 5; ++q) {
@@ -227,7 +235,8 @@
     };
 
     constexpr int WS = tw_wslots<PH>();
-    const float* wbase = a.wfrag + ((size_t)(PH == 1 ? (size_t)a.cotiles * a.UP * tw_ntp<0>() : 0) + (size_t)ct * a.UP * NTP) * 64 +
+    const float* wbase = a.wfrag + ((size_t)(PH == 1 ? (size_t)a.cotiles * a.UP * tw_ntp<0>() : 0) +
+                                    (size_t)(edge ? (size_t)a.cotiles * a.UP * (tw_ntp<0>() + tw_ntp<1>()) : 0) + (size_t)ct * a.UP * NTP) * 64 +
                          (size_t)w4 * WS * 64;
     const int total_ks = nchunk * KS;
     float a_w[RDW][NTW];
@@ -319,16 +328,19 @@
     const bool has_act = a.slope != nullptr;
     float* E = smem + cth * (NT * 4 * 64);
     const int jA = j0 + 2 * l31;
-    bool keep[2], inb[2];
-    int ja[2];
-#pragma unroll
-    for (int q = 0; q < 2; ++q) {
-        const int j = jA + q;
-        const int bj = j / a.Tp, tp = j - bj * a.Tp;
-        inb[q] = j < a.J;
-        keep[q] = inb[q] && tp >= 1 && tp <= a.t_valid;
-        ja[q] = j - (bj - bj / a.add_div) * a.Tp;
-    }
+    constexpr int NCB = PH == 0 ? 2 : 1;
+    bool keep[NCB][2], inb[NCB][2];
+    int ja[NCB][2];
+#pragma unroll
+    for (int cbk = 0; cbk < NCB; ++cbk)
+#pragma unroll
+        for (int q = 0; q < 2; ++q) {
+            const int j = jA + 64 * cbk + q;
+            const int bj = j / a.Tp, tp = j - bj * a.Tp;
+            inb[cbk][q] = j < a.J;
+            keep[cbk][q] = inb[cbk][q] && tp >= 1 && tp <= a.t_valid;
+            ja[cbk][q] = j - (bj - bj / a.add_div) * a.Tp;
+        }
 #pragma unroll
     for (int s = 0; s < ((DBG & 4) ? 1 : 4); ++s) {
         if (s > 0) __syncthreads();
@@ -368,22 +380,34 @@
         float st[5] = {0.f, 0.f, 0.f, 0.f, 0.f};
 #pragma unroll
         for (int rt = 0; rt < 2; ++rt) {
-            const int fo = 2 * m0 + PH + 2 * rt;
-            if (fo >= a.Fout) continue;
+            const int fo = edge ? 2 * m0 : 2 * m0 + PH + 2 * rt;
+            if (fo >= a.Fout || (edge && rt == 1 && !has_y)) continue;
+            const bool second = PH == 0 && rt == 1 && edge;
+            bool kp[2], ib[2];
+            int jad[2];
+#pragma unroll
+            for (int q = 0; q < 2; ++q) {
+                kp[q] = second ? keep[NCB - 1][q] : keep[0][q];
+                ib[q] = second ? inb[NCB - 1][q] : inb[0][q];
+                jad[q] = second ? ja[NCB - 1][q] : ja[0][q];
+            }
             float yr[2], yi[2];
 #pragma unroll
             for (int q = 0; q < 2; ++q) {
                 float re, im;
-                if (PH == 0) {
+                if (PH == 0 && edge) {
+                    re = pr[PH == 0 ? 2 * rt : 0][q] + pr[PH == 0 ? 2 * rt + 1 : 0][q];
+                    im = pi[PH == 0 ? 2 * rt : 0][q] + pi[PH == 0 ? 2 * rt + 1 : 0][q];
+                } else if (PH == 0) {
                     re = rt == 0 ? pr[0][q] + pr[1][q] + pr[2][q] : pr[1][q] - pr[2][q] - pr[NR - 1][q];
                     im = rt == 0 ? pi[0][q] + pi[1][q] + pi[2][q] : pi[1][q] - pi[2][q] - pi[NR - 1][q];
                 } else {
                     re = rt == 0 ? pr[0][q] + pr[1][q] : pr[1][q] - pr[2][q];
                     im = rt == 0 ? pi[0][q] + pi[1][q] : pi[1][q] - pi[2][q];
                 }
-                if (a.add && cok && inb[q]) {
-                    re += a.add[((size_t)co * a.Fout + fo) * a.add_Jp + ja[q]];
-                    im += a.add[((size_t)(a.Cout + co) * a.Fout + fo) * a.add_Jp + ja[q]];
+                if (a.add && cok && ib[q]) {
+                    re += a.add[((size_t)co * a.Fout + fo) * a.add_Jp + jad[q]];
+                    im += a.add[((size_t)(a.Cout + co) * a.Fout + fo) * a.add_Jp + jad[q]];
                 }
                 float r_, i_;
                 if (a.has_fold) {
@@ -397,9 +421,9 @@
                     r_ = r_ >= 0.f ? r_ : slope * r_;
                     i_ = i_ >= 0.f ? i_ : slope * i_;
                 }
-                yr[q] = keep[q] ? r_ : 0.f;
-                yi[q] = keep[q] ? i_ : 0.f;
-                if (STATS && keep[q]) {
+                yr[q] = kp[q] ? r_ : 0.f;
+                yi[q] = kp[q] ? i_ : 0.f;
+                if (STATS && kp[q]) {
                     st[0] += yr[q];
                     st[1] += yi[q];
                     st[2] += yr[q] * yr[q];
@@ -408,12 +432,12 @@
                 }
             }
             if (cok) {
-                float* o_r = a.out + ((size_t)co * a.Fout + fo) * a.Jp + jA;
-                float* o_i = a.out + ((size_t)(a.Cout + co) * a.Fout + fo) * a.Jp + jA;
-                if (inb[1]) {
+                float* o_r = a.out + ((size_t)co * a.Fout + fo) * a.Jp + jA + (second ? 64 : 0);
+                float* o_i = a.out + ((size_t)(a.Cout + co) * a.Fout + fo) * a.Jp + jA + (second ? 64 : 0);
+                if (ib[1]) {
                     *(float2*)o_r = make_float2(yr[0], yr[1]);
                     *(float2*)o_i = make_float2(yi[0], yi[1]);
-                } else if (inb[0]) {
+                } else if (ib[0]) {
                     o_r[0] = yr[0];
                     o_i[0] = yi[0];
                 }
@@ -434,7 +458,29 @@
 
 __global__ void pack_cconv_tw_kernel(const float* __restrict__ wino, int cotiles, int UN, int UP, int vec, float* __restrict__ out) {
     const long long n0 = (long long)cotiles * UP * tw_ntp<0>() * 64, n1 = (long long)cotiles * UP * tw_ntp<1>() * 64;
-    for (long long idx = blockIdx.x * (long long)blockDim.x + threadIdx.x; idx < n0 + n1; idx += (long long)gridDim.x * blockDim.x) {
+    for (long long idx = blockIdx.x * (long long)blockDim.x + threadIdx.x; idx < n0 + n1 + n0; idx += (long long)gridDim.x * blockDim.x) {
+        if (idx >= n0 + n1) {
+            const long long i = idx - n0 - n1;
+            const int lane = (int)(i & 63);
+            long long t_ = i >> 6;
+            const int t = (int)(t_ % tw_ntp<0>()); t_ /= tw_ntp<0>();
+            const int u = (int)(t_ % UP), ct = (int)(t_ / UP);
+            const int pos = t * 64 + lane, w = pos / (9 * 64), q = pos % (9 * 64);
+            const bool vec_ = vec & 1;
+            const int k = !vec_ ? q >> 6 : (q < 512 ? (q >> 8) * 4 + (q & 3) : 8);
+            const int ln = !vec_ ? q & 63 : (q < 512 ? (q & 255) >> 2 : q - 512);
+            const int ci = 2 * u + (ln >> 5), co = ln & 31;
+            float val = 0.f;
+            if (ci * 3 < UN) {
+                const int g = k / 3, tau = k - g * 3;
+                const float* src = wino + (((size_t)ct * UN + (size_t)ci * 3 + g) * 4) * 64;
+                const float w0 = (w & 1) ? src[64 + co] - src[128 + co] : src[co];
+                const float w1 = (w & 1) ? src[64 + 32 + co] - src[128 + 32 + co] : src[32 + co];
+                val = tau == 0 ? w0 : (tau == 1 ? w0 + w1 : w1);
+            }
+            out[idx] = val;
+            continue;
+        }
         const int ph = idx >= n0;
         const long long i = ph ? idx - n0 : idx;
         const int ntp = ph ? tw_ntp<1>() : tw_ntp<0>(), nt = ph ? tw_nt<1>() : tw_nt<0>();
@@ -461,6 +507,36 @@
     }
 }
 
+__global__ void pack_cconv_tw_edge_kernel(const float* __restrict__ w_re, const float* __restrict__ w_im, int Cout, int Cin_used, int conj,
+                                          int cotiles, int UP, int vec, float* __restrict__ out) {
+    const long long n = (long long)cotiles * UP * tw_ntp<0>() * 64;
+    for (long long idx = blockIdx.x * (long long)blockDim.x + threadIdx.x; idx < n; idx += (long long)gridDim.x * blockDim.x) {
+        const int lane = (int)(idx & 63);
+        long long t_ = idx >> 6;
+        const int t = (int)(t_ % tw_ntp<0>()); t_ /= tw_ntp<0>();
+        const int u = (int)(t_ % UP);
+        const int ct = (int)(t_ / UP);
+        const int pos = t * 64 + lane, w = pos / (9 * 64), q = pos % (9 * 64);
+        const int k = !vec ? q >> 6 : (q < 512 ? (q >> 8) * 4 + (q & 3) : 8);
+        const int ln = !vec ? q & 63 : (q < 512 ? (q & 255) >> 2 : q - 512);
+        const int ci = 2 * u + (ln >> 5), co = ct * 32 + (ln & 31);
+        float val = 0.f;
+        if (co < Cout && ci < Cin_used) {
+            const int g = k / 3, tau = k - g * 3;
+            const int kf = (w & 1) ? 2 : 4;
+            float wh[2];
+#pragma unroll
+            for (int h = 0; h < 2; ++h) {
+                const size_t off = (((size_t)ci * Cout + co) * 5 + kf) * 2 + (1 - h);
+                const float wr = w_re[off], wi = conj ? -w_im[off] : w_im[off];
+                wh[h] = g == 0 ? wr : (g == 1 ? wi - wr : wr + wi);
+            }
+            val = tau == 0 ? wh[0] : (tau == 1 ? wh[0] + wh[1] : wh[1]);
+        }
+        out[idx] = val;
+    }
+}
+
 template <int PH, int CIK, bool LEFT, int DBG, int RDW, bool WVEC = true, bool STATS = false, int NCT = 1>
 int launch_tw_ph_l(const TwArgs& a, hipStream_t st);
 inline int tw_wvec_mask() {
@@ -492,6 +568,9 @@
     TwArgs b = a;
     b.jtiles = (a.J + 63) / 64;
     b.ftiles = PH == 1 ? a.Fin / 2 : (a.Fin + 1) / 2;
+    int edge_tiles = 0, main_tiles = b.ftiles;
+    if (PH == 0 && DBG == 0) edge_tiles = idv_tw_edge_tiles(1, a.Fin, a.Fout, b.jtiles, &main_tiles);
+    if (edge_tiles) b.ftiles = main_tiles;
     if (b.ftiles == 0) return IDV_OK;
     static const int xsplit = [] { const char* e = getenv("IDV_TW_XCD_SPLIT"); return e ? atoi(e) : 1; }();
     b.cgroups = b.cotiles / NCT;
@@ -504,6 +583,8 @@
         const int G = 8 / b.cgroups;
         nblk = (long long)((b.jtiles + G - 1) / G) * b.ftiles * 8;
     }
+    b.nmain = (int)(nblk > 0x7fffffffLL ? 0 : nblk);
+    nblk += (long long)edge_tiles * b.cgroups;
     if (nblk > 0x7fffffffLL) return IDV_EINVAL;
     auto k = cconv_tw_kernel<PH, CIK, LEFT, DBG, RDW, WVEC, STATS, NCT>;
     static std::atomic<bool> attr_set[64];
@@ -515,9 +596,36 @@
     }
     hipLaunchKernelGGL(k, dim3((unsigned)nblk), dim3(256 * NCT), smem, st, b);
     if (NCT > 1) idv_tw_pair_note_launch();
+    if (edge_tiles) idv_tw_edge_note_launch();
     return idv_launch_status();
 }
 
+}
+
+namespace {
+std::atomic<int>& tw_edge_mask() {
+    static std::atomic<int> v{[] { const char* e = getenv("IDV_TW_EDGE"); return e ? atoi(e) & IDV_TW_EDGE_ALL : IDV_TW_EDGE_DEFAULT; }()};
+    return v;
+}
+std::atomic<long long> tw_edge_launches{0};
+}
+void idv_tw_edge_note_launch() { tw_edge_launches.fetch_add(1, std::memory_order_relaxed); }
+extern "C" int idv_tw_edge(int mask) {
+    if (mask < 0) return tw_edge_mask().load(std::memory_order_relaxed);
+    return tw_edge_mask().exchange(mask & IDV_TW_EDGE_ALL, std::memory_order_relaxed);
+}
+extern "C" long long idv_tw_edge_launches(int reset) {
+    return reset ? tw_edge_launches.exchange(0, std::memory_order_relaxed) : tw_edge_launches.load(std::memory_order_relaxed);
+}
+extern "C" int idv_tw_edge_tiles(int transposed, int rows, int rows_other, int jtiles, int* main_tiles) {
+    const int padded = rows > 0 ? (rows + 1) / 2 : 0;
+    if (main_tiles) *main_tiles = padded;
+    if (rows < 3 || !(rows & 1) || jtiles < 1 || !(idv_tw_edge(-1) & (transposed ? IDV_TW_EDGE_T : IDV_TW_EDGE_CONV))) return 0;
+    if (transposed ? (2 * (rows - 1) >= rows_other || 2 * (rows - 1) + 2 < rows_other)
+                   : (2 * (rows - 1) >= rows_other || 2 * (rows - 1) + 1 < rows_other))
+        return 0;
+    if (main_tiles) *main_tiles = rows / 2;
+    return (jtiles + 1) / 2;
 }
 
 namespace {
@@ -545,7 +653,7 @@
 
 extern "C" long long idv_cconv_tw_wfrag_floats(int Cout, int cin_used) {
     const long long cotiles = (Cout + 31) / 32, cpad = (cin_used + TW_PACK_CI - 1) / TW_PACK_CI * TW_PACK_CI;
-    return cotiles * (cpad / 2) * (36 + 32) * 64;
+    return cotiles * (cpad / 2) * (36 + 32 + 36) * 64;
 }
 
 extern "C" int idv_pack_cconv_tw(const float* wino_frag, int Cout, int cin_used, float* tw_frag, void* stream) {
@@ -556,6 +664,18 @@
     const unsigned blocks = (unsigned)((n + 255) / 256 > 4096 ? 4096 : (n + 255) / 256);
     hipLaunchKernelGGL(pack_cconv_tw_kernel, dim3(blocks), dim3(256), 0, (hipStream_t)stream, wino_frag, cotiles, cpad * 3, cpad / 2,
                        tw_wvec_mask(), tw_frag);
+    return idv_launch_status();
+}
+
+extern "C" int idv_pack_cconv_tw_edge(const float* w_re, const float* w_im, int Cout, int Cin_total, int Cin_used, int conj, float* tw_frag,
+                                      void* stream) {
+    if (!w_re || !w_im || !tw_frag || Cout <= 0 || Cin_used <= 0 || Cin_used > Cin_total) return IDV_EINVAL;
+    const int cotiles = (Cout + 31) / 32;
+    const int cpad = (Cin_used + TW_PACK_CI - 1) / TW_PACK_CI * TW_PACK_CI;
+    const long long n = (long long)cotiles * (cpad / 2) * 36 * 64;
+    const unsigned blocks = (unsigned)((n + 255) / 256 > 4096 ? 4096 : (n + 255) / 256);
+    hipLaunchKernelGGL(pack_cconv_tw_edge_kernel, dim3(blocks), dim3(256), 0, (hipStream_t)stream, w_re, w_im, Cout, Cin_used, conj, cotiles,
+                       cpad / 2, tw_wvec_mask() & 1, tw_frag + (long long)cotiles * (cpad / 2) * (36 + 32) * 64);
     return idv_launch_status();
 }
 
diff --git a/i-dccrn-vae_amd/csrc/cgemm_tw2.hip b/i-dccrn-vae_amd/csrc/cgemm_tw2.hip
--- a/i-dccrn-vae_amd/csrc/cgemm_tw2.hip
+++ b/i-dccrn-vae_amd/csrc/cgemm_tw2.hip
@@ -30,9 +30,16 @@
 
 constexpr int TW2_PACK_CI = 8;
 
-__host__ __device__ constexpr int tw2_ra(int q) { return q == 0 ? 0 : (q == 1 ? 2 : (q == 2 ? 4 : (q == 3 ? 2 : (q == 4 ? 1 : 3)))); }
-__host__ __device__ constexpr int tw2_rb(int q) { return q == 0 ? 4 : (q == 1 ? 4 : (q == 2 ? 2 : (q == 3 ? 6 : (q == 4 ? 3 : (q == 5 ? 3 : 5))))); }
-__host__ __device__ constexpr float tw2_cb(int q) { return q == 1 ? 1.f : (q == 5 ? 0.f : -1.f); }
+template <bool EDGE = false> __host__ __device__ constexpr int tw2_ra(int q) {
+    if (EDGE) return q == 0 ? 0 : (q == 4 ? 1 : (q == 2 ? 2 : (q == 1 ? 3 : (q == 5 ? 4 : (q == 3 ? 5 : 0)))));
+    return q == 0 ? 0 : (q == 1 ? 2 : (q == 2 ? 4 : (q == 3 ? 2 : (q == 4 ? 1 : 3))));
+}
+template <bool EDGE = false> __host__ __device__ constexpr int tw2_rb(int q) {
+    if (EDGE) return tw2_ra<true>(q);
+    return q == 0 ? 4 : (q == 1 ? 4 : (q == 2 ? 2 : (q == 3 ? 6 : (q == 4 ? 3 : (q == 5 ? 3 : 5)))));
+}
+template <bool EDGE = false> __host__ __device__ constexpr float tw2_cb(int q) { return EDGE ? 0.f : (q == 1 ? 1.f : (q == 5 ? 0.f : -1.f)); }
+__host__ __device__ constexpr int tw2_edge_tap(int q) { return (q == 0 || q == 1) ? 0 : ((q == 4 || q == 5) ? 1 : ((q == 2 || q == 3) ? 2 : -1)); }
 __host__ __device__ constexpr int tw2_qx(int a) { return a == 0 ? 0 : (a == 1 ? 1 : 3); }
 __host__ __device__ constexpr int tw2_qy(int a) { return a == 0 ? 4 : (a == 1 ? 5 : 6); }
 __host__ __device__ constexpr int tw2_main_acc(int w) { return w == 2 ? 3 : w; }
@@ -56,7 +63,7 @@
 constexpr int tw2_smem_floats(int nct) {
     return nct == 1 ? 2 * 4 * 7 * 288 : (2 * (4 * 7 * 288 + 288) > 2 * 36 * 4 * 64 ? 2 * (4 * 7 * 288 + 288) : 2 * 36 * 4 * 64);
 }
-template <bool LEFT, bool STATS, int DBG = 0, int NCT = 1>
+template <bool LEFT, bool STATS, int DBG = 0, int NCT = 1, bool EDGE = false>
 __global__ __launch_bounds__(256 * NCT, NCT == 1 ? 2 : 1) void cconv_tw2_kernel(const Tw2Args a) {
     constexpr int NT = 36, NACC = 9, NSLOT = 16;
     constexpr int NRAW = 7, CIK = 4, KS = 2;
@@ -81,7 +88,11 @@
     const int bid = blockIdx.x;
     const int xcd = bid & 7, slot = bid >> 3;
     int jt, ft, ct;
-    if (a.xcd_split) {
+    if (EDGE) {
+        ct = bid % a.cgroups;
+        jt = 2 * (bid / a.cgroups);
+        ft = a.ftiles;
+    } else if (a.xcd_split) {
         const int G = 8 / a.cgroups;
         ct = xcd % a.cgroups;
         jt = (slot / a.ftiles) * G + xcd / a.cgroups;
@@ -98,6 +109,7 @@
     const int j0 = jt * 64;
     const int m0 = 2 * ft;
     const int rbase = 2 * m0 - 2;
+    const bool has_y = jt + 1 < a.jtiles;
 
     const int Cin = a.Cin;
     const int nchunk = (Cin + CIK - 1) / CIK;
@@ -119,11 +131,11 @@
         const int e = tid + i * NTHR;
         const int c8 = e & 15;
         const int cl = e / (16 * NRAW), rl = (NCT == 2 && e >= NITEM) ? 0 : (e >> 4) % NRAW;
-        const int f = rbase + rl;
-        const int jc = j0 + 4 * c8;
+        const int f = EDGE ? rbase + rl % 3 : rbase + rl;
+        const int jc = j0 + 4 * c8 + (EDGE && rl >= 3 ? 64 : 0);
         const int je = LEFT ? jc - 1 : jc + 4;
         const bool exists = e < NITEM;
-        const bool okr = exists && f >= 0 && f < a.Fin;
+        const bool okr = exists && f >= 0 && f < a.Fin && !(EDGE && (rl == 6 || (rl >= 3 && !has_y)));
         unsigned m = 0;
 #pragma unroll
         for (int q = 0; q < 5; ++q) {
@@ -199,7 +211,7 @@
         for (int j = 0; j < 5; ++j) stage_plane2(dst, i, j);
     };
 
-    const float* wbase = a.wfrag + (((size_t)ct * a.UP) * 4 + w4) * 1024 + lane * 4;
+    const float* wbase = a.wfrag + (EDGE ? (size_t)a.cotiles * a.UP * 4096 : 0) + (((size_t)ct * a.UP) * 4 + w4) * 1024 + lane * 4;
     const int total_ks = nchunk * KS;
     float a_w[NSLOT];
     auto load_wg = [&](int g, int grp) {
@@ -211,9 +223,9 @@
 
     const int am = tw2_main_acc(w4 < 3 ? w4 : 0);
     const int qxm = tw2_qx(am), qym = tw2_qy(am);
-    const int rxa = tw2_ra(qxm) * 288, rxb = tw2_rb(qxm) * 288, rya = tw2_ra(qym) * 288, ryb = tw2_rb(qym) * 288;
-    const float cbx = tw2_cb(qxm), cby = tw2_cb(qym);
-    const int r2a = tw2_ra(2) * 288 + w4 * 64, r2b = tw2_rb(2) * 288 + w4 * 64;
+    const int rxa = tw2_ra<EDGE>(qxm) * 288, rxb = tw2_rb<EDGE>(qxm) * 288, rya = tw2_ra<EDGE>(qym) * 288, ryb = tw2_rb<EDGE>(qym) * 288;
+    const float cbx = tw2_cb<EDGE>(qxm), cby = tw2_cb<EDGE>(qym);
+    const int r2a = tw2_ra<EDGE>(2) * 288 + w4 * 64, r2b = tw2_rb<EDGE>(2) * 288 + w4 * 64;
     float xa[2][4], xb[2][4];
     auto load_grp_a = [&](const float* base, int g, float (&oa)[4], float (&ob)[4]) {
         if (g < 3) {
@@ -234,8 +246,8 @@
             int q, plane;
             tw2_slot(3, 4 * g + s4, q, plane);
             if (q < 0) continue;
-            oa[s4] = base[tw2_ra(q) * 288 + tw2_poff(plane, l31)];
-            ob[s4] = base[tw2_rb(q) * 288 + tw2_poff(plane, l31)];
+            oa[s4] = base[tw2_ra<EDGE>(q) * 288 + tw2_poff(plane, l31)];
+            ob[s4] = base[tw2_rb<EDGE>(q) * 288 + tw2_poff(plane, l31)];
         }
     };
 
@@ -271,10 +283,10 @@
                     if (ROLE_B) {
                         int q, plane;
                         tw2_slot(3, k, q, plane);
-                        cb = tw2_cb(q);
+                        cb = tw2_cb<EDGE>(q);
                         ai = k < 12 ? k >> 1 : 6 + (k - 12);
                     } else {
-                        cb = k < 14 ? ((k & 1) ? cby : cbx) : -1.f;
+                        cb = k < 14 ? ((k & 1) ? cby : cbx) : tw2_cb<EDGE>(2);
                         ai = k < 14 ? k >> 1 : 7 + (k - 14);
                     }
                     if (s4 == 0) {
@@ -338,14 +350,17 @@
     const bool has_act = a.slope != nullptr;
     float* E = smem + cth * (NT * 4 * 64);
     const int jA = j0 + 2 * l31;
-    bool keep[2], inb[2];
-#pragma unroll
-    for (int q = 0; q < 2; ++q) {
-        const int j = jA + q;
-        const int tp = j % a.Tp;
-        inb[q] = j < a.J;
-        keep[q] = inb[q] && tp >= 1 && tp <= a.t_valid;
-    }
+    constexpr int NCB = EDGE ? 2 : 1;
+    bool keep[NCB][2], inb[NCB][2];
+#pragma unroll
+    for (int cbk = 0; cbk < NCB; ++cbk)
+#pragma unroll
+        for (int q = 0; q < 2; ++q) {
+            const int j = jA + 64 * cbk + q;
+            const int tp = j % a.Tp;
+            inb[cbk][q] = j < a.J;
+            keep[cbk][q] = inb[cbk][q] && tp >= 1 && tp <= a.t_valid;
+        }
 #pragma unroll
     for (int s = 0; s < 4; ++s) {
         if (s > 0) __syncthreads();
@@ -383,13 +398,16 @@
         float st[5] = {0.f, 0.f, 0.f, 0.f, 0.f};
 #pragma unroll
         for (int rt = 0; rt < 2; ++rt) {
-            const int fo = m0 + rt;
-            if (fo >= a.Fout) continue;
+            const int fo = EDGE ? m0 : m0 + rt;
+            if (fo >= a.Fout || (EDGE && rt == 1 && !has_y)) continue;
+            const int cbk = EDGE ? rt : 0;
             float yr[2], yi[2];
 #pragma unroll
             for (int q = 0; q < 2; ++q) {
-                const float re = rt == 0 ? pr[0][q] + pr[1][q] + pr[2][q] : pr[1][q] - pr[2][q] - pr[3][q];
-                const float im = rt == 0 ? pi[0][q] + pi[1][q] + pi[2][q] : pi[1][q] - pi[2][q] - pi[3][q];
+                const float re = EDGE ? pr[rt][q] + pr[rt + 2][q]
+                                      : (rt == 0 ? pr[0][q] + pr[1][q] + pr[2][q] : pr[1][q] - pr[2][q] - pr[3][q]);
+                const float im = EDGE ? pi[rt][q] + pi[rt + 2][q]
+                                      : (rt == 0 ? pi[0][q] + pi[1][q] + pi[2][q] : pi[1][q] - pi[2][q] - pi[3][q]);
                 float r_, i_;
                 if (a.has_fold) {
                     r_ = e0[0] * re + e0[1] * im + e4;
@@ -402,9 +420,9 @@
                     r_ = r_ >= 0.f ? r_ : slope * r_;
                     i_ = i_ >= 0.f ? i_ : slope * i_;
                 }
-                yr[q] = keep[q] ? r_ : 0.f;
-                yi[q] = keep[q] ? i_ : 0.f;
-                if (STATS && keep[q]) {
+                yr[q] = keep[cbk][q] ? r_ : 0.f;
+                yi[q] = keep[cbk][q] ? i_ : 0.f;
+                if (STATS && keep[cbk][q]) {
                     st[0] += yr[q];
                     st[1] += yi[q];
                     st[2] += yr[q] * yr[q];
@@ -413,12 +431,12 @@
                 }
             }
             if (cok) {
-                float* o_r = a.out + ((size_t)co * a.Fout + fo) * a.Jp + jA;
-                float* o_i = a.out + ((size_t)(a.Cout + co) * a.Fout + fo) * a.Jp + jA;
-                if (inb[1]) {
+                float* o_r = a.out + ((size_t)co * a.Fout + fo) * a.Jp + jA + 64 * cbk;
+                float* o_i = a.out + ((size_t)(a.Cout + co) * a.Fout + fo) * a.Jp + jA + 64 * cbk;
+                if (inb[cbk][1]) {
                     *(float2*)o_r = make_float2(yr[0], yr[1]);
                     *(float2*)o_i = make_float2(yi[0], yi[1]);
-                } else if (inb[0]) {
+                } else if (inb[cbk][0]) {
                     o_r[0] = yr[0];
                     o_i[0] = yi[0];
                 }
@@ -438,6 +456,41 @@
 }
 
 __global__ void pack_cconv_tw2_kernel(const float* __restrict__ wino, int cotiles, int UN, int UP, float* __restrict__ out) {
+    const long long n = (long long)cotiles * UP * 4096;
+    for (long long idx2 = blockIdx.x * (long long)blockDim.x + threadIdx.x; idx2 < 2 * n; idx2 += (long long)gridDim.x * blockDim.x) {
+        const bool edge = idx2 >= n;
+        const long long idx = edge ? idx2 - n : idx2;
+        const int kk = (int)(idx & 3), ln = (int)((idx >> 2) & 63), grp = (int)((idx >> 8) & 3), w = (int)((idx >> 10) & 3);
+        const long long t_ = idx >> 12;
+        const int u = (int)(t_ % UP), ct = (int)(t_ / UP);
+        int q, plane;
+        tw2_slot(w, grp * 4 + kk, q, plane);
+        float val = 0.f;
+        const int ci = 2 * u + (ln >> 5), co = ln & 31;
+        if (edge) {
+            const int kf = q >= 0 ? tw2_edge_tap(q) : -1;
+            if (kf >= 0 && ci * 3 < UN) {
+                const int g = plane / 3, tau = plane % 3;
+                const float* src = wino + (((size_t)ct * UN + (size_t)ci * 3 + g) * 8) * 64;
+                const float w0 = kf == 0 ? src[co] : (kf == 1 ? src[4 * 64 + co] : src[64 + co] - src[128 + co]);
+                const float w1 = kf == 0 ? src[32 + co] : (kf == 1 ? src[4 * 64 + 32 + co] : src[64 + 32 + co] - src[128 + 32 + co]);
+                val = tau == 0 ? w0 : (tau == 1 ? w0 + w1 : w1);
+            }
+            out[idx2] = val;
+            continue;
+        }
+        if (q >= 0 && ci * 3 < UN) {
+            const int g = plane / 3, tau = plane % 3;
+            const float* src = wino + ((((size_t)ct * UN + (size_t)ci * 3 + g) * 8 + q)) * 64;
+            const float w0 = src[co], w1 = src[32 + co];
+            val = tau == 0 ? w0 : (tau == 1 ? w0 + w1 : w1);
+        }
+        out[idx2] = val;
+    }
+}
+
+__global__ void pack_cconv_tw2_edge_kernel(const float* __restrict__ w_re, const float* __restrict__ w_im, int Cout, int Cin_total, int Cin_used,
+                                           int conj, int cotiles, int UP, float* __restrict__ out) {
     const long long n = (long long)cotiles * UP * 4096;
     for (long long idx = blockIdx.x * (long long)blockDim.x + threadIdx.x; idx < n; idx += (long long)gridDim.x * blockDim.x) {
         const int kk = (int)(idx & 3), ln = (int)((idx >> 2) & 63), grp = (int)((idx >> 8) & 3), w = (int)((idx >> 10) & 3);
@@ -446,24 +499,31 @@
         int q, plane;
         tw2_slot(w, grp * 4 + kk, q, plane);
         float val = 0.f;
-        const int ci = 2 * u + (ln >> 5), co = ln & 31;
-        if (q >= 0 && ci * 3 < UN) {
+        const int ci = 2 * u + (ln >> 5), co = ct * 32 + (ln & 31);
+        const int kf = q >= 0 ? tw2_edge_tap(q) : -1;
+        if (kf >= 0 && co < Cout && ci < Cin_used) {
             const int g = plane / 3, tau = plane % 3;
-            const float* src = wino + ((((size_t)ct * UN + (size_t)ci * 3 + g) * 8 + q)) * 64;
-            const float w0 = src[co], w1 = src[32 + co];
-            val = tau == 0 ? w0 : (tau == 1 ? w0 + w1 : w1);
+            float wh[2];
+#pragma unroll
+            for (int h = 0; h < 2; ++h) {
+                const size_t off = (((size_t)co * Cin_total + ci) * 5 + kf) * 2 + h;
+                const float wr = w_re[off], wi = conj ? -w_im[off] : w_im[off];
+                wh[h] = g == 0 ? wr : (g == 1 ? wi - wr : wr + wi);
+            }
+            val = tau == 0 ? wh[0] : (tau == 1 ? wh[0] + wh[1] : wh[1]);
         }
         out[idx] = val;
     }
 }
 
-template <bool LEFT, bool STATS, int DBG, int NCT = 1>
-int launch_tw2(const Tw2Args& a, hipStream_t st) {
+template <bool LEFT, bool STATS, int DBG, int NCT = 1, bool EDGE = false>
+int launch_tw2(const Tw2Args& a, hipStream_t st, int edge_tiles = 0) {
     constexpr size_t smem = tw2_smem_floats(NCT) * sizeof(float);
     static_assert(smem * (NCT == 1 ? 2 : 1) <= 160 * 1024, "the patch buffers of two workgroups (NCT = 2: of one) must fit the 160 KB of LDS");
     Tw2Args b = a;
     b.jtiles = (a.J + 63) / 64;
-    b.ftiles = (a.Fout + 1) / 2;
+    b.ftiles = edge_tiles ? a.Fout / 2 : (a.Fout + 1) / 2;
+    if (b.ftiles == 0 || (EDGE && !edge_tiles)) return IDV_OK;
     static const int xsplit = [] { const char* e = getenv("IDV_TW_XCD_SPLIT"); return e ? atoi(e) : 1; }();
     b.cgroups = b.cotiles / NCT;
     if (b.cgroups * NCT != b.cotiles) return IDV_EINVAL;
@@ -475,8 +535,9 @@
         const int G = 8 / b.cgroups;
         nblk = (long long)((b.jtiles + G - 1) / G) * b.ftiles * 8;
     }
+    if (EDGE) nblk = (long long)edge_tiles * b.cgroups;
     if (nblk > 0x7fffffffLL) return IDV_EINVAL;
-    auto k = cconv_tw2_kernel<LEFT, STATS, DBG, NCT>;
+    auto k = cconv_tw2_kernel<LEFT, STATS, DBG, NCT, EDGE>;
     static std::atomic<bool> attr_set[64];
     int dev = 0;
     if (hipGetDevice(&dev) != hipSuccess || dev < 0 || dev >= 64) return IDV_ELAUNCH;
@@ -485,7 +546,8 @@
         attr_set[dev].store(true, std::memory_order_release);
     }
     hipLaunchKernelGGL(k, dim3((unsigned)nblk), dim3(256 * NCT), smem, st, b);
-    if (NCT > 1) idv_tw_pair_note_launch();
+    if (NCT > 1 && !EDGE) idv_tw_pair_note_launch();
+    if (EDGE) idv_tw_edge_note_launch();
     return idv_launch_status();
 }
 
@@ -500,7 +562,7 @@
 
 extern "C" long long idv_cconv_tw2_wfrag_floats(int Cout, int cin_used) {
     const long long cotiles = (Cout + 31) / 32, cpad = (cin_used + TW2_PACK_CI - 1) / TW2_PACK_CI * TW2_PACK_CI;
-    return cotiles * (cpad / 2) * 4096;
+    return cotiles * (cpad / 2) * 4096 * 2;
 }
 
 extern "C" int idv_pack_cconv_tw2(const float* wino_frag, int Cout, int cin_used, float* tw_frag, void* stream) {
@@ -511,6 +573,18 @@
     const unsigned blocks = (unsigned)((n + 255) / 256 > 4096 ? 4096 : (n + 255) / 256);
     hipLaunchKernelGGL(pack_cconv_tw2_kernel, dim3(blocks), dim3(256), 0, (hipStream_t)stream, wino_frag, cotiles, cpad * 3, cpad / 2,
                        tw_frag);
+    return idv_launch_status();
+}
+
+extern "C" int idv_pack_cconv_tw2_edge(const float* w_re, const float* w_im, int Cout, int Cin_total, int Cin_used, int conj, float* tw_frag,
+                                       void* stream) {
+    if (!w_re || !w_im || !tw_frag || Cout <= 0 || Cin_used <= 0 || Cin_used > Cin_total) return IDV_EINVAL;
+    const int cotiles = (Cout + 31) / 32;
+    const int cpad = (Cin_used + TW2_PACK_CI - 1) / TW2_PACK_CI * TW2_PACK_CI;
+    const long long n = (long long)cotiles * (cpad / 2) * 4096;
+    const unsigned blocks = (unsigned)((n + 255) / 256 > 4096 ? 4096 : (n + 255) / 256);
+    hipLaunchKernelGGL(pack_cconv_tw2_edge_kernel, dim3(blocks), dim3(256), 0, (hipStream_t)stream, w_re, w_im, Cout, Cin_total, Cin_used, conj,
+                       cotiles, cpad / 2, tw_frag + n);
     return idv_launch_status();
 }
 
@@ -543,14 +617,16 @@
     if (!stats && dbg == 3) return tshift ? launch_tw2<true, false, 3>(a, st) : launch_tw2<false, false, 3>(a, st);
 #endif
     const bool pair = a.cotiles % 2 == 0 && (idv_tw_pair(-1) & IDV_TW_PAIR_CONV);
-    if (stats && pair)
-        rc = tshift ? launch_tw2<true, true, 0, 2>(a, st) : launch_tw2<false, true, 0, 2>(a, st);
-    else if (stats)
-        rc = tshift ? launch_tw2<true, true, 0>(a, st) : launch_tw2<false, true, 0>(a, st);
-    else if (pair)
-        rc = tshift ? launch_tw2<true, false, 0, 2>(a, st) : launch_tw2<false, false, 0, 2>(a, st);
-    else
-        rc = tshift ? launch_tw2<true, false, 0>(a, st) : launch_tw2<false, false, 0>(a, st);
+    const int et = idv_tw_edge_tiles(0, a.Fout, Fin, (a.J + 63) / 64, nullptr);
+    auto go = [&](auto edge_) -> int {
+        constexpr bool E = decltype(edge_)::value;
+        if (stats && pair) return tshift ? launch_tw2<true, true, 0, 2, E>(a, st, et) : launch_tw2<false, true, 0, 2, E>(a, st, et);
+        if (stats) return tshift ? launch_tw2<true, true, 0, 1, E>(a, st, et) : launch_tw2<false, true, 0, 1, E>(a, st, et);
+        if (pair) return tshift ? launch_tw2<true, false, 0, 2, E>(a, st, et) : launch_tw2<false, false, 0, 2, E>(a, st, et);
+        return tshift ? launch_tw2<true, false, 0, 1, E>(a, st, et) : launch_tw2<false, false, 0, 1, E>(a, st, et);
+    };
+    rc = go(std::false_type{});
+    if (!rc && et) rc = go(std::true_type{});
     if (rc || !(stats && stats_work)) return rc;
     return idv_launch_stats_collapse(stats_work, stats_rep, Cout * 5, stats, st);
 }
diff --git a/i-dccrn-vae_amd/csrc/common.hpp b/i-dccrn-vae_amd/csrc/common.hpp
--- a/i-dccrn-vae_amd/csrc/common.hpp
+++ b/i-dccrn-vae_amd/csrc/common.hpp
@@ -36,3 +36,4 @@
 
 int idv_launch_stats_collapse(const double* work, int rep, int n, double* stats, hipStream_t st);
 void idv_tw_pair_note_launch();
+void idv_tw_edge_note_launch();
diff --git a/i-dccrn-vae_amd/ops.py b/i-dccrn-vae_amd/ops.py
--- a/i-dccrn-vae_amd/ops.py
+++ b/i-dccrn-vae_amd/ops.py
@@ -266,6 +266,25 @@
     return int(L.lib().idv_tw_pair_launches(1 if reset else 0))
 
 
+TW_EDGE = None
+_tw_edge_lib = None
+_tw_edge_pushed = None
+
+
+def _sync_tw_edge():
+    global _tw_edge_lib, _tw_edge_pushed
+    if TW_EDGE == _tw_edge_pushed:
+        return
+    if _tw_edge_lib is None:
+        _tw_edge_lib = int(L.lib().idv_tw_edge(-1))
+    L.lib().idv_tw_edge(_tw_edge_lib if TW_EDGE is None else int(TW_EDGE))
+    _tw_edge_pushed = TW_EDGE
+
+
+def tw_edge_launches(reset: bool = False) -> int:
+    return int(L.lib().idv_tw_edge_launches(1 if reset else 0))
+
+
 def _pack_wino_tw(w_re, w_im, cout: int, cin_total: int, cin_used: int, transposed: bool, conj: int):
     wf = _pack_wino(w_re, w_im, cout, cin_total, cin_used, transposed, conj)
     if wf is None or not TW or (not transposed and not TW_CONV):
@@ -273,9 +292,11 @@
     if transposed:
         tw = torch.empty(int(_ll_fn("idv_cconv_tw_wfrag_floats")(i(cout), i(cin_used))), dtype=torch.float32, device=w_re.device)
         call("idv_pack_cconv_tw", p(wf), i(cout), i(cin_used), p(tw), stream_ptr())
+        call("idv_pack_cconv_tw_edge", p(w_re), p(w_im), i(cout), i(cin_total), i(cin_used), i(conj), p(tw), stream_ptr())
     else:
         tw = torch.empty(int(_ll_fn("idv_cconv_tw2_wfrag_floats")(i(cout), i(cin_used))), dtype=torch.float32, device=w_re.device)
         call("idv_pack_cconv_tw2", p(wf), i(cout), i(cin_used), p(tw), stream_ptr())
+        call("idv_pack_cconv_tw2_edge", p(w_re), p(w_im), i(cout), i(cin_total), i(cin_used), i(conj), p(tw), stream_ptr())
     return wf, tw
 
 
@@ -507,6 +528,7 @@
             cfg = TW_CFG + (1 if tshift else 0)
         swork = _stats_work(stats, cout)
         _sync_tw_pair()
+        _sync_tw_edge()
         call("idv_ctconv2d_tw_fwd", x.ptr(), i(x.C), skip.ptr() if skip is not None else p(None), i(c1), p(gauss[4]), p(gauss[1]),
              i(gauss[2]), p(slope), out.ptr(), p(stats), p(swork), i(STATS_REP), i(tshift), i(cout), i(x.F), i(x.B), i(x.Tp), i(x.Jp),
              i(t_out), addend.ptr() if addend is not None else p(None), i(addend_div), i(addend.Jp if addend is not None else 0),
@@ -516,6 +538,7 @@
             cfg = TW_CFG + 2 + (1 if tshift else 0)
         swork = _stats_work(stats, cout)
         _sync_tw_pair()
+        _sync_tw_edge()
         call("idv_cconv2d_tw_fwd", x.ptr(), i(x.C), p(gauss[4]), p(gauss[1]), i(gauss[2]), p(slope), out.ptr(), p(stats), p(swork),
              i(STATS_REP), i(tshift), i(cout), i(x.F), i(x.B), i(x.Tp), i(x.Jp), i(t_out), stream_ptr())
     elif skip_div == 1 and _wino_ok(gauss, transposed, x, c1, cout, skip.Jp if skip is not None else None):
@@ -1023,12 +1046,14 @@
         if LAUNCH_LOG is not None:
             cfg = TW_CFG + (1 if tshift_adj else 0)
         _sync_tw_pair()
+        _sync_tw_edge()
         call("idv_ctconv2d_tw_fwd", dy.ptr(), i(dy.C), p(None), i(0), p(gauss[4]), p(gauss[1]), i(0), p(None), out.ptr(), p(None), p(None),
              i(0), i(tshift_adj), i(cout_adj), i(dy.F), i(dy.B), i(dy.Tp), i(dy.Jp), i(t_out), p(None), i(1), i(0), stream_ptr())
     elif wfrag_bf16 is None and not adj_transposed and _tw2_ok(gauss, dy, 0, cout_adj):
         if LAUNCH_LOG is not None:
             cfg = TW_CFG + 2 + (1 if tshift_adj else 0)
         _sync_tw_pair()
+        _sync_tw_edge()
         call("idv_cconv2d_tw_fwd", dy.ptr(), i(dy.C), p(gauss[4]), p(gauss[1]), i(0), p(None), out.ptr(), p(None), p(None), i(0),
              i(tshift_adj), i(cout_adj), i(dy.F), i(dy.B), i(dy.Tp), i(dy.Jp), i(t_out), stream_ptr())
     elif wfrag_bf16 is None and _wino_ok(gauss, adj_transposed, dy, 0, cout_adj, None):
diff --git a/include/idccrn_hip.h b/include/idccrn_hip.h
--- a/include/idccrn_hip.h
+++ b/include/idccrn_hip.h
@@ -328,6 +328,18 @@
 int idv_tw_pair(int mask);
 long long idv_tw_pair_launches(int reset);
 
+#define IDV_TW_EDGE_T 1
+#define IDV_TW_EDGE_CONV 2
+#define IDV_TW_EDGE_ALL 3
+#define IDV_TW_EDGE_DEFAULT 3
+int idv_pack_cconv_tw_edge(const float* w_re, const float* w_im, int Cout, int Cin_total, int Cin_used, int conj, float* tw_frag,
+                           void* stream);
+int idv_pack_cconv_tw2_edge(const float* w_re, const float* w_im, int Cout, int Cin_total, int Cin_used, int conj, float* tw_frag,
+                            void* stream);
+int idv_tw_edge(int mask);
+long long idv_tw_edge_launches(int reset);
+int idv_tw_edge_tiles(int transposed, int rows, int rows_other, int jtiles, int* main_tiles);
+
 #ifdef __cplusplus
 }
 #endif
```

Result: faster. 995.8 utterances/sec, median of 6 (+4.2%).
